# lelecaruso/NavierStokes_Project_NM4PDE

Hardware: AMD Instinct MI355X
Metric: time-steps/sec (assemble_time_step + solve_time_step), 3D flow past a cylinder, P2/P1, Yosida, per-rank ILU(0) (higher is better)
Workload: dtype f64

## Files before the change

### include/nsx.h

```cpp
#ifndef NSX_H
#define NSX_H

#include <stdint.h>

#ifdef __cplusplus
extern "C" {
#endif

typedef struct nsx_handle nsx_handle;

typedef enum {
  NSX_OK = 0,
  NSX_ERR_ARG = -1,
  NSX_ERR_HIP = -2,
  NSX_ERR_UNSUPPORTED = -3,
  NSX_ERR_NOCONV = -4,
  NSX_ERR_NUMERIC = -5,
  NSX_ERR_COMM = -6
} nsx_status;

typedef enum { NSX_PREC_YOSIDA = 0, NSX_PREC_SIMPLE = 1, NSX_PREC_AYOSIDA = 2, NSX_PREC_ASIMPLE = 3 } nsx_prec;

enum {
  NSX_TEMAM = 1,
// ... 32 lines not shown
                 int n_u, int n_p);

int nsx_set_ranks(nsx_handle *h, int n_ranks, const int32_t *u_ptr, const int32_t *p_ptr);
int nsx_set_schur_blocks(nsx_handle *h, int n_blocks, const int32_t *p_ptr);

enum { NSX_ORDER_FIRST_TOUCH = 0, NSX_ORDER_COLOUR = 1, NSX_ORDER_COLOUR_ALL = 2 };
int nsx_set_internal_layout(nsx_handle *h, int n_virtual_ranks, int order, int schur_max_rows);
int nsx_layout_info(nsx_handle *h, int info[5]);
int nsx_layout_get(nsx_handle *h, int32_t *node_perm, int32_t *pnode_perm, int32_t *u_ptr, int32_t *p_ptr, int32_t *schur_ptr);

int nsx_set_solution(nsx_handle *h, const double *solution_owned);
int nsx_get_solution(nsx_handle *h, double *solution_owned);
int nsx_get_solution_ghosted(nsx_handle *h, double *solution);
int nsx_get_rhs(nsx_handle *h, double *system_rhs);
int nsx_set_rhs(nsx_handle *h, const double *system_rhs);


int nsx_assemble(nsx_handle *h, int flags);
int nsx_assemble_time_step(nsx_handle *h, int flags);
int nsx_add_rhs(nsx_handle *h, int n, const int32_t *dofs, const double *values);
int nsx_apply_boundary_values(nsx_handle *h, int n, const int32_t *dofs, const double *values);
int nsx_solve_time_step(nsx_handle *h, int prec_type, double tol_abs, double inner_rtol, int maxiter,
                        int inner_maxiter, nsx_solve_stats *stats);

int nsx_prec_initialize(nsx_handle *h, int prec_type);
int nsx_prec_vmult(nsx_handle *h, int prec_type, double inner_rtol, int inner_maxiter, double *dst, const double *src,
                   nsx_solve_stats *stats);
int nsx_system_vmult(nsx_handle *h, double *dst, const double *src);
int nsx_ilu_apply(nsx_handle *h, int which, double *dst, const double *src);

enum { NSX_INNER_FP64 = 0, NSX_INNER_FP32 = 1 };
int nsx_set_inner_precision(nsx_handle *h, int precision);
int nsx_inner_F_vmult(nsx_handle *h, double *dst, const double *src);

int nsx_export_block(nsx_handle *h, int which, int block, int n_rows, const int32_t *rowptr, const int32_t *colind,
                     double *values);
int nsx_schur_nnz(nsx_handle *h, int64_t *nnz);
int nsx_schur_get(nsx_handle *h, int32_t *rowptr, int32_t *colind, double *values);
int nsx_scalar_graph_nnz(nsx_handle *h, int which, int64_t *nnz);
int nsx_scalar_graph(nsx_handle *h, int which, int32_t *rowptr, int32_t *colind);
int nsx_ilu_get(nsx_handle *h, int which, double *values);

int nsx_set_force_faces(nsx_handle *h, int n_faces, const int32_t *cells, const int32_t *local_faces, int n_qf, const double *N2f,
                        const double *dN2f, const double *N1f, const double *wf);
int nsx_compute_forces(nsx_handle *h, double *drag, double *lift);

int nsx_profile_enable(nsx_handle *h, int on);
int nsx_profile_reset(nsx_handle *h);
int nsx_profile_count(nsx_handle *h);
int nsx_profile_get(nsx_handle *h, int i, const char **name, int64_t *launches, double *total_ms, double *bytes_per_launch);

int nsx_persistent_state(nsx_handle *h, int state[4]);

int nsx_path_info(nsx_handle *h, int info[32]);

int nsx_gram_schmidt_cycle(nsx_handle *h, int n, int m, double *vectors, double norm_guard, double *coeffs, double *norms2);

int nsx_comm_unique_id(uint8_t id[128]);
int nsx_comm_init(nsx_handle *h, int rank, int world, const uint8_t id[128]);
typedef int (*nsx_allreduce_fn)(void *ctx, double *buf, int count);
typedef int (*nsx_exchange_fn)(void *ctx, int n, const int *ranks, const double *const *send, const int *send_count,
                               double *const *recv, const int *recv_count);
int nsx_comm_init_callbacks(nsx_handle *h, int rank, int world, nsx_allreduce_fn allreduce, nsx_exchange_fn exchange, void *ctx);
int nsx_comm_counters(const nsx_handle *h, long long counts[2]);
int nsx_comm_self_halo_test(nsx_handle *h, int n_own, int n_ghost, int ncomp, double *max_err);
int nsx_set_mesh_distributed(nsx_handle *h, int n_cells, int n_cells_layer1, int dofs_per_cell, const int32_t *cell_dofs,
// ... 10 lines not shown
```

### include/nsx_host.h

```cpp
#ifndef NSX_HOST_H
#define NSX_HOST_H

#include <stdint.h>

#ifdef __cplusplus
extern "C" {
#endif

typedef struct nsxh_mesh nsxh_mesh;
typedef struct nsxh_dofs nsxh_dofs;
typedef struct nsxh_tables nsxh_tables;


nsxh_mesh *nsxh_mesh_cylinder(int dim, int m, int nr, int nxu, int nxd, int nyb, int nyt, int nz,
                              double grade_x, double grade_r);
nsxh_mesh *nsxh_mesh_cylinder_level(int dim, int level);
nsxh_mesh *nsxh_mesh_cube(int n);
nsxh_mesh *nsxh_mesh_box(int dim, int nx, int ny, int nz, const double *lo, const double *hi);
nsxh_mesh *nsxh_mesh_read_msh(const char *path);
void nsxh_mesh_free(nsxh_mesh *);

int nsxh_mesh_dim(const nsxh_mesh *);
int nsxh_mesh_n_vertices(const nsxh_mesh *);
int nsxh_mesh_n_cells(const nsxh_mesh *);
// ... 52 lines not shown
const int32_t *nsxh_rank_view_send_u_ptr(const nsxh_rank_view *);
const int32_t *nsxh_rank_view_send_u_nodes(const nsxh_rank_view *);
const int32_t *nsxh_rank_view_send_p_ptr(const nsxh_rank_view *);
const int32_t *nsxh_rank_view_send_p_nodes(const nsxh_rank_view *);


nsxh_tables *nsxh_tables_create(int dim, int rule, int order);
void nsxh_tables_free(nsxh_tables *);
int nsxh_tables_n_q(const nsxh_tables *);
int nsxh_tables_n_p2(const nsxh_tables *);
int nsxh_tables_n_p1(const nsxh_tables *);
const double *nsxh_tables_points(const nsxh_tables *);
const double *nsxh_tables_weights(const nsxh_tables *);
const double *nsxh_tables_N2(const nsxh_tables *);
const double *nsxh_tables_dN2(const nsxh_tables *);
const double *nsxh_tables_N1(const nsxh_tables *);
const double *nsxh_tables_dN1(const nsxh_tables *);
int nsxh_tables_n_qf(const nsxh_tables *);


int nsxh_write_vtu(const nsxh_dofs *, const double *solution, const char *directory, const char *basename, unsigned counter);

int nsxh_pressure_difference(const nsxh_dofs *, const double *solution, const double *point_a, const double *point_b, double *diff);


int nsxh_ilu_stream_stats(int n_rows, const int32_t *rowptr, const int32_t *colind, int n_blocks, const int32_t *block_ptr,
                          int blocks_per_wave, int ncomp, int gap, int entries_per_tick, int64_t out[6]);
int nsxh_ilu_stream_apply(int n_rows, const int32_t *rowptr, const int32_t *colind, int n_blocks, const int32_t *block_ptr,
                          int blocks_per_wave, int ncomp, int gap, int entries_per_tick, const double *lu, const double *b, double *x);

int nsxh_ilu_stream_apply_f32(int n_rows, const int32_t *rowptr, const int32_t *colind, int n_blocks, const int32_t *block_ptr,
                              int blocks_per_wave, int ncomp, int gap, int entries_per_tick, const double *lu, const double *b, double *x);

int nsxh_internal_layout(int dim, int n_cells, int dofs_per_cell, const int32_t *cell_dofs, const double *cell_coords, int n_u, int n_p,
                         int n_in_ranks, const int32_t *in_u_ptr, const int32_t *in_p_ptr, int n_virtual, int order, int schur_max_rows,
                         int32_t *node_perm, int32_t *pnode_perm, int32_t *n_ranks, int32_t *u_ptr, int32_t *p_ptr, int32_t *n_schur,
                         int32_t *schur_ptr, int32_t *colours);

#ifdef __cplusplus
}
#endif
#endif
```

### navierstokes_project_nm4pde_amd/csrc/nsx_blas.hip

```cpp
#include "nsx_grid.hpp"
#include "nsx_ilu_lanes.hpp"

namespace nsx {

constexpr int RED_BLOCKS = 512;
constexpr int RED_STRIDE = 1024;

struct SRef {
  double c;
  int num, den;
  int num_nb, den_nb;
};

__device__ __forceinline__ double wave_sum_all(double v) {
#pragma unroll
  for (int o = 32; o > 0; o >>= 1) v += __shfl_xor(v, o, 64);
  return v;
}

__device__ __forceinline__ double slot_value(const double *__restrict__ scal, const double *__restrict__ partial, int slot, int nb,
                                             double *sh) {
  if (nb == 0) return scal[slot];
  if (threadIdx.x < 64) {
    const double *p = partial + (size_t)slot * RED_STRIDE;
// ... 1780 lines not shown
    double nrm2 = read_scalar(h, S_LS_NORM);
    if (nrm2 != nrm2) {
      v_dot(h, sp, w, w, S_LS_NORM);
      nrm2 = read_scalar(h, S_LS_NORM);
    }
    out[dim] = nrm2;
    if (ran_ahead) h->mgs_redo_ahead = true;
    return false;
  }
  if (!normalize) return false;
  return !consider || std::sqrt(out[dim]) > 10. * std::sqrt(out[dim + 1]) * 1.4901161193847656e-08;
}

__global__ __launch_bounds__(256) void k_axpby(int n, int split, int gap, double *__restrict__ d, SRef s, SRef a, const double *__restrict__ v,
                                               const double *__restrict__ scal, const double *__restrict__ partial, int mode) {
  __shared__ double sh;
  const double sv = mode == 1 ? 0.0 : sval(scal, partial, s, &sh), av = mode == 2 ? 0.0 : sval(scal, partial, a, &sh);
#pragma unroll 4
  for (int i0 = blockIdx.x * 256 + threadIdx.x; i0 < n; i0 += gridDim.x * 256) {
    const int i = i0 + (i0 >= split ? gap : 0);
    if (mode == 0) d[i] = sv * d[i] + av * v[i];
    else if (mode == 1) d[i] = av * v[i];
    else d[i] = sv * d[i];
  }
}
__global__ void k_scale_vec(int n, double *__restrict__ d, const double *__restrict__ f) {
  for (int i = blockIdx.x * 256 + threadIdx.x; i < n; i += gridDim.x * 256) d[i] *= f[i];
}
struct MultiArgs {
  const double *v[32];
  double c[32];
  int k;
};
__global__ void k_axpy_multi(int n, int split, int gap, double *__restrict__ x, MultiArgs m) {
  for (int i0 = blockIdx.x * 256 + threadIdx.x; i0 < n; i0 += gridDim.x * 256) {
    const int i = i0 + (i0 >= split ? gap : 0);
    double s = x[i];
    for (int j = 0; j < m.k; ++j) s += m.c[j] * m.v[j][i];
    x[i] = s;
  }
}
__global__ __launch_bounds__(256) void k_cg_update(int n, double *__restrict__ x, const double *__restrict__ dvec, double *__restrict__ g,
                                                   const double *__restrict__ hvec, SRef a, const double *__restrict__ scal,
                                                   const double *__restrict__ partial_in, double *__restrict__ partial) {
  __shared__ double sh[5];
  const double alpha = sval(scal, partial_in, a, sh + 4);
  double acc = 0.0;
#pragma unroll 2
  for (int i = blockIdx.x * 256 + threadIdx.x; i < n; i += gridDim.x * 256) {
    x[i] += alpha * dvec[i];
    const double gi = g[i] + alpha * hvec[i];
    g[i] = gi;
    acc += gi * gi;
  }
  const double t = block_sum_256(acc, sh);
  if (threadIdx.x == 0) partial[blockIdx.x] = t;
}

static int ew_blocks(int n) { return std::max(1, std::min(2048, cdiv(n, 512))); }

static void axpby(nsx_handle *h, Span sp, double *d, SRef s, SRef a, const double *v, int mode, double bytes_per) {
  const int n = sp.n;
  LaunchScope ls(h, "axpby", bytes_per * n);
  hipLaunchKernelGGL(k_axpby, dim3(ew_blocks(n)), dim3(256), 0, h->stream, n, sp.split, sp.gap, d, s, a, v, h->scal.p, h->red_partial.p, mode);
}

void v_copy(nsx_handle *h, int n, double *d, const double *s) {
  if (d != s && n) HIP_CHECK(hipMemcpyAsync(d, s, (size_t)n * sizeof(double), hipMemcpyDeviceToDevice, h->stream));
}
void v_zero(nsx_handle *h, int n, double *d) {
  if (n) HIP_CHECK(hipMemsetAsync(d, 0, (size_t)n * sizeof(double), h->stream));
}
void v_add(nsx_handle *h, Span n, double *d, double a, const double *v) { axpby(h, n, d, SRef{1, -1, -1, 0, 0}, SRef{a, -1, -1, 0, 0}, v, 0, 24); }
void v_add_dev(nsx_handle *h, Span n, double *d, double a, int slot, const double *v) {
  axpby(h, n, d, SRef{1, -1, -1, 0, 0}, sref(h, a, slot, -1), v, 0, 24);
}
void v_sadd(nsx_handle *h, Span n, double *d, double s, double a, const double *v) {
  axpby(h, n, d, SRef{s, -1, -1, 0, 0}, SRef{a, -1, -1, 0, 0}, v, 0, 24);
}
void v_scale(nsx_handle *h, Span n, double *d, double a) { axpby(h, n, d, SRef{a, -1, -1, 0, 0}, SRef{0, -1, -1, 0, 0}, nullptr, 2, 16); }
void v_scale_dev_inv(nsx_handle *h, Span n, double *d, int slot) { axpby(h, n, d, sref(h, 1, -1, slot), SRef{0, -1, -1, 0, 0}, nullptr, 2, 16); }
void v_scale_vec(nsx_handle *h, int n, double *d, const double *f) {
  LaunchScope ls(h, "scale_vec", 24.0 * n);
  hipLaunchKernelGGL(k_scale_vec, dim3(ew_blocks(n)), dim3(256), 0, h->stream, n, d, f);
}
void v_axpy_multi(nsx_handle *h, Span sp, double *x, int k, double *const *vs, const double *coef) {
  const int n = sp.n;
  for (int j0 = 0; j0 < k; j0 += 32) {
    MultiArgs m;
    m.k = std::min(32, k - j0);
    for (int j = 0; j < m.k; ++j) {
      m.v[j] = vs[j0 + j];
      m.c[j] = coef[j0 + j];
    }
    LaunchScope ls(h, "axpy_multi", 8.0 * n * (2 + m.k));
    hipLaunchKernelGGL(k_axpy_multi, dim3(ew_blocks(n)), dim3(256), 0, h->stream, n, sp.split, sp.gap, x, m);
  }
}

void cg_update(nsx_handle *h, int n, double *x, const double *d, double *g, const double *hv, int gh_slot, int dh_slot, int res_slot) {
  LaunchScope ls(h, "cg_update", 48.0 * n);
  const int nb = red_blocks(h, n);
  hipLaunchKernelGGL(k_cg_update, dim3(nb), dim3(256), 0, h->stream, n, x, d, g, hv, sref(h, 1, gh_slot, dh_slot), h->scal.p,
                     h->red_partial.p, red_out(h, res_slot, nb));
  after_reduction(h, res_slot, nb);
}
void cg_direction(nsx_handle *h, int n, double *d, const double *hv, int num_slot, int den_slot) {
  axpby(h, n, d, sref(h, 1, num_slot, den_slot), SRef{-1, -1, -1, 0, 0}, hv, 0, 24);
}

double read_scalar(nsx_handle *h, int slot) {
  double v;
  read_scalars(h, slot, 1, &v);
  return v;
}
unsigned long long publish_scalars(nsx_handle *h, int slot0, int count) {
  if (count > 64) NSX_THROW(NSX_ERR_ARG, "internal: read_scalars range too long");
  NbArgs args;
  for (int i = 0; i < count; ++i) {
    args.nb[i] = h->slot_nb[slot0 + i];
    h->slot_nb[slot0 + i] = 0;
  }
  const unsigned long long seq = ++h->pub_seq;
  unsigned long long *flag_dev = (unsigned long long *)(h->pub_dev + N_SLOTS);
  hipLaunchKernelGGL(k_publish, dim3(count), dim3(256), 0, h->stream, slot0, count, args, h->red_partial.p, h->scal.p, h->pub_dev, flag_dev, seq,
                     h->pub_counter.p);
  return seq;
}
void collect_published(nsx_handle *h, unsigned long long seq, int slot0, int count, double *out) {
// ... 93 lines not shown
    info[7] = h->cu_reserved;
    info[8] = h->cg_last_path;
    info[9] = h->schedS.n_blocks;
    info[10] = (int)h->haloU.nbr.size();
    info[11] = h->haloU.nbr.empty() ? 0 : h->haloU.send_ptr[h->haloU.nbr.size()];
    info[12] = h->N2_loc - h->N2;
    info[13] = h->schedS.dense ? 1 : 0;
    info[14] = h->mgs_disabled ? 1 : 0;
    info[15] = h->n_persistent_fallbacks;
    if (!h->mgs_disabled) {
      nsx::mgs_setup(h);
      auto fit = [&](int n, const int *caps, int n_inst) {
        for (int k = 0; k < n_inst; ++k) {
          const int es[3] = {8, 10, 12};
          if (caps[k] <= 0) continue;
          const int nwg = std::max(1, std::min(caps[k], nsx::cdiv(n, 256 * 4)));
          if (nsx::cdiv(n, (int64_t)nwg * 256) <= es[k]) return es[k];
        }
        return 0;
      };
      info[16] = fit(h->n_u, h->mgs_max_wg_dist, 1);
      info[17] = fit(h->n_u, h->mgs_dist_cap_reserved, 3);
      info[18] = fit(h->n_u + h->n_p, h->mgs_max_wg_dist, 1);
      info[19] = fit(h->n_u + h->n_p, h->mgs_dist_cap_reserved, 3);
      info[21] = fit(h->n_u, h->mgs_max_wg_e, 3);
    }
    info[20] = nsx::cdiv(std::max(1, h->schedS.n_blocks), 1024);
    info[22] = h->N2;
    info[23] = h->NP;
    info[24] = h->mgs_last_fused;
    info[25] = h->mgs_fused_launches;
    info[26] = h->inner_F_fp32_used;
    info[27] = h->ilu_F_fp32_used;
  } catch (const nsx::Error &e) {
    h->err = e.msg;
    return e.code;
  }
  return NSX_OK;
}
```

### navierstokes_project_nm4pde_amd/csrc/nsx_cg.hip

```cpp
#include "nsx_grid.hpp"

namespace nsx {

constexpr int CG_THREADS = 256;
constexpr int CG_NW = CG_THREADS / 64, CG_NG = CG_THREADS / 16;
constexpr int CG_MAXB = 256;
constexpr int CG_MAX_WG = 1024;
constexpr int CG_NV = 3;
constexpr int CG_RING = 4;
constexpr size_t CG_REGION = (size_t)CG_RING * CG_NV * CG_MAX_WG + (size_t)CG_RING * CG_NV;
enum { S_CGP = 100 };

__device__ __forceinline__ double ld_agent(const double *p) { return __hip_atomic_load(p, __ATOMIC_RELAXED, __HIP_MEMORY_SCOPE_AGENT); }
__device__ __forceinline__ void st_agent(double *p, double v) { __hip_atomic_store(p, v, __ATOMIC_RELAXED, __HIP_MEMORY_SCOPE_AGENT); }

template <int W>
__device__ __forceinline__ double cg_group_sum(double v) {
  v += dpp_f64<0xB1>(v);
  v += dpp_f64<0x4E>(v);
  if (W >= 8) v += dpp_f64<0x141>(v);
  if (W >= 16) v += dpp_f64<0x140>(v);
  return v;
}

// ... 100 lines not shown
                                              double (&va)[CG_PF], int (&la)[CG_PF]) {
  const int grp = tid >> 4, lane = tid & 15;
  double vb[CG_PF];
  int lb[CG_PF];
  double acc = 0.0;
#define NSX_CG_USE(V, L, S0)                                    \
  _Pragma("unroll") for (int k = 0; k < CG_PF; ++k) {           \
    const int s_ = (S0) + k;                                    \
    if (s_ < s1) {                                              \
      acc += V[k] * xst[L[k]];                                  \
      const int inf = sinfo[s_];                                \
      if (inf & 0x8000) {                                       \
        const double r_ = cg_group_sum<16>(acc);                \
        if (lane == 0) hvs[(inf & 0x7fff) * 16 + grp] = r_;     \
        acc = 0.0;                                              \
      }                                                         \
    }                                                           \
  }
  for (int sb = s0; sb < s1; sb += 2 * CG_PF) {
    NSX_CG_LOAD(vb, lb, sb + CG_PF)
    NSX_CG_USE(va, la, sb)
    NSX_CG_LOAD(va, la, sb + 2 * CG_PF)
    NSX_CG_USE(vb, lb, sb + CG_PF)
  }
#undef NSX_CG_USE
}
#undef NSX_CG_LOAD

template <int RPG, bool LRES>
__global__ __launch_bounds__(CG_THREADS) void k_cg_schur(const int32_t *__restrict__ bptr, const int32_t *__restrict__ u_ptr,
                                                  const int32_t *__restrict__ u_cols, const int32_t *__restrict__ s_ptr,
                                                  const double *__restrict__ sval, const uint16_t *__restrict__ slidx,
                                                  const int32_t *__restrict__ sinfo, const int64_t *__restrict__ dn_off,
                                                  const double *__restrict__ P, const double *__restrict__ b, double *x, double *D0, double *D1,
                                                  double *H, double rtol, int maxiter, unsigned long long *box, unsigned long long *box_other,
                                                  double *pub_vals, unsigned long long *pub_flag, unsigned long long seq, int *err_dev, int drop_wg,
                                                  const int32_t *__restrict__ a_rowptr, const double *__restrict__ a_val,
                                                  const uint16_t *__restrict__ a_lidx) {
  static_assert(!LRES || RPG > 0, "the LDS-resident operator needs the register-resident block inverses");
  constexpr int MAXB = RPG > 0 ? 16 * RPG : CG_MAXB;
  __shared__ double gs[MAXB], hs[MAXB], ds[MAXB], hvs[MAXB], xs[MAXB], xst[CG_MAX_UCOLS];
  __shared__ double sh[4][CG_NV * 8], bc[CG_NV];
  __shared__ int s_err;
  __shared__ double lval[LRES ? CG_LPOOL : 1];
  __shared__ uint16_t lidx[LRES ? CG_LPOOL : 2];
  __shared__ int lrow[LRES ? MAXB + 1 : 1];
  const int wg = blockIdx.x, tid = threadIdx.x, nwg = gridDim.x;
  if (tid == 0) s_err = 0;
  for (size_t q = (size_t)wg * CG_THREADS + tid; q < CG_REGION; q += (size_t)nwg * CG_THREADS) box_other[q] = GX_EMPTY;
  const int r0 = bptr[wg], nb = bptr[wg + 1] - r0;
  const int u0 = u_ptr[wg], nu = u_ptr[wg + 1] - u0;
  const int half = tid >> 8, ht = tid & 255;
  const int s0 = s_ptr[3 * wg + half], s1 = s_ptr[3 * wg + (CG_THREADS == 512 ? half + 1 : 2)];
  const double *Pb = P + dn_off[wg];
  const int grp = tid >> 4, lane = tid & 15;
  const bool own = tid < nb;
  int e = 0;
  constexpr int NU = CG_MAX_UCOLS / CG_THREADS;
  int ucol[NU];
#pragma unroll
  for (int k = 0; k < NU; ++k) ucol[k] = tid + CG_THREADS * k < nu ? u_cols[u0 + tid + CG_THREADS * k] : -1;
  if (tid < MAXB) gs[tid] = 0.0;

  double pa[8], pb[8];
  auto fetch = [&](int q, double(&pv)[8]) {
    const bool live = q < nb;
    const double *prow = Pb + (size_t)(live ? q : 0) * nb;
// ... 76 lines not shown
  double va[LRES ? 1 : CG_PF];
  int la[LRES ? 1 : CG_PF];
  if constexpr (LRES) {
    const int p0 = a_rowptr[r0], nz = a_rowptr[r0 + nb] - p0;
    for (int q = tid; q < nz; q += CG_THREADS) {
      lval[q] = a_val[p0 + q];
      lidx[q] = a_lidx[p0 + q];
    }
    if (tid <= nb) lrow[tid] = a_rowptr[r0 + tid] - p0;
  }
  auto prefetch_A = [&]() {
    if constexpr (!LRES) cg_spmv_prefetch(s0, s1, sval, slidx, ht, va, la);
  };
  auto block_spmv = [&]() {
    if constexpr (LRES) {
#pragma unroll
      for (int r = 0; r < RPG; ++r) {
        const int q = grp + CG_NG * r;
        if (q < nb) {
          const int e1 = lrow[q + 1];
          double acc = 0.0;
          for (int e = lrow[q] + lane; e < e1; e += 16) acc += lval[e] * xst[lidx[e]];
          acc = cg_group_sum<16>(acc);
          if (lane == 0) hvs[q] = acc;
        }
      }
    } else {
      cg_block_spmv(s0, s1, sval, slidx, sinfo, xst, hvs, ht, va, la);
    }
  };

  double bi = 0.0;
  if (own) {
    xs[tid] = x[r0 + tid];
    bi = b[r0 + tid];
  }
#pragma unroll
  for (int k = 0; k < NU; ++k)
    if (ucol[k] >= 0) xst[tid + CG_THREADS * k] = x[ucol[k]];
  prefetch_A();
  __syncthreads();
  block_spmv();
  __syncthreads();
  prefetch_P();
  if (own) gs[tid] = hvs[tid] - bi;
  __syncthreads();
  apply_P();
  double tot3[3];
  {
    const double part[3] = {own ? gs[tid] * gs[tid] : 0.0, own ? bi * bi : 0.0, own ? gs[tid] * hs[tid] : 0.0};
    cg_post<3>(part, box, e, nwg, sh, &s_err, wg == drop_wg);
    prefetch_A();
    if (!cg_collect<3>(tot3, box, e++, bc, &s_err)) {
      if (tid == 0) __hip_atomic_store(err_dev, 1, __ATOMIC_RELAXED, __HIP_MEMORY_SCOPE_AGENT);
      if (wg == 0 && tid == 0) {
        __hip_atomic_store(pub_vals + 2, 3.0, __ATOMIC_RELAXED, __HIP_MEMORY_SCOPE_SYSTEM);
        asm volatile("s_waitcnt vmcnt(0)" ::: "memory");
        __hip_atomic_store(pub_flag, seq, __ATOMIC_RELAXED, __HIP_MEMORY_SCOPE_SYSTEM);
      }
      return;
    }
  }
  const double tol = rtol * sqrt(tot3[1]);
  double res = sqrt(tot3[0]), gh = tot3[2], beta = 0.0;
  int it = 0;
  int conv = res <= tol ? 1 : ((it >= maxiter || res != res) ? 2 : 0);
  bool dead = false;
  while (conv == 0) {
    ++it;
    const double *Dp = (it & 1) ? D0 : D1;
    double *Dc = (it & 1) ? D1 : D0;
#pragma unroll
// ... 122 lines not shown
  hipLaunchKernelGGL(k_cg_pack, dim3(cdiv(pl.n_slots, 256)), dim3(256), 0, h->stream, pl.n_slots, pl.s_src.p, h->vSchur.p, pl.s_val.p);
  pl.values_current = true;
}

static void cg_setup(nsx_handle *h) {
  if (h->cg_box.p || h->cg_disabled) return;
  h->cg_max_wg = 0;
  if (getenv("NSX_CG_PERSISTENT") && atoi(getenv("NSX_CG_PERSISTENT")) == 0) {
    h->cg_disabled = true;
    return;
  }
  int cus = 0, per_cu = 0;
  HIP_CHECK(hipDeviceGetAttribute(&cus, hipDeviceAttributeMultiprocessorCount, h->prm.device));
  int per_cu_res[2] = {0, 0};
  HIP_CHECK(hipOccupancyMaxActiveBlocksPerMultiprocessor(&per_cu, k_cg_schur<0, false>, CG_THREADS, 0));
  HIP_CHECK(hipOccupancyMaxActiveBlocksPerMultiprocessor(&per_cu_res[0], k_cg_schur<6, false>, CG_THREADS, 0));
  HIP_CHECK(hipOccupancyMaxActiveBlocksPerMultiprocessor(&per_cu_res[1], k_cg_schur<8, false>, CG_THREADS, 0));
  h->cg_max_wg_res[0] = std::min(CG_MAX_WG, per_cu_res[0] * cus);
  h->cg_max_wg_res[1] = std::min(CG_MAX_WG, per_cu_res[1] * cus);
  int per_cu_lres[2] = {0, 0};
  HIP_CHECK(hipOccupancyMaxActiveBlocksPerMultiprocessor(&per_cu_lres[0], k_cg_schur<6, true>, CG_THREADS, 0));
  HIP_CHECK(hipOccupancyMaxActiveBlocksPerMultiprocessor(&per_cu_lres[1], k_cg_schur<8, true>, CG_THREADS, 0));
  h->cg_max_wg_lres[0] = std::min(CG_MAX_WG, per_cu_lres[0] * cus);
  h->cg_max_wg_lres[1] = std::min(CG_MAX_WG, per_cu_lres[1] * cus);
  h->cg_box.alloc(2 * CG_REGION + 2);
  HIP_CHECK(hipMemsetAsync(h->cg_box.p, 0xff, 2 * CG_REGION * sizeof(unsigned long long), h->stream));
  HIP_CHECK(hipMemsetAsync(h->cg_box.p + 2 * CG_REGION, 0, 2 * sizeof(unsigned long long), h->stream));
  h->cg_max_wg = std::min(CG_MAX_WG, per_cu * cus);
  if (getenv("NSX_DEBUG"))
    fprintf(stderr, "[nsx] persistent Schur CG: %d CUs x %d resident workgroups, grid <= %d (block inverses in registers: <= 96 rows x %d, <= 128 rows x %d; operator in LDS as well: x %d, x %d)\n", cus, per_cu,
            h->cg_max_wg, per_cu_res[0], per_cu_res[1], per_cu_lres[0], per_cu_lres[1]);
}

bool cg_schur_persistent(nsx_handle *h, double *x, const double *b, double rtol, int maxiter, int *steps, double *last, int *status) {
  const IluSchedule &s = h->schedS;
  const CgPlan &pl = h->cgplan;
  if (h->comm || !s.dense || s.max_rows > CG_MAXB || !pl.ok || !pl.values_current) return false;
  cg_setup(h);
  if (h->cg_max_wg == 0 || s.n_blocks > h->cg_max_wg) return false;
  const bool pres_ok = !(getenv("NSX_CG_PRES") && atoi(getenv("NSX_CG_PRES")) == 0);
  const int rpg = !pres_ok ? 0 : (s.max_rows <= 96 && s.n_blocks <= h->cg_max_wg_res[0]) ? 6 : (s.max_rows <= 128 && s.n_blocks <= h->cg_max_wg_res[1]) ? 8 : 0;
  const bool pres = rpg > 0;
  const bool lres_ok = !(getenv("NSX_CG_LRES") && atoi(getenv("NSX_CG_LRES")) == 0);
  const bool lres = lres_ok && pres && pl.max_block_nnz <= CG_LPOOL && s.n_blocks <= h->cg_max_wg_lres[rpg == 6 ? 0 : 1];
  const int n = h->n_p;
  if ((int)h->cg_vec.n < 3 * n) h->cg_vec.alloc((size_t)3 * n);
  double *D0 = h->cg_vec.p, *D1 = D0 + n, *H = D1 + n;
  const unsigned long long seq = ++h->pub_seq;
  unsigned long long *box = h->cg_box.p + (size_t)h->cg_parity * CG_REGION, *box_other = h->cg_box.p + (size_t)(1 - h->cg_parity) * CG_REGION;
  int *err_dev = (int *)(h->cg_box.p + 2 * CG_REGION);
  double *pub_vals = h->pub_dev + S_CGP;
  unsigned long long *pub_flag = (unsigned long long *)(h->pub_dev + N_SLOTS);
  ProfEntry *pe = nullptr;
  {
    LaunchScope ls(h, "cg_S", 0.0);
    pe = ls.e;
#define NSX_CG_GO(PRES_, LRES_)                                                                                                                       \
  hipLaunchKernelGGL((k_cg_schur<PRES_, LRES_>), dim3(s.n_blocks), dim3(CG_THREADS), 0, h->stream, s.block_ptr.p, pl.u_ptr.p, pl.u_cols.p, pl.s_ptr.p,  \
                     pl.s_val.p, pl.s_lidx.p, pl.s_info.p, s.dn_off.p, s.dn_P.p, b, x, D0, D1, H, rtol, maxiter, box, box_other, pub_vals, pub_flag, seq, \
                     err_dev, h->gx_drop_wg, h->gS.rowptr.p, h->vSchur.p, pl.a_lidx.p)
    if (rpg == 6 && lres) NSX_CG_GO(6, true); else if (rpg == 8 && lres) NSX_CG_GO(8, true);
    else if (rpg == 6) NSX_CG_GO(6, false); else if (rpg == 8) NSX_CG_GO(8, false); else NSX_CG_GO(0, false);
#undef NSX_CG_GO
    if (getenv("NSX_DEBUG") && (h->cg_resident != pres || h->cg_lds_resident != lres || !h->cg_variant_said)) {
      fprintf(stderr, "[nsx] Schur CG variant: block inverses in registers %d (rows per lane group %d), operator in LDS %d (largest block: %d entries)\n", (int)pres, rpg,
              (int)lres, (int)pl.max_block_nnz);
      h->cg_variant_said = true;
    }
    h->cg_resident = pres;
    h->cg_lds_resident = lres;
  }
  h->cg_parity ^= 1;
  h->cg_last_path = 2;
  wait_published(h, seq);
  const int st = (int)h->pub_host[S_CGP + 2];
  if (st == 3) {
    HIP_CHECK(hipStreamSynchronize(h->stream));
    HIP_CHECK(hipMemsetAsync(h->cg_box.p, 0xff, 2 * CG_REGION * sizeof(unsigned long long), h->stream));
    HIP_CHECK(hipMemsetAsync(h->cg_box.p + 2 * CG_REGION, 0, 2 * sizeof(unsigned long long), h->stream));
    h->cg_max_wg = 0;
    h->cg_disabled = true;
    h->n_persistent_fallbacks++;
    fprintf(stderr, "[nsx] warning: the persistent Schur CG timed out (grid not co-resident): this handle uses one launch per operation from now on\n");
    return false;
  }
  *steps = (int)h->pub_host[S_CGP];
  *last = h->pub_host[S_CGP + 1];
  *status = st;
  if (pe) pe->bytes += (lres ? 1.0 : (double)(*steps + 1)) * 10.0 * h->gS.nnz() + (double)(*steps + 1) * 48.0 * n + (pres ? 1.0 : (double)(*steps + 1)) * 8.0 * (double)s.dn_entries;
  return true;
}

// ... 264 lines not shown
```

### navierstokes_project_nm4pde_amd/csrc/nsx_internal.hpp

```cpp
#pragma once
#include <hip/hip_runtime.h>

#include <cstdint>
#include <cstdio>
#include <cstring>
#include <map>
#include <string>
#include <functional>
#include <vector>

#include "../../include/nsx.h"
#include "../host/graph.hpp"

#ifndef NSX_NT
#define NSX_NT 1
#endif
template <int BIT, class T>
__device__ __forceinline__ T ld_stream(const T *p) {
  if constexpr ((NSX_NT & BIT) != 0) return __builtin_nontemporal_load(p);
  else return *p;
}

namespace nsx {

// ... 165 lines not shown
  int N2_loc = 0, NP_loc = 0;
  int n_cells1 = 0;
  int g_u = 0, g_p = 0, off_p = 0, len_blk = 0, len_u = 0, len_p = 0;
  bool dist = false;
  int rank = 0, world = 1, goff_u = 0, goff_p = 0, n_u_glob = 0, n_p_glob = 0;
  std::vector<int32_t> ghost_u, ghost_p;
  nsx::HaloPlan haloU, haloP;
  nsx::RowSplit splitA, splitVel, splitB, splitG, splitS;
  hipStream_t comm_stream = nullptr;
  hipEvent_t ev_ready = nullptr;
  bool have_tables = false, have_mesh = false, assembled = false, prec_ready = false;
  std::vector<double> N2_h, dN2_h, N1_h, w_h;
  nsx::DevBuf<double> tab_N2, tab_dN2, tab_N1, tab_w, tab_N2T, tab_dN2T;
  nsx::DevBuf<int32_t> cell_n2, cell_n1;
  nsx::DevBuf<double> geo;
  std::vector<int32_t> cell_n2_h, cell_n1_h;
  std::vector<int32_t> cell_n2_in, cell_n1_in;
  std::vector<double> cell_coords_in;
  std::vector<int32_t> in_rank_u_h, in_rank_p_h, in_sblk_h;
  int layout_req_ranks = 0, layout_req_order = 0, layout_req_schur = 0;
  bool layout_on = false;
  int layout_colours = 0, layout_colours_p = 0;
  std::vector<int32_t> perm2_h, perm1_h, iperm2_h, iperm1_h;
  nsx::DevBuf<int32_t> perm2_d, perm1_d;
  nsx::DevBuf<double> io_stage;
  nsx::Csr caller_graph[2];
  std::vector<int32_t> caller_pos[2];
  nsx::DevCsr gA, gG, gB, gS, gPM;
  nsx::SpmvBlocked blkA;
  nsx::DevBuf<double> vS0, vMass, vStiff, vConv, vF, vG, vB, vPM, vSchur, luF, luS;
  int inner_precision = NSX_INNER_FP64;
  nsx::DevBuf<float> vF32;
  int inner_F_fp32_used = 0, ilu_F_fp32_used = 0;
  nsx::DevBuf<int32_t> bt_of_g;
  nsx::GatherMap gmA, gmG, gmB, gmPM;
  nsx::DevBuf<double> cellbuf;
  nsx::DevBuf<double> sol, sol_owned, prev_sol, rhs;
  std::vector<int32_t> rank_u_h, rank_p_h, sblk_h;
  nsx::DevBuf<int32_t> rank_u;
  nsx::IluSchedule schedF, schedS;
  nsx::DevBuf<double> dbar;
  nsx::DevBuf<int32_t> bc_dofs;
  nsx::DevBuf<double> bc_vals;
  nsx::DevBuf<double> dirmask;
  std::vector<int32_t> bc_cache;
  nsx::DevBuf<double> diag_D, diag_D_inv, neg_diag_D_inv, lump_M, schur_w;
  nsx::DevBuf<double> schur_w_prev;
  bool schur_valid = false, schur_pending = false;
  int schur_type = -1;
  std::vector<nsx::DevBuf<double> *> pool;
  nsx::DevBuf<double> red_partial;
  nsx::DevBuf<double> scal;
  int slot_nb[nsx::N_SLOTS] = {0};
  double *scal_host = nullptr;
  double *pub_host = nullptr, *pub_dev = nullptr;
  unsigned long long pub_seq = 0;
  nsx::DevBuf<unsigned int> pub_counter;
  nsx::DevBuf<unsigned long long> mgs_box;
  bool sched_dirty = true;
  int mgs_used_wg[2] = {0, 0}, mgs_used_steps[2] = {0, 0};
  int mgs_parity = 0, mgs_max_wg = 0;
  int mgs_max_wg_e[3] = {0, 0, 0};
  int mgs_links = 2;
  bool mgs_disabled = false;
  double mgs_guard_override = -1.0;
  int gx_drop_wg = -1;
// ... 56 lines not shown
  LaunchScope(nsx_handle *h_, const char *name, double bytes) : h(h_) {
    if (!h->prof_on) return;
    e = &h->prof[name];
    e->bytes += bytes;
    (void)hipEventCreate(&a);
    (void)hipEventCreate(&b);
    (void)hipEventRecord(a, h->stream);
  }
  ~LaunchScope() {
    if (!e) return;
    (void)hipEventRecord(b, h->stream);
    e->launches++;
    e->pending.emplace_back(a, b);
  }
};

inline int cdiv(int64_t a, int64_t b) { return (int)((a + b - 1) / b); }

void setup_ilu_schedule(nsx_handle *h, const Csr &g, const std::vector<int32_t> &block_ptr, IluSchedule &s, int blocks_per_wave, bool allow_dense = false,
                        int ncomp = 1);
void build_schur_graph(nsx_handle *h);
void vec_from_caller(nsx_handle *h, double *dev, const double *host, bool with_ghosts);
void vec_to_caller(nsx_handle *h, const double *dev, double *host);
void part_from_caller(nsx_handle *h, int which, double *dev, const double *host);
void part_to_caller(nsx_handle *h, int which, const double *dev, double *host);
inline int32_t node_to_internal(const nsx_handle *h, int32_t local_node) { return h->layout_on ? h->perm2_h[local_node] : local_node; }
inline int32_t pnode_to_internal(const nsx_handle *h, int32_t local_node) { return h->layout_on ? h->perm1_h[local_node] : local_node; }
void ensure_schedules(nsx_handle *h);

void run_assemble(nsx_handle *h, bool first, int flags);
void run_dirichlet(nsx_handle *h, int n, const int32_t *dofs, const double *vals);

bool blocked_usable(const nsx_handle *h);
void spmv_F(nsx_handle *h, const double *vals, const double *x, double *y, const float *vals32 = nullptr);
void spmv_F_inner(nsx_handle *h, const double *x, double *y);
void convert_F_f32(nsx_handle *h);
void spmv_saddle(nsx_handle *h, const double *x, double *y);
void spmv_G(nsx_handle *h, const double *xp, double *yu, bool accumulate);
void spmv_B(nsx_handle *h, const double *xu, double *yp);
void spmv_S(nsx_handle *h, const double *x, double *y);
void schur_numeric(nsx_handle *h, const double *w);
void ilu_factor(nsx_handle *h, const DevCsr &g, IluSchedule &s, const double *vals, double *lu, const char *name, bool f32 = false);
void ilu_check(nsx_handle *h);
bool ilu_solve(nsx_handle *h, const DevCsr &g, const IluSchedule &s, const double *lu, const double *b, double *x, int ncomp,
               const char *name, int dot_slot = -1, bool f32 = false, int *used_f32 = nullptr);
void extract_diag(nsx_handle *h, const DevCsr &g, const double *vals, double *d);
void abs_rowsum(nsx_handle *h, const DevCsr &g, const double *vals, double *d);

struct Span {
  int n, split, gap;
  Span(int n_) : n(n_), split(n_), gap(0) {}
  Span(int n_, int split_, int gap_) : n(n_), split(split_), gap(gap_) {}
};
inline Span blk_span(const nsx_handle *h) { return Span(h->n_u + h->n_p, h->n_u, h->g_u); }

template <int CTRL>
__device__ __forceinline__ double dpp_f64(double v) {
  int lo = __double2loint(v), hi = __double2hiint(v);
  lo = __builtin_amdgcn_update_dpp(0, lo, CTRL, 0xf, 0xf, true);
  hi = __builtin_amdgcn_update_dpp(0, hi, CTRL, 0xf, 0xf, true);
  return __hiloint2double(hi, lo);
}
template <int CTRL, int ROW_MASK>
__device__ __forceinline__ double dpp_f64_rows(double v) {
  int lo = __double2loint(v), hi = __double2hiint(v);
  lo = __builtin_amdgcn_update_dpp(0, lo, CTRL, ROW_MASK, 0xf, false);
  hi = __builtin_amdgcn_update_dpp(0, hi, CTRL, ROW_MASK, 0xf, false);
  return __hiloint2double(hi, lo);
}

void v_copy(nsx_handle *h, int n, double *d, const double *s);
void v_zero(nsx_handle *h, int n, double *d);
void v_add(nsx_handle *h, Span n, double *d, double a, const double *v);
void v_add_dev(nsx_handle *h, Span n, double *d, double a, int slot, const double *v);
void v_sadd(nsx_handle *h, Span n, double *d, double s, double a, const double *v);
void v_scale(nsx_handle *h, Span n, double *d, double a);
void v_scale_dev_inv(nsx_handle *h, Span n, double *d, int slot);
void v_scale_vec(nsx_handle *h, int n, double *d, const double *f);
void v_dot(nsx_handle *h, Span n, const double *a, const double *b, int slot);
void v_add_and_dot(nsx_handle *h, Span n, double *d, double a, int aslot, const double *v, const double *w, int slot);
bool v_mgs(nsx_handle *h, Span n, double *w, int dim, double *const *vs, int slot0, bool normalize, double *out,
           const std::function<void()> *after_launch = nullptr, bool consider = false, double *gram = nullptr, const double *ilu_rhs = nullptr);
void v_axpy_multi(nsx_handle *h, Span n, double *x, int k, double *const *vs, const double *coef_host);
void finalize_slots(nsx_handle *h, int slot0, int count);
double *red_out(nsx_handle *h, int slot, int nb);
void after_reduction(nsx_handle *h, int slot, int nb);
void defer_reductions(nsx_handle *h, bool on);
double read_scalar(nsx_handle *h, int slot);
void read_scalars(nsx_handle *h, int slot0, int count, double *out);
unsigned long long publish_scalars(nsx_handle *h, int slot0, int count);
void collect_published(nsx_handle *h, unsigned long long seq, int slot0, int count, double *out);
void wait_published(nsx_handle *h, unsigned long long seq);
void build_cg_plan(nsx_handle *h);
void cg_pack_values(nsx_handle *h);
bool cg_schur_persistent(nsx_handle *h, double *x, const double *b, double rtol, int maxiter, int *steps, double *last, int *status);
bool cg_schur_fused(nsx_handle *h, double *x, const double *b, double rtol, int maxiter, int *steps, double *last, int *status);
void write_scalar(nsx_handle *h, int slot, double v);

void prec_initialize(nsx_handle *h, int type);
void prec_confirm(nsx_handle *h);
void prec_vmult(nsx_handle *h, int type, double inner_rtol, int inner_maxiter, double *dst, const double *src,
                nsx_solve_stats *st);
void solve_time_step(nsx_handle *h, int type, double tol, double inner_rtol, int maxiter, int inner_maxiter,
                     nsx_solve_stats *st);

void comm_allreduce_scalars(nsx_handle *h, int slot0, int count);
void comm_allreduce_partials(nsx_handle *h, double *partials, int count);
bool comm_agree_all(nsx_handle *h, bool mine);
void comm_release_cus(nsx_handle *h);
bool comm_reserve_cus(nsx_handle *h);
bool comm_streams_concurrent(nsx_handle *h);
bool comm_on_stream(const nsx_handle *h);
void comm_ext_allreduce(nsx_handle *h, double *vals, int count, int fail_word, unsigned int *arrive, unsigned int expected, unsigned long long *flag,
                        unsigned long long seq);
void comm_halo(nsx_handle *h, HaloPlan &plan, double *x, int ncomp);
void comm_halo_begin(nsx_handle *h, HaloPlan &plan, double *x, int ncomp,
                     const std::function<void(hipStream_t, double *sendbuf, const int32_t *send_idx, int n_send)> *packer = nullptr);
void comm_halo_finish(nsx_handle *h, HaloPlan &plan, double *x, int ncomp);
void build_row_splits(nsx_handle *h);
inline void comm_halo_u(nsx_handle *h, const double *x) { if (h->dist) comm_halo(h, h->haloU, const_cast<double *>(x), h->dim); }
inline void comm_halo_p(nsx_handle *h, const double *x) { if (h->dist) comm_halo(h, h->haloP, const_cast<double *>(x), 1); }
void comm_destroy(nsx_handle *h);

}
```

### navierstokes_project_nm4pde_amd/csrc/nsx_setup.hip

```cpp
#include <algorithm>
#include <cmath>
#include <numeric>

#include "nsx_internal.hpp"
#include "../host/ilu_stream.hpp"
#include "../host/layout.hpp"

using namespace nsx;

static thread_local std::string g_create_error;

namespace nsx {

static void upload_csr(nsx_handle *h, DevCsr &d, bool square) {
  d.rowptr.upload(d.host.rowptr, h->stream);
  d.colind.upload(d.host.colind, h->stream);
  if (square) {
    std::vector<int32_t> diag(d.host.n_rows);
    for (int32_t i = 0; i < d.host.n_rows; ++i) {
      diag[i] = find_in_row(d.host, i, i);
      if (diag[i] < 0) NSX_THROW(NSX_ERR_ARG, "square graph has no diagonal entry in row %d", i);
    }
    d.diag.upload(diag, h->stream);
  }
// ... 168 lines not shown
    }
    const int64_t limit = getenv("NSX_DENSE_MAX") ? atoll(getenv("NSX_DENSE_MAX")) : ((int64_t)32 << 20);
    if (off[nb] > 0 && (off[nb] <= limit || (s.max_rows <= 256 && !getenv("NSX_DENSE_MAX"))) && s.max_rows <= 4096) {
      s.dense = true;
      s.dn_entries = off[nb];
      s.dn_off.upload(off, h->stream);
      s.dn_P.alloc((size_t)off[nb]);
      if (getenv("NSX_DEBUG")) fprintf(stderr, "[nsx] ilu schedule: explicit block inverses, %lld entries (%.1f MB)\n", (long long)off[nb], 8e-6 * off[nb]);
    }
  }
  const bool stream_fits = ((size_t)s.max_rows + 64) * sizeof(double) * ncomp <= 65536;
  s.n_waves = 0;
  s.n_slabs = 0;
  s.stream_ncomp = 0;
  if (!s.dense && stream_fits) {
    IluStream st;
    const int ept = getenv("NSX_ILU_EPT") ? std::max(1, std::min(4, atoi(getenv("NSX_ILU_EPT")))) : 2;
    build_ilu_stream(g, bptr, std::max(1, blocks_per_wave), ncomp, 2, st, ept);
    s.stream_ncomp = ncomp;
    s.stream_epl = st.epl;
    s.blocks_per_wave = blocks_per_wave;
    s.n_waves = st.n_waves;
    s.max_wave_rows = st.max_wave_rows;
    s.n_slabs = st.n_slabs;
    s.packed_ok = st.ok;
    if (getenv("NSX_DEBUG"))
      fprintf(stderr, "[nsx] ilu schedule: rows %d blocks %d max_rows %d levels(max) %d lane-owner stream: %d waves (%d blocks each), %d entries per tick, slabs %lld (max/wave %lld) fill %.2f, "
                      "%.1f MB, in-block entries %lld, LDS rows/wave <= %d%s\n",
              g.n_rows, nb, s.max_rows, s.max_levels, st.n_waves, blocks_per_wave, st.epl, (long long)st.n_slabs, (long long)st.max_wave_slabs,
              (double)st.used_slots / (double)std::max<int64_t>(1, st.n_slabs * 64 * st.epl), 1e-6 * (double)st.n_slabs * 64 * (8 * st.epl + 4 * ilu_meta_words(st.epl)),
              (long long)st.in_block_nnz, st.max_wave_rows, st.ok ? "" : " (too many: not used)");
    s.pk_row_ptr.upload(st.row_ptr, h->stream);
    s.pk_rows.upload(st.rows, h->stream);
    {
      std::vector<int32_t> slot(g.n_rows);
      for (size_t k = 0; k < st.rows.size(); ++k) slot[st.rows[k]] = (int32_t)k;
      s.pk_dinv_slot.upload(slot, h->stream);
    }
    s.pk_slab_ptr.upload(st.slab_ptr, h->stream);
    s.pk_meta.upload(reinterpret_cast<const int32_t *>(st.meta.data()), st.meta.size(), h->stream);
    s.pk_slot_of.upload(st.slot_of, h->stream);
    s.pk_val.alloc((size_t)(st.n_slabs + ILU_STREAM_PAD) * 64 * st.epl);
    s.pk_val.zero(h->stream);
    s.pk_val32.release();
    s.stream_f32 = false;
    s.pk_dinv.alloc(g.n_rows);
  }

}

void build_blocked(nsx_handle *h, const Csr &g, const std::vector<int32_t> &bounds, SpmvBlocked &b, int n_own) {
  b.n_chunks = (int)bounds.size() - 1;
  std::vector<int32_t> cptr((size_t)b.n_chunks + 1, 0), ucols, tmp;
  std::vector<uint16_t> lidx(g.nnz());
  b.max_ucols = b.max_rows = 0;
  for (int c = 0; c < b.n_chunks; ++c) {
    const int r0 = bounds[c], r1 = bounds[c + 1];
    b.max_rows = std::max(b.max_rows, r1 - r0);
    tmp.assign(g.colind.begin() + g.rowptr[r0], g.colind.begin() + g.rowptr[r1]);
    std::sort(tmp.begin(), tmp.end());
    tmp.erase(std::unique(tmp.begin(), tmp.end()), tmp.end());
    if (tmp.size() > 65535) NSX_THROW(NSX_ERR_UNSUPPORTED, "blocked SpMV: chunk touches more than 65535 columns");
    for (int p = g.rowptr[r0]; p < g.rowptr[r1]; ++p)
      lidx[p] = (uint16_t)(std::lower_bound(tmp.begin(), tmp.end(), g.colind[p]) - tmp.begin());
    ucols.insert(ucols.end(), tmp.begin(), tmp.end());
    cptr[c + 1] = (int32_t)ucols.size();
    b.max_ucols = std::max<int>(b.max_ucols, (int)tmp.size());
  }
  b.ucols_total = (double)ucols.size();
  auto make_desc = [&](const std::vector<int32_t> &chunks, DevBuf<int32_t> &out, int &grid, std::vector<int32_t> *order) {
    const int nc = (int)chunks.size();
// ... 994 lines not shown
```

### navierstokes_project_nm4pde_amd/csrc/nsx_solve.hip

```cpp
#include <chrono>
#include <cmath>
#include <functional>
#include <memory>

#include "nsx_internal.hpp"

namespace nsx {

void cg_update(nsx_handle *h, int n, double *x, const double *d, double *g, const double *hv, int gh_slot, int dh_slot, int res_slot);
void cg_direction(nsx_handle *h, int n, double *d, const double *hv, int num_slot, int den_slot);
void v_reciprocal(nsx_handle *h, int n, double *d, const double *s, double num);

struct Tmp {
  nsx_handle *h;
  DevBuf<double> *b;
  Tmp(nsx_handle *h_, size_t n) : h(h_), b(nullptr) {
    for (size_t i = 0; i < h->pool.size(); ++i)
      if (h->pool[i]->n >= n) {
        b = h->pool[i];
        h->pool.erase(h->pool.begin() + i);
        break;
      }
    if (!b) {
      b = new DevBuf<double>();
      b->alloc(n);
      b->zero(h->stream);
    }
  }
  ~Tmp() { h->pool.push_back(b); }
  Tmp(const Tmp &) = delete;
  double *p() const { return b->p; }
};

using Op = std::function<void(double *dst, const double *src)>;

struct SolveResult {
  int status;
  int steps;
  double last;
};

struct DeferScope {
  nsx_handle *h;
  bool active;
  DeferScope(nsx_handle *h_, bool on) : h(h_), active(on) {
    if (active) defer_reductions(h, true);
  }
  void release() {
    if (!active) return;
    active = false;
    defer_reductions(h, false);
  }
  ~DeferScope() {
    if (!active) return;
    h->defer_red = false;
    h->pending_red.clear();
  }
};

static int sc_check(int step, double value, double tol, int maxsteps) {
  if (value <= tol) return 1;
  if (step >= maxsteps || std::isnan(value)) return 2;
  return 0;
}

static double now_s() { return std::chrono::duration<double>(std::chrono::steady_clock::now().time_since_epoch()).count(); }

constexpr int N_TMP = 30;
enum { S_H = 8 , S_NRM = 40, S_H2 = 41 , S_DH = 2, S_GH = 3, S_RES = 4, S_GH2 = 5 , S_T = 6 };

static SolveResult gmres(nsx_handle *h, const Op &A, double *x, const double *b, const Op &P, Span n, int len, double tol, int maxiter,
                         bool zero_new = false, bool x_is_zero = false, bool plain_P = false, bool P_is_ilu_F = false) {
  SolveResult res{1, 0, 0.0};
  std::vector<std::unique_ptr<Tmp>> tmp(N_TMP);
  auto vec = [&](int i) -> double * {
    if (!tmp[i]) {
      tmp[i] = std::make_unique<Tmp>(h, len);
      if (zero_new) v_zero(h, len, tmp[i]->p());
    }
    return tmp[i]->p();
  };
  struct Depth {
    nsx_handle *h;
    int d;
    explicit Depth(nsx_handle *h_) : h(h_), d(h_->gmres_depth++) {}
    ~Depth() { h->gmres_depth--; }
  } depth(h);
  double *gram = nullptr;
  if (depth.d < 4) {
    if (!h->ls_gram.p) {
      h->ls_gram.alloc(4 * 1024);
      h->ls_gram.zero(h->stream);
    }
    gram = h->ls_gram.p + (size_t)depth.d * 1024;
  }
  const bool ilu_conv = P_is_ilu_F && h->inner_precision == NSX_INNER_FP64  && !h->comm && h->schedF.packed_ok && !h->schedF.levelled && h->schedF.stream_ncomp == h->dim &&
                        (getenv("NSX_ILU_MGS") && atoi(getenv("NSX_ILU_MGS")) == 1);
  double H[N_TMP][N_TMP - 1];
  double gamma[N_TMP], ci[N_TMP - 1], si[N_TMP - 1], hh[N_TMP + 2], h2[N_TMP + 2];
  int accumulated = 0, state = 0, dim = 0;
  bool re_orth = false;
  double *v = vec(0), *p = vec(N_TMP - 1);
  int ahead = 0;
  do {
    ahead = 0;
    if (x_is_zero) {
      P(v, b);
      x_is_zero = false;
    } else {
      A(p, x);
      v_sadd(h, n, p, -1., 1., b);
      P(v, p);
    }
    v_dot(h, n, v, v, S_NRM);
    double rho = std::sqrt(read_scalar(h, S_NRM));
    res.last = rho;
    state = sc_check(accumulated, rho, tol, maxiter);
    if (state != 0) break;
    gamma[0] = rho;
    v_scale(h, n, v, 1. / rho);
    dim = 0;
    double rho_before = 0.0;
    for (int inner = 0; inner < N_TMP - 2 && state == 0; ++inner) {
      ++accumulated;
      static const bool trace = getenv("NSX_TRACE") != nullptr;
      if (trace && h->gmres_depth == 1) fprintf(stderr, "[nsx trace] rank %d: outer iteration %d, residual %.3e\n", h->rank, accumulated, rho);
      double *vv = vec(inner + 1);
      auto apply_AP = [&](double *dst, const double *src) {
        A(p, src);
        P(dst, p);
      };
      const bool fuse = ilu_conv && !re_orth;
      if (ilu_conv) {
        if (ahead == 0) A(vv, vec(inner));
        if (!fuse) {
          v_copy(h, n.n, p, vv);
          P(vv, p);
        }
      } else if (ahead == 0) apply_AP(vv, vec(inner));
      else if (ahead == 1) P(vv, p);
      ahead = 0;
      dim = inner + 1;
      const bool consider = !re_orth && (inner % 5 == 4);
      double *basis[N_TMP];
      for (int i = 0; i < dim; ++i) basis[i] = vec(i);
      static const double ahead_margin = getenv("NSX_AHEAD_MARGIN") ? atof(getenv("NSX_AHEAD_MARGIN")) : 2.0;
      const bool likely_last = rho_before > 0.0 && rho * std::min(1.0, rho / rho_before) <= ahead_margin * tol;
      const std::function<void()> next_A = [&]() {
        if (inner + 1 < N_TMP - 2 && !likely_last) {
          static const int ahead_mode = getenv("NSX_AHEAD_MODE") ? atoi(getenv("NSX_AHEAD_MODE")) : 2;
          if (ilu_conv) {
            A(vec(inner + 2), vv);
            ahead = 1;
          } else if (plain_P && ahead_mode == 2) {
            apply_AP(vec(inner + 2), vv);
            ahead = 2;
          } else {
            A(p, vv);
            ahead = 1;
          }
        }
// ... 10 lines not shown
      }
      if (re_orth) {
        normalized = v_mgs(h, n, vv, dim, basis, S_H2, true, h2, nullptr, false, gram);
        for (int i = 0; i < dim; ++i) hh[i] += h2[i];
        s = std::sqrt(h2[dim]);
      }
      hh[inner + 1] = s;
      if (s != 0 && !normalized) v_scale(h, n, vv, 1. / s);
      for (int i = 0; i < inner; ++i) {
        const double sn = si[i], cs = ci[i], dummy = hh[i];
        hh[i] = cs * dummy + sn * hh[i + 1];
        hh[i + 1] = -sn * dummy + cs * hh[i + 1];
      }
      const double r = 1. / std::sqrt(hh[inner] * hh[inner] + hh[inner + 1] * hh[inner + 1]);
      si[inner] = hh[inner + 1] * r;
      ci[inner] = hh[inner] * r;
      hh[inner] = ci[inner] * hh[inner] + si[inner] * hh[inner + 1];
      gamma[inner + 1] = -si[inner] * gamma[inner];
      gamma[inner] *= ci[inner];
      for (int i = 0; i < dim; ++i) H[i][inner] = hh[i];
      rho_before = rho;
      rho = std::fabs(gamma[dim]);
      res.last = rho;
      state = sc_check(accumulated, rho, tol, maxiter);
    }
    double y[N_TMP];
    for (int i = dim - 1; i >= 0; --i) {
      double s = gamma[i];
      for (int j = i + 1; j < dim; ++j) s -= H[i][j] * y[j];
      y[i] = s / H[i][i];
    }
    double *vs[N_TMP];
    for (int i = 0; i < dim; ++i) vs[i] = vec(i);
    v_axpy_multi(h, n, x, dim, vs, y);
  } while (state == 0);
  res.status = state == 1 ? 0 : 1;
  res.steps = accumulated;
  return res;
}

using OpDot = std::function<bool(double *dst, const double *src, int slot)>;
static SolveResult cg(nsx_handle *h, const Op &A, double *x, const double *b, const Op &P, Span n, int len, double tol, int maxiter,
                      const OpDot *Pdot = nullptr) {
  auto apply_P_dot = [&](double *dst, const double *src, int slot) {
    if (Pdot && (*Pdot)(dst, src, slot)) return;
    if (!Pdot) P(dst, src);
    v_dot(h, n, src, dst, slot);
  };
  SolveResult res{1, 0, 0.0};
  Tmp g(h, len), d(h, len), hv(h, len);
  int it = 0;
  A(g.p(), x);
  v_add(h, n, g.p(), -1., b);
  v_dot(h, n, g.p(), g.p(), S_RES);
  double r = std::sqrt(read_scalar(h, S_RES));
  res.last = r;
  int conv = sc_check(0, r, tol, maxiter);
  if (conv == 0) {
    int gh = S_GH, gh_new = S_GH2;
    apply_P_dot(hv.p(), g.p(), gh);
    v_copy(h, n.n, d.p(), hv.p());
    v_scale(h, n, d.p(), -1.);
    while (conv == 0) {
      it++;
      A(hv.p(), d.p());
      v_dot(h, n, d.p(), hv.p(), S_DH);
      const bool batch = h->comm != nullptr;
      DeferScope defer(h, batch);
// ... 101 lines not shown
  }
  if (h->schur_pending) {
    h->schur_pending = false;
    h->schur_valid = true;
  }
}

static void count(nsx_solve_stats *st, bool F, const SolveResult &r) {
  if (!st) return;
  if (F) {
    st->inner_F_iterations += r.steps;
    st->n_F_solves++;
  } else {
    st->inner_S_iterations += r.steps;
    st->n_S_solves++;
  }
  if (r.status) st->status = 2;
}

void prec_vmult(nsx_handle *h, int type, double tol, int maxit, double *dst, const double *src, nsx_solve_stats *st) {
  if (!h->prec_ready) NSX_THROW(NSX_ERR_ARG, "preconditioner not initialised");
  const int n_u = h->n_u, n_p = h->n_p, dim = h->dim, len_u = h->len_u, len_p = h->len_p;
  const double *src_u = src, *src_p = src + h->off_p;
  double *dst_u = dst, *dst_p = dst + h->off_p;
  Op Fm = [h](double *d, const double *s) { spmv_F_inner(h, s, d); };
  const bool f32 = h->inner_precision == NSX_INNER_FP32;
  Op Sm = [h](double *d, const double *s) { spmv_S(h, s, d); };
  Op PF = [h, dim, f32](double *d, const double *s) {
    int used = 0;
    ilu_solve(h, h->gA, h->schedF, h->luF.p, s, d, dim, "ilu_solve_F", -1, f32, &used);
    if (used) h->ilu_F_fp32_used = 1;
  };
  Op PS = [h](double *d, const double *s) { ilu_solve(h, h->gS, h->schedS, h->luS.p, s, d, 1, "ilu_solve_S"); };
  OpDot PSdot = [h](double *d, const double *s, int slot) { return ilu_solve(h, h->gS, h->schedS, h->luS.p, s, d, 1, "ilu_solve_S", slot); };
  auto cg_S = [&](double *x, const double *b) {
    int steps = 0, status = 0;
    double last = 0.0;
    if (cg_schur_persistent(h, x, b, tol, maxit, &steps, &last, &status)) return SolveResult{status, steps, last};
    if (cg_schur_fused(h, x, b, tol, maxit, &steps, &last, &status)) return SolveResult{status, steps, last};
    h->cg_last_path = 1;
    return cg(h, Sm, x, b, PS, n_p, len_p, tol * norm2(h, n_p, b), maxit, &PSdot);
  };

  if (type == NSX_PREC_YOSIDA) {
    Tmp yu(h, len_u), yp(h, len_p), tmp(h, len_p), tmp2(h, len_u), res(h, len_u);
    v_copy(h, n_u, yu.p(), src_u);
    v_copy(h, n_p, yp.p(), src_p);
    count(st, true, gmres(h, Fm, yu.p(), src_u, PF, n_u, len_u, tol * norm2(h, n_u, src_u), maxit, false, false, true, true));
    spmv_B(h, yu.p(), tmp.p());
    v_add(h, n_p, tmp.p(), -1.0, src_p);
    count(st, false, cg_S(yp.p(), tmp.p()));
    v_copy(h, n_p, dst_p, yp.p());
    spmv_G(h, dst_p, tmp2.p(), false);
    v_zero(h, n_u, res.p());
    v_copy(h, n_u, dst_u, yu.p());
    count(st, true, gmres(h, Fm, res.p(), tmp2.p(), PF, n_u, len_u, tol * norm2(h, n_u, tmp2.p()), maxit, false, true, true, true));
    v_sadd(h, n_u, dst_u, -1., 1., res.p());
  } else if (type == NSX_PREC_SIMPLE) {
    Tmp sol1_u(h, len_u), sol1_p(h, len_p), temp_1(h, len_p), tmp(h, len_u);
    v_copy(h, n_u, sol1_u.p(), src_u);
    v_copy(h, n_p, sol1_p.p(), src_p);
    count(st, true, gmres(h, Fm, sol1_u.p(), src_u, PF, n_u, len_u, tol * norm2(h, n_u, src_u), maxit, false, false, true, true));
    spmv_B(h, sol1_u.p(), temp_1.p());
    v_add(h, n_p, temp_1.p(), -1.0, src_p);
    count(st, false, cg_S(sol1_p.p(), temp_1.p()));
    v_copy(h, n_p, dst_p, sol1_p.p());
    v_scale(h, n_p, dst_p, 1. / 0.5);
    v_copy(h, n_u, dst_u, sol1_u.p());
    spmv_G(h, dst_p, tmp.p(), false);
    v_scale_vec(h, n_u, tmp.p(), h->diag_D_inv.p);
    v_add(h, n_u, dst_u, -1.0, tmp.p());
  } else if (type == NSX_PREC_ASIMPLE) {
    Tmp tmp_u(h, len_u), tmp_p(h, len_p);
    count(st, true, gmres(h, Fm, dst_u, src_u, PF, n_u, len_u, tol * norm2(h, n_u, src_u), maxit, false, false, true, true));
    spmv_B(h, dst_u, dst_p);
    v_sadd(h, n_p, dst_p, -1.0, 1.0, src_p);
    v_copy(h, n_p, tmp_p.p(), dst_p);
    count(st, false, gmres(h, Sm, dst_p, tmp_p.p(), PS, n_p, len_p, tol * norm2(h, n_p, tmp_p.p()), maxit));
    v_scale_vec(h, n_u, dst_u, h->diag_D.p);
    v_scale(h, n_p, dst_p, 1. / 1.0);
    spmv_G(h, dst_p, tmp_u.p(), false);
    v_add(h, n_u, dst_u, -1.0, tmp_u.p());
    v_scale_vec(h, n_u, dst_u, h->diag_D_inv.p);
  } else if (type == NSX_PREC_AYOSIDA) {
    Tmp tmp(h, len_u), tmp2(h, len_p), yu(h, len_u), yp(h, len_p), t(h, len_u);
    v_copy(h, n_p, yp.p(), src_p);
    v_copy(h, n_u, tmp.p(), src_u);
    v_scale_vec(h, n_u, tmp.p(), h->diag_D_inv.p);
    v_copy(h, n_u, yu.p(), tmp.p());
    spmv_B(h, tmp.p(), tmp2.p());
    v_sadd(h, n_p, yp.p(), -1.0, 1.0, tmp2.p());
    count(st, false, cg_S(dst_p, yp.p()));
    v_copy(h, n_p, yp.p(), dst_p);
    spmv_F_inner(h, yu.p(), t.p());
    v_copy(h, n_u, yu.p(), t.p());
    spmv_G(h, yp.p(), tmp.p(), false);
    v_sadd(h, n_u, yu.p(), -1.0, 1.0, tmp.p());
    v_scale_vec(h, n_u, yu.p(), h->diag_D_inv.p);
    v_copy(h, n_u, dst_u, yu.p());
  } else {
    NSX_THROW(NSX_ERR_ARG, "Invalid preconditioner type");
  }
}

void solve_time_step(nsx_handle *h, int type, double tol, double inner_rtol, int maxiter, int inner_maxiter, nsx_solve_stats *st) {
  HIP_CHECK(hipSetDevice(h->prm.device));
  const Span n = blk_span(h);
  nsx_solve_stats local;
  if (!st) st = &local;
  memset(st, 0, sizeof(*st));
  h->inner_F_fp32_used = h->ilu_F_fp32_used = 0;
  v_copy(h, h->len_blk, h->prev_sol.p, h->sol.p);
  HIP_CHECK(hipStreamSynchronize(h->stream));
  double t0 = now_s();
  h->defer_red = false;
  h->pending_red.clear();
  static const bool trace = getenv("NSX_TRACE") != nullptr;
  if (trace) fprintf(stderr, "[nsx trace] rank %d: solve_time_step: preconditioner set-up\n", h->rank);
  prec_initialize(h, type);
  HIP_CHECK(hipStreamSynchronize(h->stream));
  prec_confirm(h);
  if (trace) fprintf(stderr, "[nsx trace] rank %d: solve_time_step: outer solve\n", h->rank);
  st->t_prec = now_s() - t0;
  t0 = now_s();
  Op A = [h](double *d, const double *s) { spmv_saddle(h, s, d); };
  Op P = [h, type, inner_rtol, inner_maxiter, st](double *d, const double *s) { prec_vmult(h, type, inner_rtol, inner_maxiter, d, s, st); };
  SolveResult r = gmres(h, A, h->sol_owned.p, h->rhs.p, P, n, h->len_blk, tol, maxiter, true);
  v_copy(h, h->len_blk, h->sol.p, h->sol_owned.p);
  comm_halo_u(h, h->sol.p);
  comm_halo_p(h, h->sol.p + h->off_p);
  HIP_CHECK(hipStreamSynchronize(h->stream));
  ilu_check(h);
  st->t_solve = now_s() - t0;
  st->outer_iterations = r.steps;
  st->final_residual = r.last;
  st->persistent_fallbacks = h->n_persistent_fallbacks;
  if (r.status && st->status == 0) st->status = 1;
}

__global__ void k_reciprocal(int n, double *__restrict__ d, const double *__restrict__ s, double num) {
  const int i = blockIdx.x * blockDim.x + threadIdx.x;
  if (i < n) d[i] = num / s[i];
}
void v_reciprocal(nsx_handle *h, int n, double *d, const double *s, double num) {
// ... 19 lines not shown

int nsx_solve_time_step(nsx_handle *h, int prec_type, double tol_abs, double inner_rtol, int maxiter, int inner_maxiter,
                        nsx_solve_stats *stats) {
  NSX_API_BODY(h, {
    if (!h->assembled) NSX_THROW(NSX_ERR_ARG, "assemble before solving");
    nsx::solve_time_step(h, prec_type, tol_abs, inner_rtol, maxiter, inner_maxiter, stats);
    if (stats && stats->status) {
      h->err = stats->status == 1 ? "outer GMRES did not converge (SolverControl::NoConvergence)" : "an inner solve did not converge";
      return NSX_ERR_NOCONV;
    }
  })
}

int nsx_prec_initialize(nsx_handle *h, int prec_type) {
  NSX_API_BODY(h, {
    nsx::prec_initialize(h, prec_type);
    HIP_CHECK(hipStreamSynchronize(h->stream));
    nsx::prec_confirm(h);
  })
}

int nsx_prec_vmult(nsx_handle *h, int prec_type, double inner_rtol, int inner_maxiter, double *dst, const double *src, nsx_solve_stats *stats) {
  NSX_API_BODY(h, {
    if (!dst || !src) NSX_THROW(NSX_ERR_ARG, "null vector");
    if (h->dist) NSX_THROW(NSX_ERR_UNSUPPORTED, "nsx_prec_vmult with host vectors works on a single-process handle only");
    HIP_CHECK(hipSetDevice(h->prm.device));
    const int n = h->n_u + h->n_p;
    nsx::Tmp d(h, n), s(h, n);
    nsx::vec_from_caller(h, s.p(), src, false);
    nsx::vec_from_caller(h, d.p(), dst, false);
    if (stats) memset(stats, 0, sizeof(*stats));
    h->defer_red = false;
    h->pending_red.clear();
    h->inner_F_fp32_used = h->ilu_F_fp32_used = 0;
    nsx::prec_vmult(h, prec_type, inner_rtol, inner_maxiter, d.p(), s.p(), stats);
    if (stats) stats->persistent_fallbacks = h->n_persistent_fallbacks;
    nsx::vec_to_caller(h, d.p(), dst);
    nsx::ilu_check(h);
  })
}

int nsx_system_vmult(nsx_handle *h, double *dst, const double *src) {
  NSX_API_BODY(h, {
    if (!dst || !src || !h->assembled) NSX_THROW(NSX_ERR_ARG, "null vector / nothing assembled");
    HIP_CHECK(hipSetDevice(h->prm.device));
    nsx::Tmp d(h, h->len_blk), s(h, h->len_blk);
    nsx::vec_from_caller(h, s.p(), src, false);
    nsx::spmv_saddle(h, s.p(), d.p());
    nsx::vec_to_caller(h, d.p(), dst);
  })
}

int nsx_ilu_apply(nsx_handle *h, int which, double *dst, const double *src) {
  NSX_API_BODY(h, {
    if (!dst || !src || which < 0 || which > 1) NSX_THROW(NSX_ERR_ARG, "bad arguments");
    if (!h->prec_ready) NSX_THROW(NSX_ERR_ARG, "no factors: call nsx_prec_initialize first");
    if (h->dist) NSX_THROW(NSX_ERR_UNSUPPORTED, "nsx_ilu_apply with host vectors works on a single-process handle only");
    HIP_CHECK(hipSetDevice(h->prm.device));
    const int n = which == 0 ? h->n_u : h->n_p;
    nsx::Tmp d(h, n), s(h, n);
    nsx::part_from_caller(h, which, s.p(), src);
    if (which == 0) nsx::ilu_solve(h, h->gA, h->schedF, h->luF.p, s.p(), d.p(), h->dim, "ilu_solve_F", -1, h->inner_precision == NSX_INNER_FP32, &h->ilu_F_fp32_used);
    else nsx::ilu_solve(h, h->gS, h->schedS, h->luS.p, s.p(), d.p(), 1, "ilu_solve_S");
    nsx::part_to_caller(h, which, d.p(), dst);
    nsx::ilu_check(h);
  })
}

int nsx_set_inner_precision(nsx_handle *h, int precision) {
  NSX_API_BODY(h, {
    if (precision != NSX_INNER_FP64 && precision != NSX_INNER_FP32) NSX_THROW(NSX_ERR_ARG, "unknown inner precision %d (NSX_INNER_FP64 = 0, NSX_INNER_FP32 = 1)", precision);
    h->inner_precision = precision;
    h->prec_ready = false;
  })
}

int nsx_inner_F_vmult(nsx_handle *h, double *dst, const double *src) {
  NSX_API_BODY(h, {
    if (!dst || !src || !h->assembled) NSX_THROW(NSX_ERR_ARG, "null vector / nothing assembled");
    if (!h->prec_ready) NSX_THROW(NSX_ERR_ARG, "call nsx_prec_initialize first (it brings F's copy in the inner precision up to date)");
    if (h->dist) NSX_THROW(NSX_ERR_UNSUPPORTED, "nsx_inner_F_vmult with host vectors works on a single-process handle only");
    HIP_CHECK(hipSetDevice(h->prm.device));
    nsx::Tmp d(h, h->n_u), s(h, h->n_u);
    nsx::part_from_caller(h, 0, s.p(), src);
    h->inner_F_fp32_used = 0;
    nsx::spmv_F_inner(h, s.p(), d.p());
    nsx::part_to_caller(h, 0, d.p(), dst);
  })
}

}
```

### navierstokes_project_nm4pde_amd/csrc/nsx_sparse.hip

```cpp
#include <atomic>

#include "nsx_internal.hpp"
#include "nsx_ilu_lanes.hpp"

namespace nsx {

template <int LW>
__device__ __forceinline__ double lane_group_sum(double v) {
  if (LW >= 2) v += dpp_f64<0xB1>(v);
  if (LW >= 4) v += dpp_f64<0x4E>(v);
  if (LW >= 8) v += dpp_f64<0x141>(v);
  if (LW >= 16) v += dpp_f64<0x140>(v);
  if (LW >= 32) v += __shfl_xor(v, 16, 64);
  if (LW >= 64) v += __shfl_xor(v, 32, 64);
  return v;
}

template <int W>
__device__ __forceinline__ double group_sum(double v) {
  return lane_group_sum<W>(v);
}

template <int DIM, int W, bool WITH_G>
__global__ __launch_bounds__(256) void k_spmv_vel(int n_rows, const int32_t *__restrict__ rp, const int32_t *__restrict__ ci,
// ... 78 lines not shown

template <int W>
__global__ __launch_bounds__(256) void k_spmv_csr(int n_rows, const int32_t *__restrict__ rp, const int32_t *__restrict__ ci,
                                                  const double *__restrict__ v, const double *__restrict__ x,
                                                  double *__restrict__ y, const int32_t *__restrict__ rows) {
  const int slot = (blockIdx.x * 256 + threadIdx.x) / W, lane = threadIdx.x % W;
  if (slot >= n_rows) return;
  const int row = rows ? rows[slot] : slot;
  double acc = 0.0;
  const int e = rp[row + 1];
  for (int p = rp[row] + lane; p < e; p += W) acc += v[p] * x[ci[p]];
  acc = group_sum<W>(acc);
  if (lane == 0) y[row] = acc;
}

#ifdef NSX_SPMV_TRACE
__device__ unsigned long long *g_spmv_trace = nullptr;
__device__ int g_spmv_dbg = 0;
#define SPMV_DBG (g_spmv_trace ? g_spmv_dbg : 0)
#define SPMV_STAMP(k)                                                                              \
  do {                                                                                             \
    if (g_spmv_trace && threadIdx.x == 0) g_spmv_trace[(size_t)blockIdx.x * 4 + (k)] = wall_clock64(); \
  } while (0)
#else
#define SPMV_DBG 0
#define SPMV_STAMP(k) \
  do {                \
  } while (0)
#endif

template <int DIM, int W, class VT>
__device__ __forceinline__ void spmv_blocked_rows(int n_rows, const int32_t *__restrict__ desc, const int32_t *__restrict__ rp,
                                                  const uint16_t *__restrict__ lidx, const VT *__restrict__ av, const int32_t *__restrict__ ucols,
                                                  const double *__restrict__ x, double *__restrict__ y) {
  extern __shared__ double xs[];
  __shared__ int rps[449];
  const int4 d = reinterpret_cast<const int4 *>(desc)[blockIdx.x];
  const int c0 = d.x, nu = d.y, r0 = d.z, r1 = d.w;
  if (r1 <= r0) return;
  SPMV_STAMP(0);
  [[maybe_unused]] const int dbg = SPMV_DBG;
  for (int t = threadIdx.x; t <= r1 - r0; t += 256) rps[t] = rp[r0 + t];
  for (int t = threadIdx.x; t < nu && dbg != 4; t += 256) {
    const int u = dbg == 2 ? (c0 + t) % n_rows : ucols[c0 + t];
    const double *xj = x + (size_t)u * DIM;
#pragma unroll
    for (int c = 0; c < DIM; ++c) xs[t * DIM + c] = dbg == 1 ? (double)u : xj[c];
  }
  __syncthreads();
  SPMV_STAMP(1);
  static_assert(W == 8 || W == 16 || W == 32, "lanes per row");
  constexpr int G = 256 / W, U = 64 / W;
  const int grp = threadIdx.x / W, lane = threadIdx.x % W;
  double a[U], na[U];
  int l[U], nl[U];
  int row = r0 + grp;
  auto fetch = [&](int rw, double (&va)[U], int (&vl)[U]) {
    const bool live = rw < r1;
    const int p0 = live ? rps[rw - r0] + lane : 0, e = live ? rps[rw - r0 + 1] : 0;
#pragma unroll
    for (int k = 0; k < U; ++k) {
      const int q = p0 + k * W;
      const bool ok = q < e;
      va[k] = ok ? (double)ld_stream<2>(av + q) : 0.0;
      vl[k] = ok ? (int)ld_stream<2>(lidx + q) : 0;
    }
  };
  auto consume = [&](int rw, const double (&va)[U], const int (&vl)[U]) {
    if (rw >= r1) return;
    double acc[DIM];
#pragma unroll
    for (int c = 0; c < DIM; ++c) acc[c] = 0.0;
#pragma unroll
    for (int k = 0; k < U; ++k) {
      const double *xj = xs + vl[k] * DIM;
#pragma unroll
      for (int c = 0; c < DIM; ++c) acc[c] += va[k] * xj[c];
    }
    const int e = rps[rw - r0 + 1];
    for (int p = rps[rw - r0] + lane + U * W; p < e; p += W) {
      const double av_ = (double)av[p];
      const double *xj = xs + (int)lidx[p] * DIM;
#pragma unroll
      for (int c = 0; c < DIM; ++c) acc[c] += av_ * xj[c];
    }
#pragma unroll
    for (int c = 0; c < DIM; ++c) acc[c] = group_sum<W>(acc[c]);
    if (lane == 0) {
#pragma unroll
      for (int c = 0; c < DIM; ++c) y[(size_t)rw * DIM + c] = acc[c];
    }
  };
  if (SPMV_DBG == 3) row = r1;
  fetch(row, a, l);
  fetch(row + G, na, nl);
  for (; row < r1; row += 2 * G) {
    consume(row, a, l);
    fetch(row + 2 * G, a, l);
    consume(row + G, na, nl);
    fetch(row + 3 * G, na, nl);
  }
#ifdef NSX_SPMV_TRACE
  __syncthreads();
  SPMV_STAMP(2);
  if (g_spmv_trace && threadIdx.x == 0) {
    unsigned xcc, id;
    asm volatile("s_getreg_b32 %0, hwreg(HW_REG_XCC_ID)" : "=s"(xcc));
    asm volatile("s_getreg_b32 %0, hwreg(HW_REG_HW_ID)" : "=s"(id));
    g_spmv_trace[(size_t)blockIdx.x * 4 + 3] = ((unsigned long long)xcc << 32) | id;
  }
#endif
}

template <int DIM, int W>
__global__ __launch_bounds__(256) void k_spmv_blocked(int n_rows, const int32_t *__restrict__ desc, const int32_t *__restrict__ rp, const uint16_t *__restrict__ lidx,
                                                      const double *__restrict__ av, const int32_t *__restrict__ ucols, const double *__restrict__ x,
                                                      double *__restrict__ y) {
  spmv_blocked_rows<DIM, W, double>(n_rows, desc, rp, lidx, av, ucols, x, y);
}
#ifndef NSX_SPMV_F32_W
#define NSX_SPMV_F32_W 16
#endif
template <int DIM, int W>
__global__ __launch_bounds__(256) void k_spmv_blocked_f32(int n_rows, const int32_t *__restrict__ desc, const int32_t *__restrict__ rp, const uint16_t *__restrict__ lidx,
                                                          const float *__restrict__ av, const int32_t *__restrict__ ucols, const double *__restrict__ x,
                                                          double *__restrict__ y) {
  spmv_blocked_rows<DIM, W, float>(n_rows, desc, rp, lidx, av, ucols, x, y);
}

__global__ __launch_bounds__(256) void k_to_f32(int64_t n, const double *__restrict__ v, float *__restrict__ out, int *__restrict__ err) {
  const int64_t i = (int64_t)blockIdx.x * 256 + threadIdx.x;
  if (i >= n) return;
  const double d = v[i];
  const float f = (float)d;
  out[i] = f;
  if (!(fabsf(f) <= 3.402823466e+38f)) __hip_atomic_store(err, 4, __ATOMIC_RELAXED, __HIP_MEMORY_SCOPE_SYSTEM);
}

static double bytes_vel(nsx_handle *h, bool with_g, bool f32 = false) {
  double b = (f32 ? 8.0 : 12.0) * h->gA.nnz() + (double)h->N2 * (4 + 8.0 * h->dim * 2);
  if (with_g) b += (4.0 + 8.0 * h->dim) * h->gG.nnz() + 4.0 * h->N2 + 8.0 * h->NP;
  return b;
}

static void launch_vel(nsx_handle *h, bool with_g, const double *vals, const double *x, const double *xp, double *y, const int32_t *rows, int n) {
  if (n <= 0) return;
  static const int Wsel = getenv("NSX_SPMV_W") ? atoi(getenv("NSX_SPMV_W")) : 16;
#define NSX_SPMV(D, W_, G_)                                                                                                            \
  hipLaunchKernelGGL((k_spmv_vel<D, W_, G_>), dim3((cdiv((int64_t)n * W_, 256) + 7) & ~7), dim3(256), 0, h->stream, n, h->gA.rowptr.p, \
                     h->gA.colind.p, vals, x, h->gG.rowptr.p, h->gG.colind.p, h->vG.p, xp, y, rows)
  if (with_g) {
    if (h->dim == 2) NSX_SPMV(2, 16, true); else NSX_SPMV(3, 16, true);
  } else if (h->dim == 2) {
    if (Wsel == 8) NSX_SPMV(2, 8, false); else if (Wsel == 32) NSX_SPMV(2, 32, false); else NSX_SPMV(2, 16, false);
  } else {
    if (Wsel == 8) NSX_SPMV(3, 8, false); else if (Wsel == 32) NSX_SPMV(3, 32, false); else NSX_SPMV(3, 16, false);
  }
#undef NSX_SPMV
}
static void launch_B(nsx_handle *h, const double *xu, double *yp, const int32_t *rows, int n) {
  if (n <= 0) return;
  if (h->dim == 2)
    hipLaunchKernelGGL((k_spmv_B<2, 32>), dim3(cdiv((int64_t)n * 32, 256)), dim3(256), 0, h->stream, n, h->gB.rowptr.p, h->gB.colind.p, h->vB.p, xu, yp, rows);
  else
    hipLaunchKernelGGL((k_spmv_B<3, 64>), dim3(cdiv((int64_t)n * 64, 256)), dim3(256), 0, h->stream, n, h->gB.rowptr.p, h->gB.colind.p, h->vB.p, xu, yp, rows);
}
static void launch_G(nsx_handle *h, const double *xp, double *yu, bool accumulate, const int32_t *rows, int n) {
  if (n <= 0) return;
  const int W = 8, grid = cdiv((int64_t)n * W, 256);
  if (h->dim == 2)
    hipLaunchKernelGGL((k_spmv_G<2, W>), dim3(grid), dim3(256), 0, h->stream, n, h->gG.rowptr.p, h->gG.colind.p, h->vG.p, xp, yu, (int)accumulate, rows);
  else
    hipLaunchKernelGGL((k_spmv_G<3, W>), dim3(grid), dim3(256), 0, h->stream, n, h->gG.rowptr.p, h->gG.colind.p, h->vG.p, xp, yu, (int)accumulate, rows);
}
static void launch_S(nsx_handle *h, const double *x, double *y, const int32_t *rows, int n) {
  if (n <= 0) return;
  const int W = 32;
  hipLaunchKernelGGL((k_spmv_csr<W>), dim3(cdiv((int64_t)n * W, 256)), dim3(256), 0, h->stream, n, h->gS.rowptr.p, h->gS.colind.p, h->vSchur.p, x, y, rows);
}

bool blocked_usable(const nsx_handle *h) {
  static const bool blocked = !(getenv("NSX_SPMV_BLOCKED") && atoi(getenv("NSX_SPMV_BLOCKED")) == 0);
  const SpmvBlocked &b = h->blkA;
  return blocked && b.n_chunks > 0 && b.max_rows <= 448 && (size_t)b.max_ucols * h->dim * sizeof(double) <= 64 * 1024;
}
static bool launch_blocked(nsx_handle *h, const double *vals, const double *x, double *y, int part = 0, const float *vals32 = nullptr) {
  const SpmvBlocked &b = h->blkA;
  if (!blocked_usable(h)) return false;
  const size_t shm = (size_t)b.max_ucols * h->dim * sizeof(double);
  const int grid = part ? b.grid_if : b.grid;
  const int32_t *desc = part ? b.desc_if.p : b.desc.p;
  if (grid == 0) return true;
#define NSX_BLK(D) \
  hipLaunchKernelGGL((k_spmv_blocked<D, 16>), dim3(grid), dim3(256), shm, h->stream, h->N2, desc, h->gA.rowptr.p, b.lidx.p, vals, b.ucols.p, x, y)
  if (vals32) {
    if (h->dim == 2)
      hipLaunchKernelGGL((k_spmv_blocked_f32<2, NSX_SPMV_F32_W>), dim3(grid), dim3(256), shm, h->stream, h->N2, desc, h->gA.rowptr.p, b.lidx.p, vals32, b.ucols.p, x, y);
    else
      hipLaunchKernelGGL((k_spmv_blocked_f32<3, NSX_SPMV_F32_W>), dim3(grid), dim3(256), shm, h->stream, h->N2, desc, h->gA.rowptr.p, b.lidx.p, vals32, b.ucols.p, x, y);
    return true;
  }
#ifdef NSX_SPMV_TRACE
  static int n_call = 0;
  const bool traced = getenv("NSX_SPMV_TRACE_OUT") && ++n_call == (getenv("NSX_SPMV_TRACE_CALL") ? atoi(getenv("NSX_SPMV_TRACE_CALL")) : 5000);
  for (int mode = 0; traced && part == 0 && mode <= 4; ++mode) {
    unsigned long long *tr = nullptr;
    (void)hipStreamSynchronize(h->stream);
    (void)hipMalloc(&tr, (size_t)grid * 4 * sizeof(unsigned long long));
    (void)hipMemset(tr, 0, (size_t)grid * 4 * sizeof(unsigned long long));
    (void)hipMemcpyToSymbol(HIP_SYMBOL(g_spmv_trace), &tr, sizeof(tr));
    (void)hipMemcpyToSymbol(HIP_SYMBOL(g_spmv_dbg), &mode, sizeof(mode));
    if (h->dim == 2) NSX_BLK(2); else NSX_BLK(3);
    (void)hipStreamSynchronize(h->stream);
    std::vector<unsigned long long> host((size_t)grid * 4);
    (void)hipMemcpy(host.data(), tr, host.size() * sizeof(unsigned long long), hipMemcpyDeviceToHost);
    unsigned long long *none = nullptr;
    (void)hipMemcpyToSymbol(HIP_SYMBOL(g_spmv_trace), &none, sizeof(none));
    (void)hipFree(tr);
    const std::string path = std::string(getenv("NSX_SPMV_TRACE_OUT")) + "_mode" + std::to_string(mode) + ".txt";
    if (FILE *f = fopen(path.c_str(), "w")) {
      fprintf(f, "# block chunk rows ucols t_start t_staged t_end xcc hw_id   (wall_clock64 ticks of 10 ns)\n");
      std::vector<int32_t> ds((size_t)grid * 4);
      (void)hipMemcpy(ds.data(), b.desc.p, ds.size() * 4, hipMemcpyDeviceToHost);
      for (int blk = 0; blk < grid; ++blk) {
        if (b.order[blk] < 0) continue;
        fprintf(f, "%d %d %d %d %llu %llu %llu %llu %llu\n", blk, b.order[blk], ds[4 * (size_t)blk + 3] - ds[4 * (size_t)blk + 2], ds[4 * (size_t)blk + 1],
                host[4 * (size_t)blk], host[4 * (size_t)blk + 1], host[4 * (size_t)blk + 2], host[4 * (size_t)blk + 3] >> 32, host[4 * (size_t)blk + 3] & 0xffffffffull);
      }
      fclose(f);
    }
  }
#endif
  if (h->dim == 2) NSX_BLK(2); else NSX_BLK(3);
#undef NSX_BLK
  return true;
}

static double bytes_halo(const HaloPlan &p, int ncomp) {
  const int nn = (int)p.nbr.size();
  return nn ? 16.0 * (p.send_ptr[nn] + p.recv_ptr[nn]) * ncomp : 0.0;
}

void spmv_F(nsx_handle *h, const double *vals, const double *x, double *y, const float *vals32) {
  if (vals32 && !blocked_usable(h)) vals32 = nullptr;
  const bool f32 = vals32 != nullptr;
  if (f32) h->inner_F_fp32_used = 1;
  if (h->dist) {
    double *xx = const_cast<double *>(x);
    const bool blk = blocked_usable(h);
    const double frac_if = blk ? h->blkA.frac_if : (double)h->splitA.n_interface / std::max(1, h->N2);
    comm_halo_begin(h, h->haloU, xx, h->dim);
    {
      LaunchScope ls(h, "spmv_F", bytes_vel(h, false, f32) * (1.0 - frac_if));
      if (blk) launch_blocked(h, vals, x, y, 0, vals32);
      else launch_vel(h, false, vals, x, nullptr, y, h->splitA.interior.p, h->splitA.n_interior);
    }
    {
      LaunchScope ls(h, "halo_u_wait", bytes_halo(h->haloU, h->dim));
      comm_halo_finish(h, h->haloU, xx, h->dim);
    }
    {
      LaunchScope ls(h, "spmv_F_if", bytes_vel(h, false, f32) * frac_if);
      if (blk) launch_blocked(h, vals, x, y, 1, vals32);
      else launch_vel(h, false, vals, x, nullptr, y, h->splitA.interface.p, h->splitA.n_interface);
    }
    return;
  }
  LaunchScope ls(h, "spmv_F", bytes_vel(h, false, f32));
  if (!launch_blocked(h, vals, x, y, 0, vals32)) launch_vel(h, false, vals, x, nullptr, y, nullptr, h->N2);
}

void spmv_F_inner(nsx_handle *h, const double *x, double *y) {
  spmv_F(h, h->vF.p, x, y, h->inner_precision == NSX_INNER_FP32 ? h->vF32.p : nullptr);
}

static double bytes_B(nsx_handle *h) { return (4.0 + 8.0 * h->dim) * h->gB.nnz() + 12.0 * h->NP + 8.0 * h->dim * h->N2; }
void spmv_B(nsx_handle *h, const double *xu, double *yp) {
  LaunchScope ls(h, "spmv_B", bytes_B(h));
  if (h->dist) {
    double *xx = const_cast<double *>(xu);
    comm_halo_begin(h, h->haloU, xx, h->dim);
    launch_B(h, xu, yp, h->splitB.interior.p, h->splitB.n_interior);
    comm_halo_finish(h, h->haloU, xx, h->dim);
    launch_B(h, xu, yp, h->splitB.interface.p, h->splitB.n_interface);
    return;
  }
  launch_B(h, xu, yp, nullptr, h->NP);
}

void spmv_G(nsx_handle *h, const double *xp, double *yu, bool accumulate) {
  LaunchScope ls(h, "spmv_G", (4.0 + 8.0 * h->dim) * h->gG.nnz() + (double)h->N2 * (4 + 8.0 * h->dim) + 8.0 * h->NP);
  if (h->dist) {
    double *xx = const_cast<double *>(xp);
    comm_halo_begin(h, h->haloP, xx, 1);
    launch_G(h, xp, yu, accumulate, h->splitG.interior.p, h->splitG.n_interior);
    comm_halo_finish(h, h->haloP, xx, 1);
    launch_G(h, xp, yu, accumulate, h->splitG.interface.p, h->splitG.n_interface);
    return;
  }
  launch_G(h, xp, yu, accumulate, nullptr, h->N2);
}

void spmv_saddle(nsx_handle *h, const double *x, double *y) {
  double *xx = const_cast<double *>(x);
  if (h->dist) {
    comm_halo_begin(h, h->haloU, xx, h->dim);
// ... 729 lines not shown
    for (int r = grp; r < cnt; r += ngrp) {
      const int i = rowsB[l0 + r];
      double acc[NCOMP];
#pragma unroll
      for (int c = 0; c < NCOMP; ++c) acc[c] = 0.0;
      const int e = rp[i + 1];
      for (int p = diag[i] + 1 + lane; p < e; p += LW) {
        const int j = ci[p];
        if (j < r1) {
          const double u = lu[p];
#pragma unroll
          for (int c = 0; c < NCOMP; ++c) acc[c] += u * xs[(j - r0) * NCOMP + c];
        }
      }
#pragma unroll
      for (int c = 0; c < NCOMP; ++c) acc[c] = group_sum<LW>(acc[c]);
      if (lane == 0) {
#pragma unroll
        for (int c = 0; c < NCOMP; ++c) xs[(i - r0) * NCOMP + c] -= acc[c];
      }
    }
    __syncthreads();
  }
  if (USE_LDS)
    for (int t = threadIdx.x; t < nloc * NCOMP; t += 256) x[(size_t)r0 * NCOMP + t] = xs[t];
}

constexpr int LANES_K = 12;

template <int NCOMP, int E, int PF, class VT>
__device__ __forceinline__ void ilu_solve_lanes_wave(const int32_t *__restrict__ row_ptr, const int32_t *__restrict__ rows,
                                                     const int32_t *__restrict__ slab_ptr, const uint32_t *__restrict__ meta,
                                                     const VT *__restrict__ val, const double *__restrict__ dinv, const double *b, double *x,
                                                     double *__restrict__ dot_partial, int *err_host, int force_guard) {
  extern __shared__ double xs[];
  if ((uint32_t)(uintptr_t)(lds_f64 *)xs != 0u || force_guard) {
    if (threadIdx.x == 0) __hip_atomic_store(err_host, 3, __ATOMIC_RELAXED, __HIP_MEMORY_SCOPE_SYSTEM);
    return;
  }
  const int w = blockIdx.x;
  const unsigned lane = threadIdx.x;
  const int s0 = slab_ptr[2 * w], s1 = slab_ptr[2 * w + 1], s2 = slab_ptr[2 * w + 2];
  const int rb = row_ptr[w], nr = row_ptr[w + 1] - rb;
  constexpr int K = LANES_K;
  LaneSlot<E, VT> A[PF];
  lane_load<E, PF, VT>(A, s0, meta, val, lane);
  int idx0[K];
  double d0[K];
#pragma unroll
  for (int k = 0; k < K; ++k) {
    const int t = 64 * k + (int)lane;
    idx0[k] = t < nr ? rows[rb + t] : -1;
    d0[k] = t < nr ? dinv[rb + t] : 0.0;
  }
  {
    double v[K][NCOMP];
#pragma unroll
    for (int k = 0; k < K; ++k)
#pragma unroll
      for (int c = 0; c < NCOMP; ++c) v[k][c] = idx0[k] >= 0 ? b[(size_t)idx0[k] * NCOMP + c] : 0.0;
#pragma unroll
    for (int k = 0; k < K; ++k)
      if (idx0[k] >= 0) {
#pragma unroll
        for (int c = 0; c < NCOMP; ++c) xs[(64 * k + (int)lane) * NCOMP + c] = v[k][c];
      }
  }
  for (int base = 64 * K; base < nr; base += 64 * K) {
    int idx[K];
    double v[K][NCOMP];
#pragma unroll
    for (int k = 0; k < K; ++k) {
      const int t = base + 64 * k + (int)lane;
      idx[k] = t < nr ? rows[rb + t] : -1;
    }
#pragma unroll
    for (int k = 0; k < K; ++k)
#pragma unroll
      for (int c = 0; c < NCOMP; ++c) v[k][c] = idx[k] >= 0 ? b[(size_t)idx[k] * NCOMP + c] : 0.0;
#pragma unroll
    for (int k = 0; k < K; ++k)
      if (idx[k] >= 0) {
#pragma unroll
        for (int c = 0; c < NCOMP; ++c) xs[(base + 64 * k + (int)lane) * NCOMP + c] = v[k][c];
      }
  }
#pragma unroll
  for (int c = 0; c < NCOMP; ++c) xs[(nr + lane) * NCOMP + c] = 0.0;
  const uint32_t scratch = (uint32_t)(nr + lane) * (8u * NCOMP);
  __builtin_amdgcn_wave_barrier();
  lane_sweep<NCOMP, E, PF, VT>(A, s0, s1, meta, val, lane, scratch);
  lane_load<E, PF, VT>(A, s1, meta, val, lane);
#pragma unroll
  for (int k = 0; k < K; ++k) {
    const int t = 64 * k + (int)lane;
    if (t < nr) {
#pragma unroll
      for (int c = 0; c < NCOMP; ++c) xs[t * NCOMP + c] *= d0[k];
    }
  }
  for (int base = 64 * K; base < nr; base += 64 * K) {
    double d[K];
#pragma unroll
    for (int k = 0; k < K; ++k) {
      const int t = base + 64 * k + (int)lane;
      d[k] = t < nr ? dinv[rb + t] : 0.0;
    }
#pragma unroll
    for (int k = 0; k < K; ++k) {
      const int t = base + 64 * k + (int)lane;
      if (t < nr) {
#pragma unroll
        for (int c = 0; c < NCOMP; ++c) xs[t * NCOMP + c] *= d[k];
      }
    }
  }
  __builtin_amdgcn_wave_barrier();
  lane_sweep<NCOMP, E, PF, VT>(A, s1, s2, meta, val, lane, scratch);
  double dot = 0.0;
  for (int base = 0; base < nr; base += 64 * K) {
    int idx[K];
    double bv[K][NCOMP];
#pragma unroll
    for (int k = 0; k < K; ++k) {
      const int t = base + 64 * k + (int)lane;
      idx[k] = base == 0 ? idx0[k] : (t < nr ? rows[rb + t] : -1);
    }
    if (dot_partial) {
#pragma unroll
      for (int k = 0; k < K; ++k)
#pragma unroll
        for (int c = 0; c < NCOMP; ++c) bv[k][c] = idx[k] >= 0 ? b[(size_t)idx[k] * NCOMP + c] : 0.0;
    }
#pragma unroll
    for (int k = 0; k < K; ++k)
      if (idx[k] >= 0) {
#pragma unroll
        for (int c = 0; c < NCOMP; ++c) {
          const double xv = xs[(base + 64 * k + (int)lane) * NCOMP + c];
          if (dot_partial) dot += bv[k][c] * xv;
          x[(size_t)idx[k] * NCOMP + c] = xv;
        }
      }
  }
  if (dot_partial) {
    dot = lane_group_sum<64>(dot);
    if (lane == 0) dot_partial[w] = dot;
  }
}

template <int NCOMP, int E, int PF>
__global__ __launch_bounds__(64) void k_ilu_solve_lanes(const int32_t *__restrict__ row_ptr, const int32_t *__restrict__ rows,
                                                        const int32_t *__restrict__ slab_ptr, const uint32_t *__restrict__ meta,
                                                        const double *__restrict__ val, const double *__restrict__ dinv, const double *b, double *x,
                                                        double *__restrict__ dot_partial, int *err_host, int force_guard) {
  ilu_solve_lanes_wave<NCOMP, E, PF, double>(row_ptr, rows, slab_ptr, meta, val, dinv, b, x, dot_partial, err_host, force_guard);
}
template <int NCOMP, int E, int PF>
__global__ __launch_bounds__(64) void k_ilu_solve_lanes_f32(const int32_t *__restrict__ row_ptr, const int32_t *__restrict__ rows,
                                                            const int32_t *__restrict__ slab_ptr, const uint32_t *__restrict__ meta,
                                                            const float *__restrict__ val, const double *__restrict__ dinv, const double *b, double *x,
                                                            double *__restrict__ dot_partial, int *err_host, int force_guard) {
  ilu_solve_lanes_wave<NCOMP, E, PF, float>(row_ptr, rows, slab_ptr, meta, val, dinv, b, x, dot_partial, err_host, force_guard);
}

template <int NCOMP>
static void launch_lanes(nsx_handle *h, const IluSchedule &s, const double *b, double *x, double *dot_partial, bool f32) {
  const size_t shm = (size_t)(s.max_wave_rows + 64) * NCOMP * sizeof(double);
  static const int pf = getenv("NSX_PF") ? atoi(getenv("NSX_PF")) : 8;
  int *err = (int *)(h->pub_dev + N_SLOTS + 3);
  const int force_guard = getenv("NSX_ILU_LDS_GUARD_TEST") ? atoi(getenv("NSX_ILU_LDS_GUARD_TEST")) : 0;
#define NSX_GO(E_, PF_)                                                                                                                        \
  hipLaunchKernelGGL((k_ilu_solve_lanes<NCOMP, E_, PF_>), dim3(s.n_waves), dim3(64), shm, h->stream, s.pk_row_ptr.p, s.pk_rows.p, s.pk_slab_ptr.p, \
                     reinterpret_cast<const uint32_t *>(s.pk_meta.p), s.pk_val.p, s.pk_dinv.p, b, x, dot_partial, err, force_guard)
#define NSX_GO32(E_, PF_)                                                                                                                          \
  hipLaunchKernelGGL((k_ilu_solve_lanes_f32<NCOMP, E_, PF_>), dim3(s.n_waves), dim3(64), shm, h->stream, s.pk_row_ptr.p, s.pk_rows.p, s.pk_slab_ptr.p, \
                     reinterpret_cast<const uint32_t *>(s.pk_meta.p), s.pk_val32.p, s.pk_dinv.p, b, x, dot_partial, err, force_guard)
#define NSX_GO_E(E_)                                            \
  if (f32) {                                                    \
    if (pf == 4) NSX_GO32(E_, 4); else NSX_GO32(E_, 8);         \
  } else if (pf == 4) NSX_GO(E_, 4); else NSX_GO(E_, 8)
  switch (s.stream_epl) {
    case 1: NSX_GO_E(1); break;
    case 2: NSX_GO_E(2); break;
    case 3: NSX_GO_E(3); break;
    case 4: NSX_GO_E(4); break;
    default: NSX_THROW(NSX_ERR_ARG, "internal: %d entries per tick", s.stream_epl);
  }
#undef NSX_GO_E
#undef NSX_GO32
#undef NSX_GO
}

template <int NCOMP>
static void launch_ilu_solve(nsx_handle *h, const DevCsr &g, const IluSchedule &s, const double *lu, const double *b, double *x) {
  const size_t shm = (size_t)s.max_rows * NCOMP * sizeof(double);
  constexpr int LW = 8;
#define NSX_ILU_ARGS s.block_ptr.p, s.blk_lvl_off.p, s.fwd_lvl_ptr.p, s.fwd_rows.p, s.blk_lvl_off_b.p, s.bwd_lvl_ptr.p, s.bwd_rows.p, \
                     g.rowptr.p, g.colind.p, g.diag.p, lu, b, x
  if (shm <= 64 * 1024)
    hipLaunchKernelGGL((k_ilu_solve<NCOMP, LW, true>), dim3(s.n_blocks), dim3(256), shm, h->stream, NSX_ILU_ARGS);
  else
    hipLaunchKernelGGL((k_ilu_solve<NCOMP, LW, false>), dim3(s.n_blocks), dim3(256), 0, h->stream, NSX_ILU_ARGS);
#undef NSX_ILU_ARGS
}

bool ilu_solve(nsx_handle *h, const DevCsr &g, const IluSchedule &s, const double *lu, const double *b, double *x, int ncomp,
               const char *name, int dot_slot, bool f32, int *used_f32) {
  if (used_f32) *used_f32 = 0;
  if (s.levelled) {
    LaunchScope ls(h, name, 12.0 * (double)s.in_block_nnz + (double)g.n_rows() * (4 + 16.0 * ncomp));
    if (ncomp == 1) ilu_solve_levelled<1>(h, g, s, lu, b, x);
    else if (ncomp == 2) ilu_solve_levelled<2>(h, g, s, lu, b, x);
    else ilu_solve_levelled<3>(h, g, s, lu, b, x);
    return false;
  }
  const bool packed = ilu_lanes_stream(s, ncomp);
  if (s.dense && ncomp == 1 && (size_t)s.max_rows * sizeof(double) <= 48 * 1024) {
    LaunchScope ls(h, name, 8.0 * (double)s.dn_entries + 16.0 * g.n_rows());
    const bool with_dot = dot_slot >= 0 && !h->comm && s.n_blocks >= 2 && s.n_blocks <= 512;
    hipLaunchKernelGGL(k_ilu_apply_dense, dim3(s.n_blocks), dim3(DENSE_THREADS), (size_t)s.max_rows * sizeof(double), h->stream, s.block_ptr.p, s.dn_off.p,
                       s.dn_P.p, b, x, with_dot ? red_out(h, dot_slot, s.n_blocks) : nullptr);
    if (with_dot) after_reduction(h, dot_slot, s.n_blocks);
    return with_dot;
  }
  const bool lanes32 = packed && f32 && s.stream_f32;
  if (packed && s.stream_f32 && !lanes32) NSX_THROW(NSX_ERR_ARG, "internal: the double solve stream is stale (the last factorisation wrote the float stream)");
  LaunchScope ls(h, name, 12.0 * (double)s.in_block_nnz - (lanes32 ? 4.0 * (double)(s.in_block_nnz - g.n_rows()) : 0.0) + (double)g.n_rows() * (4 + 16.0 * ncomp));
  if (packed) {
    if (used_f32) *used_f32 = lanes32 ? 1 : 0;
    const bool with_dot = dot_slot >= 0 && !h->comm && s.n_waves >= 2 && s.n_waves <= 512;
    double *dp = with_dot ? red_out(h, dot_slot, s.n_waves) : nullptr;
    if (ncomp == 1) launch_lanes<1>(h, s, b, x, dp, lanes32);
    else if (ncomp == 2) launch_lanes<2>(h, s, b, x, dp, lanes32);
    else launch_lanes<3>(h, s, b, x, dp, lanes32);
    if (with_dot) after_reduction(h, dot_slot, s.n_waves);
    return with_dot;
  }
  if (ncomp == 1) launch_ilu_solve<1>(h, g, s, lu, b, x);
  else if (ncomp == 2) launch_ilu_solve<2>(h, g, s, lu, b, x);
  else launch_ilu_solve<3>(h, g, s, lu, b, x);
  return false;
}

}
```

### navierstokes_project_nm4pde_amd/frontend.py

```python
import ctypes as C

import numpy as np

from ._lib import HOST_SO, load

_i32p = C.POINTER(C.c_int32)
_f64p = C.POINTER(C.c_double)


def _lib():
    lib = load(HOST_SO)
    if getattr(lib, "_nsxh_ready", False):
        return lib
    vp = C.c_void_p
    sig = {
        "nsxh_mesh_cylinder": (vp, [C.c_int] * 8 + [C.c_double] * 2),
        "nsxh_mesh_cylinder_level": (vp, [C.c_int, C.c_int]),
        "nsxh_mesh_cube": (vp, [C.c_int]),
        "nsxh_mesh_box": (vp, [C.c_int] * 4 + [_f64p, _f64p]),
        "nsxh_mesh_read_msh": (vp, [C.c_char_p]),
        "nsxh_mesh_free": (None, [vp]),
        "nsxh_mesh_dim": (C.c_int, [vp]),
        "nsxh_mesh_n_vertices": (C.c_int, [vp]),
        "nsxh_mesh_n_cells": (C.c_int, [vp]),
# ... 13 lines not shown
        "nsxh_write_vtu": (C.c_int, [vp, C.POINTER(C.c_double), C.c_char_p, C.c_char_p, C.c_uint]),
        "nsxh_pressure_difference": (C.c_int, [vp, C.POINTER(C.c_double), C.POINTER(C.c_double), C.POINTER(C.c_double), C.POINTER(C.c_double)]),
        "nsxh_dofs_free": (None, [vp]),
        "nsxh_dofs_per_cell": (C.c_int, [vp]),
        "nsxh_n_nodes_p2": (C.c_int, [vp]),
        "nsxh_n_nodes_p1": (C.c_int, [vp]),
        "nsxh_n_u": (C.c_int, [vp]),
        "nsxh_n_p": (C.c_int, [vp]),
        "nsxh_cell_dofs": (_i32p, [vp]),
        "nsxh_cell_coords": (_f64p, [vp]),
        "nsxh_support_points": (_f64p, [vp]),
        "nsxh_node_owner": (_i32p, [vp]),
        "nsxh_pnode_owner": (_i32p, [vp]),
        "nsxh_owned_u_ptr": (_i32p, [vp]),
        "nsxh_owned_p_ptr": (_i32p, [vp]),
        "nsxh_n_subdomains": (C.c_int, [vp]),
        "nsxh_boundary_dofs": (C.c_int, [vp, C.c_int, C.POINTER(_i32p)]),
        "nsxh_reference_sparsity": (C.c_int, [vp, C.c_int, C.POINTER(_i32p), C.POINTER(_i32p)]),
        "nsxh_tables_create": (vp, [C.c_int, C.c_int, C.c_int]),
        "nsxh_tables_free": (None, [vp]),
        "nsxh_tables_n_q": (C.c_int, [vp]),
        "nsxh_tables_n_qf": (C.c_int, [vp]),
        "nsxh_tables_n_p2": (C.c_int, [vp]),
        "nsxh_tables_n_p1": (C.c_int, [vp]),
        "nsxh_tables_points": (_f64p, [vp]),
        "nsxh_tables_weights": (_f64p, [vp]),
        "nsxh_tables_N2": (_f64p, [vp]),
        "nsxh_tables_dN2": (_f64p, [vp]),
        "nsxh_tables_N1": (_f64p, [vp]),
        "nsxh_tables_dN1": (_f64p, [vp]),
        "nsxh_ilu_stream_stats": (C.c_int, [C.c_int, _i32p, _i32p, C.c_int, _i32p, C.c_int, C.c_int, C.c_int, C.c_int, C.POINTER(C.c_int64)]),
        "nsxh_ilu_stream_apply": (C.c_int, [C.c_int, _i32p, _i32p, C.c_int, _i32p, C.c_int, C.c_int, C.c_int, C.c_int, _f64p, _f64p, _f64p]),
        "nsxh_ilu_stream_apply_f32": (C.c_int, [C.c_int, _i32p, _i32p, C.c_int, _i32p, C.c_int, C.c_int, C.c_int, C.c_int, _f64p, _f64p, _f64p]),
        "nsxh_internal_layout": (C.c_int, [C.c_int, C.c_int, C.c_int, _i32p, _f64p, C.c_int, C.c_int, C.c_int, _i32p, _i32p, C.c_int, C.c_int, C.c_int,
                                           _i32p, _i32p, _i32p, _i32p, _i32p, _i32p, _i32p, _i32p]),
    }
    for name, (res, args) in sig.items():
        fn = getattr(lib, name)
        fn.restype = res
        fn.argtypes = args
    lib._nsxh_ready = True
    return lib


def _arr(ptr, shape, dtype, copy=True):
    n = int(np.prod(shape))
    if n == 0:
        return np.zeros(shape, dtype=dtype)
    nbytes = n * np.dtype(dtype).itemsize
    buf = (C.c_char * nbytes).from_address(C.cast(ptr, C.c_void_p).value)
    a = np.frombuffer(buf, dtype=dtype, count=n).reshape(shape)
    return a.copy() if copy else a


class Mesh:

    def __init__(self, handle):
        if not handle:
            raise ValueError("mesh construction failed (bad parameters or unreadable file)")
        self._h = handle
        self._lib = _lib()
        self.refresh()

    def refresh(self):
        L, h = self._lib, self._h
        self.dim = L.nsxh_mesh_dim(h)
# ... 163 lines not shown
        self.dN2 = _arr(L.nsxh_tables_dN2(h), (nq, n2, dim), np.float64)
        self.N1 = _arr(L.nsxh_tables_N1(h), (nq, n1), np.float64)
        self.dN1 = _arr(L.nsxh_tables_dN1(h), (nq, n1, dim), np.float64)
        L.nsxh_tables_free(h)


def ilu_stream_stats(rowptr, colind, block_ptr, blocks_per_wave=8, ncomp=3, gap=2, entries_per_tick=1):
    rp, ci, bp = (np.ascontiguousarray(a, dtype=np.int32) for a in (rowptr, colind, block_ptr))
    out = (C.c_int64 * 6)()
    rc = _lib().nsxh_ilu_stream_stats(len(rp) - 1, rp.ctypes.data_as(_i32p), ci.ctypes.data_as(_i32p), len(bp) - 1, bp.ctypes.data_as(_i32p),
                                      int(blocks_per_wave), int(ncomp), int(gap), int(entries_per_tick), out)
    if rc:
        raise ValueError("nsxh_ilu_stream_stats failed (%d)" % rc)
    keys = ("slabs", "max_wave_slabs", "in_block_nnz", "max_wave_rows", "waves", "used_slots")
    d = dict(zip(keys, (int(v) for v in out)))
    d["fill"] = d["used_slots"] / max(1, 64 * d["slabs"] * int(entries_per_tick))
    d["stream_bytes"] = d["slabs"] * 64 * (8 * int(entries_per_tick) + 4 * ((int(entries_per_tick) + 2) // 2))
    return d


def ilu_stream_apply(rowptr, colind, block_ptr, lu, b, ncomp=1, blocks_per_wave=8, gap=2, entries_per_tick=1, f32=False):
    rp, ci, bp = (np.ascontiguousarray(a, dtype=np.int32) for a in (rowptr, colind, block_ptr))
    lu, b = np.ascontiguousarray(lu, dtype=np.float64), np.ascontiguousarray(b, dtype=np.float64)
    x = np.empty_like(b)
    fn = _lib().nsxh_ilu_stream_apply_f32 if f32 else _lib().nsxh_ilu_stream_apply
    rc = fn(len(rp) - 1, rp.ctypes.data_as(_i32p), ci.ctypes.data_as(_i32p), len(bp) - 1, bp.ctypes.data_as(_i32p),
            int(blocks_per_wave), int(ncomp), int(gap), int(entries_per_tick), lu.ctypes.data_as(_f64p), b.ctypes.data_as(_f64p),
            x.ctypes.data_as(_f64p))
    if rc:
        raise ValueError("nsxh_ilu_stream_apply%s failed (%d)" % ("_f32" if f32 else "", rc))
    return x


def merge_ranks(ptr, max_rows):
    ptr = np.asarray(ptr)
    out = [int(ptr[0])]
    for k in range(1, len(ptr)):
        if ptr[k] - out[-1] > max_rows and ptr[k - 1] > out[-1]:
            out.append(int(ptr[k - 1]))
    if out[-1] != ptr[-1]:
        out.append(int(ptr[-1]))
    return np.array(out, dtype=np.int32)


def internal_layout(dofs, n_virtual, order="colour", schur_max_rows=0):
    L = _lib()
    cd = np.ascontiguousarray(dofs.cell_dofs, dtype=np.int32)
    cc = np.ascontiguousarray(dofs.cell_coords, dtype=np.float64)
    iu, ip = (np.ascontiguousarray(a, dtype=np.int32) for a in (dofs.owned_u_ptr, dofs.owned_p_ptr))
    cap = int(n_virtual) + len(iu) + 1
    perm2, perm1 = np.empty(dofs.n_nodes_p2, np.int32), np.empty(dofs.n_nodes_p1, np.int32)
    u_ptr, p_ptr, s_ptr = (np.empty(cap, np.int32) for _ in range(3))
    nr, ns, col = C.c_int32(), C.c_int32(), (C.c_int32 * 2)()
    rc = L.nsxh_internal_layout(dofs.dim, dofs.n_cells, dofs.dofs_per_cell, cd.ctypes.data_as(_i32p), cc.ctypes.data_as(_f64p), dofs.n_u, dofs.n_p,
                                len(iu) - 1, iu.ctypes.data_as(_i32p), ip.ctypes.data_as(_i32p), int(n_virtual), DoFs.ORDERINGS[order], int(schur_max_rows),
                                perm2.ctypes.data_as(_i32p), perm1.ctypes.data_as(_i32p), C.byref(nr), u_ptr.ctypes.data_as(_i32p),
                                p_ptr.ctypes.data_as(_i32p), C.byref(ns), s_ptr.ctypes.data_as(_i32p), col)
    if rc:
        raise ValueError("nsxh_internal_layout failed (%d)" % rc)
    return {"node_perm": perm2, "pnode_perm": perm1, "u_ptr": u_ptr[:nr.value + 1].copy(), "p_ptr": p_ptr[:nr.value + 1].copy(),
            "schur_ptr": s_ptr[:ns.value + 1].copy(), "colours": (int(col[0]), int(col[1]))}


class PermutedDoFs:

    def __init__(self, dofs, node_perm, pnode_perm, u_ptr, p_ptr):
# ... 44 lines not shown
```

### navierstokes_project_nm4pde_amd/host/frontend.cpp

```cpp
#include "../../include/nsx_host.h"

#include <algorithm>
#include <array>
#include <cmath>
#include <cstdio>
#include <cstring>
#include <fstream>
#include <iomanip>
#include <map>
#include <numeric>
#include <sstream>
#include <string>
#include <unordered_map>
#include <vector>

#include <sys/stat.h>

#include "graph.hpp"
#include "ilu_stream.hpp"
#include "layout.hpp"

namespace {

const int TRI_LINES[3][2] = {{0, 1}, {1, 2}, {2, 0}};
// ... 1274 lines not shown
  if (!rowptr || !colind || !block_ptr || !lu || !b || !x || ncomp < 1 || gap < 1 || entries_per_tick < 1 || entries_per_tick > 4) return -1;
  try {
    const nsx::Csr g = csr_of(n_rows, rowptr, colind);
    const std::vector<int32_t> bptr(block_ptr, block_ptr + n_blocks + 1);
    nsx::IluStream s;
    nsx::build_ilu_stream(g, bptr, blocks_per_wave, ncomp, gap, s, entries_per_tick);
    if (!s.ok) return -3;
    nsx::replay_ilu_stream(g, bptr, s, lu, b, x);
    return 0;
  } catch (const std::exception &) {
    return -1;
  }
}

extern "C" int nsxh_ilu_stream_apply_f32(int n_rows, const int32_t *rowptr, const int32_t *colind, int n_blocks, const int32_t *block_ptr,
                                         int blocks_per_wave, int ncomp, int gap, int entries_per_tick, const double *lu, const double *b, double *x) {
  if (!rowptr || !colind || !block_ptr || !lu || !b || !x || ncomp < 1 || gap < 1 || entries_per_tick < 1 || entries_per_tick > 4) return -1;
  try {
    const nsx::Csr g = csr_of(n_rows, rowptr, colind);
    const std::vector<int32_t> bptr(block_ptr, block_ptr + n_blocks + 1);
    nsx::IluStream s;
    nsx::build_ilu_stream(g, bptr, blocks_per_wave, ncomp, gap, s, entries_per_tick);
    if (!s.ok) return -3;
    std::vector<double> lu32(lu, lu + g.nnz());
    for (int64_t q = 0; q < g.nnz(); ++q)
      if (s.slot_of[q] >= 0) lu32[q] = (double)(float)lu[q];
    nsx::replay_ilu_stream(g, bptr, s, lu32.data(), b, x);
    return 0;
  } catch (const std::exception &) {
    return -1;
  }
}

extern "C" int nsxh_internal_layout(int dim, int n_cells, int dofs_per_cell, const int32_t *cell_dofs, const double *cell_coords, int n_u, int n_p,
                                    int n_in_ranks, const int32_t *in_u_ptr, const int32_t *in_p_ptr, int n_virtual, int order, int schur_max_rows,
                                    int32_t *node_perm, int32_t *pnode_perm, int32_t *n_ranks, int32_t *u_ptr, int32_t *p_ptr, int32_t *n_schur,
                                    int32_t *schur_ptr, int32_t *colours) {
  if ((dim != 2 && dim != 3) || n_cells < 1 || !cell_dofs || !cell_coords || n_in_ranks < 1 || !in_u_ptr || !in_p_ptr || n_virtual < 1 || n_u % dim) return -1;
  const int nv = dim + 1, nl = dim == 2 ? 3 : 6, np2 = nv + nl;
  if (dofs_per_cell != nv * (dim + 1) + nl * dim) return -1;
  std::vector<int32_t> c2((size_t)n_cells * np2), c1((size_t)n_cells * nv);
  std::vector<double> cen((size_t)n_cells * dim, 0.0);
  for (int c = 0; c < n_cells; ++c) {
    const int32_t *cd = cell_dofs + (size_t)c * dofs_per_cell;
    for (int a = 0; a < np2; ++a) c2[(size_t)c * np2 + a] = cd[a < nv ? (dim + 1) * a : nv * (dim + 1) + dim * (a - nv)] / dim;
    for (int v = 0; v < nv; ++v) c1[(size_t)c * nv + v] = cd[(dim + 1) * v + dim] - n_u;
    for (int k = 0; k < nv; ++k)
      for (int d = 0; d < dim; ++d) cen[(size_t)c * dim + d] += cell_coords[((size_t)c * nv + k) * dim + d] / nv;
  }
  nsx::LayoutIn in;
  in.dim = dim;
  in.n_cells = n_cells;
  in.np2 = np2;
  in.np1 = nv;
  in.c2 = c2.data();
  in.c1 = c1.data();
  in.cen = cen.data();
  in.N2 = in.N2_all = n_u / dim;
  in.NP = n_p;
  in.in_u_ptr.assign(in_u_ptr, in_u_ptr + n_in_ranks + 1);
  in.in_p_ptr.assign(in_p_ptr, in_p_ptr + n_in_ranks + 1);
  nsx::LayoutOut out;
  nsx::build_layout(in, n_virtual, order, schur_max_rows, out);
  std::copy(out.perm2.begin(), out.perm2.end(), node_perm);
  std::copy(out.perm1.begin(), out.perm1.end(), pnode_perm);
  *n_ranks = (int32_t)out.u_ptr.size() - 1;
// ... 12 lines not shown
```

### navierstokes_project_nm4pde_amd/host/ilu_stream.hpp

```cpp
#pragma once
#include <algorithm>
#include <cstdint>
#include <queue>
#include <stdexcept>
#include <vector>

#include "graph.hpp"

namespace nsx {

struct IluStream {
  int n_waves = 0, ncomp = 1, gap = 2, epl = 1;
  int max_wave_rows = 0;
  int64_t n_slabs = 0, max_wave_slabs = 0;
  int64_t in_block_nnz = 0;
  int64_t used_slots = 0;
  std::vector<int32_t> wave_ptr;
  std::vector<int32_t> wave_blk;
  std::vector<int32_t> slab_ptr;
  std::vector<uint32_t> meta;
  std::vector<int32_t> slot_of;
  std::vector<int32_t> xoff;
  std::vector<int32_t> row_ptr;
  std::vector<int32_t> rows;
  bool ok = false;
};

constexpr int ilu_meta_words(int epl) { return (epl + 2) / 2; }
constexpr int ILU_STREAM_PAD = 32;
#ifndef NSX_ILU_STREAM_ALIGN
#define NSX_ILU_STREAM_ALIGN 4
#endif
constexpr int ILU_STREAM_ALIGN = NSX_ILU_STREAM_ALIGN;

inline void build_ilu_stream(const Csr &g, const std::vector<int32_t> &bptr, int blocks_per_wave, int ncomp, int gap, IluStream &s,
                             int entries_per_tick = 1) {
  const int E = std::max(1, std::min(4, entries_per_tick)), MW = ilu_meta_words(E);
  s.epl = E;
  const int nb = (int)bptr.size() - 1, BPW = std::max(1, blocks_per_wave);
  const int nw = std::max(1, (nb + BPW - 1) / BPW);
  gap = std::max(1, gap);
  s.n_waves = nw;
  s.ncomp = ncomp;
  s.gap = gap;
  s.slab_ptr.assign(2 * (size_t)nw + 1, 0);
  s.meta.clear();
  s.slot_of.assign((size_t)g.nnz(), -1);
  s.xoff.assign(g.n_rows, 0);
  s.max_wave_rows = 0;
  s.in_block_nnz = s.used_slots = 0;
  std::vector<int32_t> blk_of(g.n_rows, 0);
  std::vector<int64_t> blk_work(nb, 0);
  for (int b = 0; b < nb; ++b)
    for (int i = bptr[b]; i < bptr[b + 1]; ++i) {
      blk_of[i] = b;
      for (int q = g.rowptr[i]; q < g.rowptr[i + 1]; ++q) blk_work[b] += g.colind[q] >= bptr[b] && g.colind[q] < bptr[b + 1];
    }
// ... 146 lines not shown
          for (int e = 0; e < n_here; ++e) {
            const int q = order[order_ptr[L.row] + L.k + e];
            put_half(base + l, e, (uint32_t)s.xoff[g.colind[q]] * row_bytes);
            s.slot_of[q] = (int32_t)((base + l) * E + e);
            s.used_slots++;
          }
          L.k += n_here;
          const uint32_t last = L.k == len[L.row] ? 2u : 0u;
          s.meta[(base + l) * MW] |= first | last;
          put_half(base + l, E, (uint32_t)s.xoff[L.row] * row_bytes);
          if (last) {
            ++done;
            L.row = -1;
          }
        }
        avail.erase(avail.begin(), avail.begin() + next_avail);
        if (!any && planned.empty()) throw std::runtime_error("ILU stream: dependency cycle (graph not structurally symmetric inside a block?)");
        for (int j : started) {
          const int b = blk_of[j];
          for (int q = g.rowptr[j]; q < g.rowptr[j + 1]; ++q) {
            const int i = g.colind[q];
            if (!(fwd ? (i > j && i < bptr[b + 1]) : (i < j && i >= bptr[b]))) continue;
            if (len[i] == 0) continue;
            if (--pend[i] == 0) plan(i, tick + 1);
          }
        }
        ++tick;
      }
      for (; tick % ILU_STREAM_ALIGN != 0; ++tick) idle_slab();
      s.slab_ptr[2 * (size_t)w + 1 + dir] = (int32_t)(s.meta.size() / ((size_t)64 * MW));
    }
    s.max_wave_slabs = std::max<int64_t>(s.max_wave_slabs, s.slab_ptr[2 * (size_t)w + 2] - s.slab_ptr[2 * (size_t)w]);
  }
  s.n_slabs = (int64_t)(s.meta.size() / ((size_t)64 * MW));
  s.meta.resize(s.meta.size() + (size_t)ILU_STREAM_PAD * 64 * MW, 0u);
}

inline void replay_ilu_stream(const Csr &g, const std::vector<int32_t> &bptr, const IluStream &s, const double *lu, const double *b, double *x) {
  const int nc = s.ncomp, E = s.epl, MW = ilu_meta_words(E);
  std::vector<double> val((size_t)(s.n_slabs + ILU_STREAM_PAD) * 64 * E, 0.0);
  for (int64_t q = 0; q < g.nnz(); ++q)
    if (s.slot_of[q] >= 0) val[s.slot_of[q]] = -lu[q];
  std::vector<int32_t> diag(g.n_rows, -1);
  for (int i = 0; i < g.n_rows; ++i) diag[i] = find_in_row(g, i, i);
  auto half = [&](size_t slot, int k) { return (s.meta[slot * MW + k / 2] >> (16 * (k & 1))) & 0xffffu; };
  std::vector<double> xs, acc(64 * (size_t)nc), gx(64 * (size_t)nc * E), fx(64 * (size_t)nc), pend_w(64 * (size_t)nc);
  std::vector<int64_t> pend_a(64);
  for (int w = 0; w < s.n_waves; ++w) {
    xs.assign((size_t)(s.max_wave_rows + 64) * nc, 0.0);
    for (int t = s.row_ptr[w]; t < s.row_ptr[w + 1]; ++t)
      for (int c = 0; c < nc; ++c) xs[(size_t)(t - s.row_ptr[w]) * nc + c] = b[(size_t)s.rows[t] * nc + c];
    for (int dir = 0; dir < 2; ++dir) {
      std::fill(acc.begin(), acc.end(), 0.0);
      std::fill(pend_a.begin(), pend_a.end(), -1);
      const int sa = s.slab_ptr[2 * (size_t)w + dir], sb = s.slab_ptr[2 * (size_t)w + dir + 1];
      auto land = [&]() {
        for (int l = 0; l < 64; ++l)
          if (pend_a[l] >= 0) {
            for (int c = 0; c < nc; ++c) xs[(size_t)pend_a[l] + c] = pend_w[(size_t)l * nc + c];
            pend_a[l] = -1;
          }
      };
      for (int sl = sa; sl < sb; ++sl) {
        for (int l = 0; l < 64; ++l) {
          const size_t slot = (size_t)sl * 64 + l;
          for (int e = 0; e < E; ++e) {
            const size_t ca = (half(slot, e) & 0xfff8u) / 8;
            for (int c = 0; c < nc; ++c) gx[((size_t)l * E + e) * nc + c] = xs[ca + c];
          }
          const size_t da = half(slot, E) / 8;
          for (int c = 0; c < nc; ++c) fx[(size_t)l * nc + c] = xs[da + c];
        }
        land();
        for (int l = 0; l < 64; ++l) {
          const size_t slot = (size_t)sl * 64 + l;
          const uint32_t fl = half(slot, 0) & 3u;
          for (int c = 0; c < nc; ++c) {
            double a = (fl & 1u) ? fx[(size_t)l * nc + c] : acc[(size_t)l * nc + c];
            for (int e = 0; e < E; ++e) a += val[slot * E + e] * gx[((size_t)l * E + e) * nc + c];
            acc[(size_t)l * nc + c] = a;
            if (fl & 2u) pend_w[(size_t)l * nc + c] = a;
          }
          if (fl & 2u) pend_a[l] = (int64_t)(half(slot, E) / 8);
        }
// ... 13 lines not shown
```

### navierstokes_project_nm4pde_amd/nsx.py

```python
import ctypes as C

import numpy as np

from ._lib import DEV_SO, load

_i32p = C.POINTER(C.c_int32)
_f64p = C.POINTER(C.c_double)

TEMAM, DOUBLE_CONVECTION = 1, 2
YOSIDA, SIMPLE, AYOSIDA, ASIMPLE = 0, 1, 2, 3

API = [
    "nsx_create", "nsx_destroy", "nsx_last_error", "nsx_version", "nsx_set_tables", "nsx_set_mesh", "nsx_set_ranks",
    "nsx_set_schur_blocks", "nsx_set_solution", "nsx_get_solution", "nsx_get_solution_ghosted", "nsx_get_rhs",
    "nsx_set_rhs", "nsx_assemble", "nsx_assemble_time_step", "nsx_add_rhs", "nsx_apply_boundary_values",
    "nsx_solve_time_step", "nsx_prec_initialize", "nsx_prec_vmult", "nsx_system_vmult", "nsx_ilu_apply",
    "nsx_export_block", "nsx_schur_nnz", "nsx_schur_get", "nsx_scalar_graph_nnz", "nsx_scalar_graph", "nsx_ilu_get",
    "nsx_profile_enable", "nsx_profile_reset", "nsx_profile_count", "nsx_profile_get", "nsx_persistent_state", "nsx_path_info", "nsx_comm_self_halo_test", "nsx_comm_unique_id",
    "nsx_comm_init", "nsx_comm_init_callbacks", "nsx_comm_counters", "nsx_set_mesh_distributed", "nsx_set_force_faces", "nsx_compute_forces",
    "nsx_set_internal_layout", "nsx_layout_info", "nsx_layout_get", "nsx_gram_schmidt_cycle", "nsx_set_inner_precision",
]
API_EXTRA = ["nsx_inner_F_vmult"]
FIRST_TOUCH, COLOUR, COLOUR_ALL = 0, 1, 2
INNER_FP64, INNER_FP32 = 0, 1

ALLREDUCE_FN = C.CFUNCTYPE(C.c_int, C.c_void_p, _f64p, C.c_int)
EXCHANGE_FN = C.CFUNCTYPE(C.c_int, C.c_void_p, C.c_int, C.POINTER(C.c_int), C.POINTER(_f64p), C.POINTER(C.c_int),
                          C.POINTER(_f64p), C.POINTER(C.c_int))


class Params(C.Structure):
    _fields_ = [("dim", C.c_int), ("device", C.c_int), ("nu", C.c_double), ("deltat", C.c_double)]


class Stats(C.Structure):
    _fields_ = [("outer_iterations", C.c_int), ("inner_F_iterations", C.c_int), ("inner_S_iterations", C.c_int),
                ("n_F_solves", C.c_int), ("n_S_solves", C.c_int), ("final_residual", C.c_double),
                ("t_prec", C.c_double), ("t_solve", C.c_double), ("status", C.c_int), ("persistent_fallbacks", C.c_int)]

    def as_dict(self):
        return {k: getattr(self, k) for k, _ in self._fields_}


class NsxError(RuntimeError):
    def __init__(self, code, msg):
        super().__init__("nsx error %d: %s" % (code, msg))
        self.code = code


def lib():
    L = load(DEV_SO)
    if getattr(L, "_nsx_ready", False):
        return L
    vp = C.c_void_p
    L.nsx_create.argtypes = [C.POINTER(Params), C.POINTER(vp)]
# ... 11 lines not shown
    L.nsx_gram_schmidt_cycle.argtypes = [vp, C.c_int, C.c_int, _f64p, C.c_double, _f64p, _f64p]
    for f in ("nsx_set_solution", "nsx_get_solution", "nsx_get_solution_ghosted", "nsx_get_rhs", "nsx_set_rhs"):
        getattr(L, f).argtypes = [vp, _f64p]
    L.nsx_assemble.argtypes = [vp, C.c_int]
    L.nsx_assemble_time_step.argtypes = [vp, C.c_int]
    L.nsx_add_rhs.argtypes = [vp, C.c_int, _i32p, _f64p]
    L.nsx_apply_boundary_values.argtypes = [vp, C.c_int, _i32p, _f64p]
    L.nsx_solve_time_step.argtypes = [vp, C.c_int, C.c_double, C.c_double, C.c_int, C.c_int, C.POINTER(Stats)]
    L.nsx_prec_initialize.argtypes = [vp, C.c_int]
    L.nsx_prec_vmult.argtypes = [vp, C.c_int, C.c_double, C.c_int, _f64p, _f64p, C.POINTER(Stats)]
    L.nsx_system_vmult.argtypes = [vp, _f64p, _f64p]
    L.nsx_ilu_apply.argtypes = [vp, C.c_int, _f64p, _f64p]
    L.nsx_export_block.argtypes = [vp, C.c_int, C.c_int, C.c_int, _i32p, _i32p, _f64p]
    L.nsx_schur_nnz.argtypes = [vp, C.POINTER(C.c_int64)]
    L.nsx_schur_get.argtypes = [vp, _i32p, _i32p, _f64p]
    L.nsx_scalar_graph_nnz.argtypes = [vp, C.c_int, C.POINTER(C.c_int64)]
    L.nsx_scalar_graph.argtypes = [vp, C.c_int, _i32p, _i32p]
    L.nsx_ilu_get.argtypes = [vp, C.c_int, _f64p]
    L.nsx_profile_enable.argtypes = [vp, C.c_int]
    L.nsx_profile_reset.argtypes = [vp]
    L.nsx_profile_count.argtypes = [vp]
    L.nsx_profile_get.argtypes = [vp, C.c_int, C.POINTER(C.c_char_p), C.POINTER(C.c_int64), _f64p, _f64p]
    L.nsx_persistent_state.argtypes = [vp, C.POINTER(C.c_int)]
    L.nsx_comm_unique_id.argtypes = [C.POINTER(C.c_uint8)]
    L.nsx_comm_init.argtypes = [vp, C.c_int, C.c_int, C.POINTER(C.c_uint8)]
    L.nsx_comm_init_callbacks.argtypes = [vp, C.c_int, C.c_int, ALLREDUCE_FN, EXCHANGE_FN, C.c_void_p]
    L.nsx_comm_counters.argtypes = [vp, C.POINTER(C.c_longlong)]
    L.nsx_set_mesh_distributed.argtypes = [vp, C.c_int, C.c_int, C.c_int, _i32p, _f64p, C.c_int, C.c_int, C.c_int, C.c_int,
                                           _i32p, _i32p, C.c_int, _i32p, _i32p, _i32p, _i32p, _i32p]
    L.nsx_set_force_faces.argtypes = [vp, C.c_int, _i32p, _i32p, C.c_int, _f64p, _f64p, _f64p, _f64p]
    L.nsx_compute_forces.argtypes = [vp, _f64p, _f64p]
    L.nsx_set_inner_precision.argtypes = [vp, C.c_int]
    L.nsx_inner_F_vmult.argtypes = [vp, _f64p, _f64p]
    L._nsx_ready = True
    return L


def _i(a):
    return a.ctypes.data_as(_i32p)


def _d(a):
    return a.ctypes.data_as(_f64p)


def _ci(a):
    return np.ascontiguousarray(a, dtype=np.int32)


def _cd(a):
    return np.ascontiguousarray(a, dtype=np.float64)


def gloo_callbacks():
    import torch
    import torch.distributed as dist

    def allreduce(ctx, buf, count):
        t = torch.from_numpy(np.ctypeslib.as_array(buf, shape=(count,)))
        dist.all_reduce(t)
        return 0

    def exchange(ctx, n, ranks, send, scount, recv, rcount):
        reqs, keep = [], []
        for k in range(n):
            if rcount[k]:
# ... 39 lines not shown
            return
        v = dofs.rank_view(rank, world)
        self.view = v
        cd, cc = _ci(v["cell_dofs"]), _cd(v["cell_coords"])
        arrs = [_ci(v[k]) for k in ("gpu_u_ptr", "gpu_p_ptr", "neighbors", "send_u_ptr", "send_u_nodes", "send_p_ptr", "send_p_nodes")]
        self._ck(L.nsx_set_mesh_distributed(self._h, v["n_cells"], v["n_cells_layer1"], dofs.dofs_per_cell, _i(cd), _d(cc),
                                            dofs.n_u, dofs.n_p, world, rank, _i(arrs[0]), _i(arrs[1]), len(arrs[2]), _i(arrs[2]),
                                            _i(arrs[3]), _i(arrs[4]), _i(arrs[5]), _i(arrs[6])))
        if len(v["rank_u_ptr"]) > 2:
            self.set_ranks(v["rank_u_ptr"], v["rank_p_ptr"])
        if comm == "callbacks":
            self._cb = gloo_callbacks()
            self._ck(L.nsx_comm_init_callbacks(self._h, rank, world, self._cb[0], self._cb[1], None))
        else:
            import torch.distributed as dist
            ident = (C.c_uint8 * 128)()
            if rank == 0:
                self._ck(L.nsx_comm_unique_id(ident))
            box = [bytes(ident)]
            dist.broadcast_object_list(box, src=0)
            ident = (C.c_uint8 * 128).from_buffer_copy(box[0])
            self._ck(L.nsx_comm_init(self._h, rank, world, ident))

    def persistent_state(self):
        st = (C.c_int * 4)()
        self._ck(self.L.nsx_persistent_state(self._h, st))
        return {"sweep_persistent": bool(st[0]), "cg_persistent": bool(st[1]), "fallbacks": int(st[2]), "dirty_mailbox_words": int(st[3])}

    PATH_KEYS = ("spmv_lds_staged", "spmv_chunks", "spmv_chunks_behind_halo", "sweep_entries_per_thread", "sweep_grid", "sweep_collective_inside",
                 "sweep_entries_per_thread_max", "cus_reserved", "schur_cg_path", "schur_blocks", "neighbours", "nodes_sent_per_exchange", "ghost_nodes",
                 "schur_dense_inverses", "sweep_off", "fallbacks", "rccl_sweep_velocity_plain", "rccl_sweep_velocity_masked", "rccl_sweep_block_plain",
                 "rccl_sweep_block_masked", "schur_blocks_per_partial", "sweep_velocity_one_gpu", "owned_p2_nodes", "owned_p1_nodes", "sweep_with_ilu_inside", "fused_launches",
                 "inner_F_fp32", "ilu_F_fp32")

    def path_info(self):
        v = (C.c_int * 32)()
        self._ck(self.L.nsx_path_info(self._h, v))
        return {k: int(v[i]) for i, k in enumerate(self.PATH_KEYS)}

    def comm_counters(self):
        c = (C.c_longlong * 2)()
        self._ck(self.L.nsx_comm_counters(self._h, c))
        return int(c[0]), int(c[1])

    def comm_self_halo_test(self, n_own, n_ghost, ncomp):
        e = C.c_double(0.0)
        self._ck(self.L.nsx_comm_self_halo_test(self._h, int(n_own), int(n_ghost), int(ncomp), C.byref(e)))
        return float(e.value)

    def comm_init_single(self):
        ident = (C.c_uint8 * 128)()
        self._ck(self.L.nsx_comm_unique_id(ident))
        self._ck(self.L.nsx_comm_init(self._h, 0, 1, ident))

    def gather_solution(self):
        x = np.zeros(self.n)
        self._ck(self.L.nsx_get_solution(self._h, _d(x)))
        if self.world > 1:
            import torch
            import torch.distributed as dist
            t = torch.from_numpy(x)
            if dist.get_backend() == "nccl":
                t = t.cuda()
            dist.all_reduce(t)
            x = t.cpu().numpy()
        return x

    def _ck(self, rc):
        if rc:
            raise NsxError(rc, (self.L.nsx_last_error(self._h) or b"").decode())

# ... 80 lines not shown
        dofs, vals = _ci(dofs), _cd(vals)
        self._ck(self.L.nsx_apply_boundary_values(self._h, len(dofs), _i(dofs), _d(vals)))

    def solve_time_step(self, prec=YOSIDA, tol_abs=1e-4, inner_rtol=1e-2, maxiter=100000, inner_maxiter=100000,
                        check=True):
        st = Stats()
        rc = self.L.nsx_solve_time_step(self._h, prec, tol_abs, inner_rtol, maxiter, inner_maxiter, C.byref(st))
        if rc and (check or rc != -4):
            self._ck(rc)
        return st.as_dict()

    def prec_initialize(self, prec):
        self._ck(self.L.nsx_prec_initialize(self._h, prec))

    def prec_vmult(self, prec, src, inner_rtol=1e-2, inner_maxiter=100000, dst0=None):
        src = _cd(src)
        dst = np.zeros_like(src) if dst0 is None else _cd(dst0).copy()
        st = Stats()
        self._ck(self.L.nsx_prec_vmult(self._h, prec, inner_rtol, inner_maxiter, _d(dst), _d(src), C.byref(st)))
        return dst, st.as_dict()

    def system_vmult(self, src):
        src = _cd(src)
        dst = np.zeros_like(src)
        self._ck(self.L.nsx_system_vmult(self._h, _d(dst), _d(src)))
        return dst

    def inner_F_vmult(self, src):
        src = _cd(src)
        dst = np.empty_like(src)
        self._ck(self.L.nsx_inner_F_vmult(self._h, _d(dst), _d(src)))
        return dst

    def ilu_apply(self, which, src):
        src = _cd(src)
        dst = np.empty_like(src)
        self._ck(self.L.nsx_ilu_apply(self._h, which, _d(dst), _d(src)))
        return dst

    def gram_schmidt_cycle(self, vectors, norm_guard=-1.0):
        v = np.ascontiguousarray(vectors, dtype=np.float64).copy()
        m, n = v.shape
        coeffs, norms2 = np.zeros((m, m)), np.zeros(m)
        self._ck(self.L.nsx_gram_schmidt_cycle(self._h, n, m, _d(v), float(norm_guard), _d(coeffs), _d(norms2)))
        return v, coeffs, norms2

    def set_force_faces(self, cells, lfaces, ftab):
        cells, lfaces = np.asarray(cells), np.asarray(lfaces)
        if self.world > 1:
            n_sub = self.dofs.n_subdomains // self.world
            mine = (self.dofs.mesh.subdomain[cells] // n_sub) == self.rank
            pos = {int(c): i for i, c in enumerate(self.view["cell_ids"])}
            cells = np.array([pos[int(c)] for c in cells[mine]], dtype=np.int32)
            lfaces = lfaces[mine]
        cells, lfaces = _ci(cells), _ci(lfaces)
        N2, dN2, N1, w = _cd(ftab.N2), _cd(ftab.dN2), _cd(ftab.N1), _cd(ftab.weights[:ftab.n_qf])
        self._ck(self.L.nsx_set_force_faces(self._h, len(cells), _i(cells), _i(lfaces), ftab.n_qf, _d(N2), _d(dN2), _d(N1), _d(w)))

    def compute_forces(self):
        d, l = C.c_double(), C.c_double()
        self._ck(self.L.nsx_compute_forces(self._h, C.byref(d), C.byref(l)))
        return d.value, l.value

    def export_block(self, which, block, graph=None):
        rowptr, colind = graph if graph is not None else self.dofs.reference_sparsity(3 if which == 4 else block)
        rowptr, colind = _ci(rowptr), _ci(colind)
# ... 39 lines not shown
```

Baseline: 14.09.

## Hand F SpMV output to ILU in packed order and drop Yosida copies

Adds a fused path in which the F matrix-vector product writes its result directly in the ILU stream's packed row order, so the ILU solve reads it without a gather. GMRES now accepts a separate initial guess and a final destination with subtraction, which removes several vector copies and zeroing passes in the Yosida preconditioner (the lean mode is on by default). The CG Schur solve likewise reads its initial guess from a separate buffer. These changes target memory traffic and launch count per preconditioner application, at the cost of more complex buffer aliasing logic in GMRES.

```diff
diff --git a/include/nsx.h b/include/nsx.h
--- a/include/nsx.h
+++ b/include/nsx.h
@@ -88,6 +88,7 @@
 enum { NSX_INNER_FP64 = 0, NSX_INNER_FP32 = 1 };
 int nsx_set_inner_precision(nsx_handle *h, int precision);
 int nsx_inner_F_vmult(nsx_handle *h, double *dst, const double *src);
+int nsx_inner_F_ilu_apply(nsx_handle *h, double *dst, const double *src, int packed);
 
 int nsx_export_block(nsx_handle *h, int which, int block, int n_rows, const int32_t *rowptr, const int32_t *colind,
                      double *values);
diff --git a/include/nsx_host.h b/include/nsx_host.h
--- a/include/nsx_host.h
+++ b/include/nsx_host.h
@@ -108,6 +108,12 @@
 int nsxh_ilu_stream_apply_f32(int n_rows, const int32_t *rowptr, const int32_t *colind, int n_blocks, const int32_t *block_ptr,
                               int blocks_per_wave, int ncomp, int gap, int entries_per_tick, const double *lu, const double *b, double *x);
 
+int nsxh_ilu_stream_tables(int n_rows, const int32_t *rowptr, const int32_t *colind, int n_blocks, const int32_t *block_ptr,
+                           int blocks_per_wave, int ncomp, int gap, int entries_per_tick, int32_t *rows, int32_t *pos_of_row,
+                           int32_t *n_waves, int32_t *row_ptr);
+int nsxh_ilu_stream_apply_packed(int n_rows, const int32_t *rowptr, const int32_t *colind, int n_blocks, const int32_t *block_ptr,
+                                 int blocks_per_wave, int ncomp, int gap, int entries_per_tick, const double *lu, const double *b_packed, double *x);
+
 int nsxh_internal_layout(int dim, int n_cells, int dofs_per_cell, const int32_t *cell_dofs, const double *cell_coords, int n_u, int n_p,
                          int n_in_ranks, const int32_t *in_u_ptr, const int32_t *in_p_ptr, int n_virtual, int order, int schur_max_rows,
                          int32_t *node_perm, int32_t *pnode_perm, int32_t *n_ranks, int32_t *u_ptr, int32_t *p_ptr, int32_t *n_schur,
diff --git a/navierstokes_project_nm4pde_amd/csrc/nsx_blas.hip b/navierstokes_project_nm4pde_amd/csrc/nsx_blas.hip
--- a/navierstokes_project_nm4pde_amd/csrc/nsx_blas.hip
+++ b/navierstokes_project_nm4pde_amd/csrc/nsx_blas.hip
@@ -1836,12 +1836,12 @@
   double c[32];
   int k;
 };
-__global__ void k_axpy_multi(int n, int split, int gap, double *__restrict__ x, MultiArgs m) {
+__global__ void k_axpy_multi(int n, int split, int gap, const double *x_in, double *x_out, const double *sub, MultiArgs m) {
   for (int i0 = blockIdx.x * 256 + threadIdx.x; i0 < n; i0 += gridDim.x * 256) {
     const int i = i0 + (i0 >= split ? gap : 0);
-    double s = x[i];
+    double s = x_in ? x_in[i] : 0.0;
     for (int j = 0; j < m.k; ++j) s += m.c[j] * m.v[j][i];
-    x[i] = s;
+    x_out[i] = sub ? s - sub[i] : s;
   }
 }
 __global__ __launch_bounds__(256) void k_cg_update(int n, double *__restrict__ x, const double *__restrict__ dvec, double *__restrict__ g,
@@ -1888,17 +1888,19 @@
   LaunchScope ls(h, "scale_vec", 24.0 * n);
   hipLaunchKernelGGL(k_scale_vec, dim3(ew_blocks(n)), dim3(256), 0, h->stream, n, d, f);
 }
-void v_axpy_multi(nsx_handle *h, Span sp, double *x, int k, double *const *vs, const double *coef) {
+void v_axpy_multi(nsx_handle *h, Span sp, double *x, int k, double *const *vs, const double *coef) { v_axpy_multi(h, sp, x, x, k, vs, coef, nullptr); }
+void v_axpy_multi(nsx_handle *h, Span sp, const double *x_in, double *x_out, int k, double *const *vs, const double *coef, const double *sub) {
   const int n = sp.n;
-  for (int j0 = 0; j0 < k; j0 += 32) {
+  for (int j0 = 0; j0 < std::max(k, 1); j0 += 32) {
     MultiArgs m;
     m.k = std::min(32, k - j0);
     for (int j = 0; j < m.k; ++j) {
       m.v[j] = vs[j0 + j];
       m.c[j] = coef[j0 + j];
     }
-    LaunchScope ls(h, "axpy_multi", 8.0 * n * (2 + m.k));
-    hipLaunchKernelGGL(k_axpy_multi, dim3(ew_blocks(n)), dim3(256), 0, h->stream, n, sp.split, sp.gap, x, m);
+    const bool last = j0 + 32 >= k;
+    LaunchScope ls(h, "axpy_multi", 8.0 * n * ((x_in ? 2 : 1) + (sub && last ? 1 : 0) + m.k));
+    hipLaunchKernelGGL(k_axpy_multi, dim3(ew_blocks(n)), dim3(256), 0, h->stream, n, sp.split, sp.gap, j0 == 0 ? x_in : x_out, x_out, last ? sub : nullptr, m);
   }
 }
 
@@ -2058,6 +2060,7 @@
     info[25] = h->mgs_fused_launches;
     info[26] = h->inner_F_fp32_used;
     info[27] = h->ilu_F_fp32_used;
+    info[28] = h->handover_used;
   } catch (const nsx::Error &e) {
     h->err = e.msg;
     return e.code;
diff --git a/navierstokes_project_nm4pde_amd/csrc/nsx_cg.hip b/navierstokes_project_nm4pde_amd/csrc/nsx_cg.hip
--- a/navierstokes_project_nm4pde_amd/csrc/nsx_cg.hip
+++ b/navierstokes_project_nm4pde_amd/csrc/nsx_cg.hip
@@ -156,7 +156,7 @@
                                                   const int32_t *__restrict__ u_cols, const int32_t *__restrict__ s_ptr,
                                                   const double *__restrict__ sval, const uint16_t *__restrict__ slidx,
                                                   const int32_t *__restrict__ sinfo, const int64_t *__restrict__ dn_off,
-                                                  const double *__restrict__ P, const double *__restrict__ b, double *x, double *D0, double *D1,
+                                                  const double *__restrict__ P, const double *__restrict__ b, const double *x_in, double *x, double *D0, double *D1,
                                                   double *H, double rtol, int maxiter, unsigned long long *box, unsigned long long *box_other,
                                                   double *pub_vals, unsigned long long *pub_flag, unsigned long long seq, int *err_dev, int drop_wg,
                                                   const int32_t *__restrict__ a_rowptr, const double *__restrict__ a_val,
@@ -299,12 +299,12 @@
 
   double bi = 0.0;
   if (own) {
-    xs[tid] = x[r0 + tid];
+    xs[tid] = x_in[r0 + tid];
     bi = b[r0 + tid];
   }
 #pragma unroll
   for (int k = 0; k < NU; ++k)
-    if (ucol[k] >= 0) xst[tid + CG_THREADS * k] = x[ucol[k]];
+    if (ucol[k] >= 0) xst[tid + CG_THREADS * k] = x_in[ucol[k]];
   prefetch_A();
   __syncthreads();
   block_spmv();
@@ -493,7 +493,7 @@
             h->cg_max_wg, per_cu_res[0], per_cu_res[1], per_cu_lres[0], per_cu_lres[1]);
 }
 
-bool cg_schur_persistent(nsx_handle *h, double *x, const double *b, double rtol, int maxiter, int *steps, double *last, int *status) {
+bool cg_schur_persistent(nsx_handle *h, const double *x_in, double *x, const double *b, double rtol, int maxiter, int *steps, double *last, int *status) {
   const IluSchedule &s = h->schedS;
   const CgPlan &pl = h->cgplan;
   if (h->comm || !s.dense || s.max_rows > CG_MAXB || !pl.ok || !pl.values_current) return false;
@@ -518,7 +518,7 @@
     pe = ls.e;
 #define NSX_CG_GO(PRES_, LRES_)                                                                                                                       \
   hipLaunchKernelGGL((k_cg_schur<PRES_, LRES_>), dim3(s.n_blocks), dim3(CG_THREADS), 0, h->stream, s.block_ptr.p, pl.u_ptr.p, pl.u_cols.p, pl.s_ptr.p,  \
-                     pl.s_val.p, pl.s_lidx.p, pl.s_info.p, s.dn_off.p, s.dn_P.p, b, x, D0, D1, H, rtol, maxiter, box, box_other, pub_vals, pub_flag, seq, \
+                     pl.s_val.p, pl.s_lidx.p, pl.s_info.p, s.dn_off.p, s.dn_P.p, b, x_in, x, D0, D1, H, rtol, maxiter, box, box_other, pub_vals, pub_flag, seq, \
                      err_dev, h->gx_drop_wg, h->gS.rowptr.p, h->vSchur.p, pl.a_lidx.p)
     if (rpg == 6 && lres) NSX_CG_GO(6, true); else if (rpg == 8 && lres) NSX_CG_GO(8, true);
     else if (rpg == 6) NSX_CG_GO(6, false); else if (rpg == 8) NSX_CG_GO(8, false); else NSX_CG_GO(0, false);
diff --git a/navierstokes_project_nm4pde_amd/csrc/nsx_internal.hpp b/navierstokes_project_nm4pde_amd/csrc/nsx_internal.hpp
--- a/navierstokes_project_nm4pde_amd/csrc/nsx_internal.hpp
+++ b/navierstokes_project_nm4pde_amd/csrc/nsx_internal.hpp
@@ -221,6 +221,7 @@
   int inner_precision = NSX_INNER_FP64;
   nsx::DevBuf<float> vF32;
   int inner_F_fp32_used = 0, ilu_F_fp32_used = 0;
+  int handover_used = 0;
   nsx::DevBuf<int32_t> bt_of_g;
   nsx::GatherMap gmA, gmG, gmB, gmPM;
   nsx::DevBuf<double> cellbuf;
@@ -343,8 +344,10 @@
 void run_dirichlet(nsx_handle *h, int n, const int32_t *dofs, const double *vals);
 
 bool blocked_usable(const nsx_handle *h);
-void spmv_F(nsx_handle *h, const double *vals, const double *x, double *y, const float *vals32 = nullptr);
+void spmv_F(nsx_handle *h, const double *vals, const double *x, double *y, const float *vals32 = nullptr, const int32_t *pos = nullptr);
 void spmv_F_inner(nsx_handle *h, const double *x, double *y);
+void spmv_F_ilu(nsx_handle *h, const double *src, double *tmp, double *dst, bool allow_packed);
+bool handover_enabled();
 void convert_F_f32(nsx_handle *h);
 void spmv_saddle(nsx_handle *h, const double *x, double *y);
 void spmv_G(nsx_handle *h, const double *xp, double *yu, bool accumulate);
@@ -354,7 +357,7 @@
 void ilu_factor(nsx_handle *h, const DevCsr &g, IluSchedule &s, const double *vals, double *lu, const char *name, bool f32 = false);
 void ilu_check(nsx_handle *h);
 bool ilu_solve(nsx_handle *h, const DevCsr &g, const IluSchedule &s, const double *lu, const double *b, double *x, int ncomp,
-               const char *name, int dot_slot = -1, bool f32 = false, int *used_f32 = nullptr);
+               const char *name, int dot_slot = -1, bool f32 = false, int *used_f32 = nullptr, bool b_packed = false);
 void extract_diag(nsx_handle *h, const DevCsr &g, const double *vals, double *d);
 void abs_rowsum(nsx_handle *h, const DevCsr &g, const double *vals, double *d);
 
@@ -393,6 +396,7 @@
 bool v_mgs(nsx_handle *h, Span n, double *w, int dim, double *const *vs, int slot0, bool normalize, double *out,
            const std::function<void()> *after_launch = nullptr, bool consider = false, double *gram = nullptr, const double *ilu_rhs = nullptr);
 void v_axpy_multi(nsx_handle *h, Span n, double *x, int k, double *const *vs, const double *coef_host);
+void v_axpy_multi(nsx_handle *h, Span n, const double *x_in, double *x_out, int k, double *const *vs, const double *coef_host, const double *sub);
 void finalize_slots(nsx_handle *h, int slot0, int count);
 double *red_out(nsx_handle *h, int slot, int nb);
 void after_reduction(nsx_handle *h, int slot, int nb);
@@ -404,7 +408,7 @@
 void wait_published(nsx_handle *h, unsigned long long seq);
 void build_cg_plan(nsx_handle *h);
 void cg_pack_values(nsx_handle *h);
-bool cg_schur_persistent(nsx_handle *h, double *x, const double *b, double rtol, int maxiter, int *steps, double *last, int *status);
+bool cg_schur_persistent(nsx_handle *h, const double *x_in, double *x, const double *b, double rtol, int maxiter, int *steps, double *last, int *status);
 bool cg_schur_fused(nsx_handle *h, double *x, const double *b, double rtol, int maxiter, int *steps, double *last, int *status);
 void write_scalar(nsx_handle *h, int slot, double v);
 
diff --git a/navierstokes_project_nm4pde_amd/csrc/nsx_setup.hip b/navierstokes_project_nm4pde_amd/csrc/nsx_setup.hip
--- a/navierstokes_project_nm4pde_amd/csrc/nsx_setup.hip
+++ b/navierstokes_project_nm4pde_amd/csrc/nsx_setup.hip
@@ -224,11 +224,7 @@
               (long long)st.in_block_nnz, st.max_wave_rows, st.ok ? "" : " (too many: not used)");
     s.pk_row_ptr.upload(st.row_ptr, h->stream);
     s.pk_rows.upload(st.rows, h->stream);
-    {
-      std::vector<int32_t> slot(g.n_rows);
-      for (size_t k = 0; k < st.rows.size(); ++k) slot[st.rows[k]] = (int32_t)k;
-      s.pk_dinv_slot.upload(slot, h->stream);
-    }
+    s.pk_dinv_slot.upload(st.pos_of_row, h->stream);
     s.pk_slab_ptr.upload(st.slab_ptr, h->stream);
     s.pk_meta.upload(reinterpret_cast<const int32_t *>(st.meta.data()), st.meta.size(), h->stream);
     s.pk_slot_of.upload(st.slot_of, h->stream);
diff --git a/navierstokes_project_nm4pde_amd/csrc/nsx_solve.hip b/navierstokes_project_nm4pde_amd/csrc/nsx_solve.hip
--- a/navierstokes_project_nm4pde_amd/csrc/nsx_solve.hip
+++ b/navierstokes_project_nm4pde_amd/csrc/nsx_solve.hip
@@ -33,6 +33,7 @@
 };
 
 using Op = std::function<void(double *dst, const double *src)>;
+using OpPair = std::function<void(double *dst, double *tmp, const double *src)>;
 
 struct SolveResult {
   int status;
@@ -70,7 +71,8 @@
 enum { S_H = 8 , S_NRM = 40, S_H2 = 41 , S_DH = 2, S_GH = 3, S_RES = 4, S_GH2 = 5 , S_T = 6 };
 
 static SolveResult gmres(nsx_handle *h, const Op &A, double *x, const double *b, const Op &P, Span n, int len, double tol, int maxiter,
-                         bool zero_new = false, bool x_is_zero = false, bool plain_P = false, bool P_is_ilu_F = false) {
+                         bool zero_new = false, bool x_is_zero = false, bool plain_P = false, bool P_is_ilu_F = false, const OpPair *AP = nullptr,
+                         const double *x0 = nullptr, double *fin_dst = nullptr, const double *fin_sub = nullptr) {
   SolveResult res{1, 0, 0.0};
   std::vector<std::unique_ptr<Tmp>> tmp(N_TMP);
   auto vec = [&](int i) -> double * {
@@ -102,13 +104,14 @@
   bool re_orth = false;
   double *v = vec(0), *p = vec(N_TMP - 1);
   int ahead = 0;
+  const double *xin = x0 ? x0 : x;
+  bool fin_written = false;
   do {
     ahead = 0;
     if (x_is_zero) {
       P(v, b);
-      x_is_zero = false;
     } else {
-      A(p, x);
+      A(p, xin);
       v_sadd(h, n, p, -1., 1., b);
       P(v, p);
     }
@@ -127,6 +130,10 @@
       if (trace && h->gmres_depth == 1) fprintf(stderr, "[nsx trace] rank %d: outer iteration %d, residual %.3e\n", h->rank, accumulated, rho);
       double *vv = vec(inner + 1);
       auto apply_AP = [&](double *dst, const double *src) {
+        if (AP && plain_P) {
+          (*AP)(dst, p, src);
+          return;
+        }
         A(p, src);
         P(dst, p);
       };
@@ -203,8 +210,15 @@
     }
     double *vs[N_TMP];
     for (int i = 0; i < dim; ++i) vs[i] = vec(i);
-    v_axpy_multi(h, n, x, dim, vs, y);
+    const bool fin = fin_dst && state != 0;
+    v_axpy_multi(h, n, x_is_zero ? nullptr : xin, fin ? fin_dst : x, dim, vs, y, fin ? fin_sub : nullptr);
+    fin_written = fin;
+    x_is_zero = false;
+    xin = x;
   } while (state == 0);
+  if (fin_dst && !fin_written) v_axpy_multi(h, n, x_is_zero ? nullptr : xin, fin_dst, 0, nullptr, nullptr, fin_sub);
+  else if (!fin_dst && x_is_zero) v_zero(h, n.n, x);
+  else if (!fin_dst && xin != x) v_copy(h, n.n, x, xin);
   res.status = state == 1 ? 0 : 1;
   res.steps = accumulated;
   return res;
@@ -372,35 +386,45 @@
     if (used) h->ilu_F_fp32_used = 1;
   };
   Op PS = [h](double *d, const double *s) { ilu_solve(h, h->gS, h->schedS, h->luS.p, s, d, 1, "ilu_solve_S"); };
+  OpPair FPF = [h](double *d, double *t, const double *s) { spmv_F_ilu(h, s, t, d, true); };
   OpDot PSdot = [h](double *d, const double *s, int slot) { return ilu_solve(h, h->gS, h->schedS, h->luS.p, s, d, 1, "ilu_solve_S", slot); };
-  auto cg_S = [&](double *x, const double *b) {
+  auto cg_S = [&](double *x, const double *b, const double *x0 = nullptr) {
     int steps = 0, status = 0;
     double last = 0.0;
-    if (cg_schur_persistent(h, x, b, tol, maxit, &steps, &last, &status)) return SolveResult{status, steps, last};
+    if (cg_schur_persistent(h, x0 ? x0 : x, x, b, tol, maxit, &steps, &last, &status)) return SolveResult{status, steps, last};
+    if (x0) v_copy(h, n_p, x, x0);
     if (cg_schur_fused(h, x, b, tol, maxit, &steps, &last, &status)) return SolveResult{status, steps, last};
     h->cg_last_path = 1;
     return cg(h, Sm, x, b, PS, n_p, len_p, tol * norm2(h, n_p, b), maxit, &PSdot);
   };
 
+  const bool lean = !(getenv("NSX_PREC_LEAN") && atoi(getenv("NSX_PREC_LEAN")) == 0);
   if (type == NSX_PREC_YOSIDA) {
     Tmp yu(h, len_u), yp(h, len_p), tmp(h, len_p), tmp2(h, len_u), res(h, len_u);
-    v_copy(h, n_u, yu.p(), src_u);
-    v_copy(h, n_p, yp.p(), src_p);
-    count(st, true, gmres(h, Fm, yu.p(), src_u, PF, n_u, len_u, tol * norm2(h, n_u, src_u), maxit, false, false, true, true));
+    if (!lean) v_copy(h, n_u, yu.p(), src_u);
+    if (!lean) v_copy(h, n_p, yp.p(), src_p);
+    count(st, true, gmres(h, Fm, yu.p(), src_u, PF, n_u, len_u, tol * norm2(h, n_u, src_u), maxit, false, false, true, true, &FPF, lean ? src_u : nullptr));
     spmv_B(h, yu.p(), tmp.p());
     v_add(h, n_p, tmp.p(), -1.0, src_p);
-    count(st, false, cg_S(yp.p(), tmp.p()));
-    v_copy(h, n_p, dst_p, yp.p());
+    if (lean) {
+      count(st, false, cg_S(dst_p, tmp.p(), src_p));
+    } else {
+      count(st, false, cg_S(yp.p(), tmp.p()));
+      v_copy(h, n_p, dst_p, yp.p());
+    }
     spmv_G(h, dst_p, tmp2.p(), false);
-    v_zero(h, n_u, res.p());
-    v_copy(h, n_u, dst_u, yu.p());
-    count(st, true, gmres(h, Fm, res.p(), tmp2.p(), PF, n_u, len_u, tol * norm2(h, n_u, tmp2.p()), maxit, false, true, true, true));
-    v_sadd(h, n_u, dst_u, -1., 1., res.p());
+    if (!lean) {
+      v_zero(h, n_u, res.p());
+      v_copy(h, n_u, dst_u, yu.p());
+    }
+    count(st, true, gmres(h, Fm, res.p(), tmp2.p(), PF, n_u, len_u, tol * norm2(h, n_u, tmp2.p()), maxit, false, true, true, true, &FPF, nullptr,
+                          lean ? dst_u : nullptr, lean ? yu.p() : nullptr));
+    if (!lean) v_sadd(h, n_u, dst_u, -1., 1., res.p());
   } else if (type == NSX_PREC_SIMPLE) {
     Tmp sol1_u(h, len_u), sol1_p(h, len_p), temp_1(h, len_p), tmp(h, len_u);
-    v_copy(h, n_u, sol1_u.p(), src_u);
+    if (!lean) v_copy(h, n_u, sol1_u.p(), src_u);
     v_copy(h, n_p, sol1_p.p(), src_p);
-    count(st, true, gmres(h, Fm, sol1_u.p(), src_u, PF, n_u, len_u, tol * norm2(h, n_u, src_u), maxit, false, false, true, true));
+    count(st, true, gmres(h, Fm, sol1_u.p(), src_u, PF, n_u, len_u, tol * norm2(h, n_u, src_u), maxit, false, false, true, true, &FPF, lean ? src_u : nullptr));
     spmv_B(h, sol1_u.p(), temp_1.p());
     v_add(h, n_p, temp_1.p(), -1.0, src_p);
     count(st, false, cg_S(sol1_p.p(), temp_1.p()));
@@ -412,7 +436,7 @@
     v_add(h, n_u, dst_u, -1.0, tmp.p());
   } else if (type == NSX_PREC_ASIMPLE) {
     Tmp tmp_u(h, len_u), tmp_p(h, len_p);
-    count(st, true, gmres(h, Fm, dst_u, src_u, PF, n_u, len_u, tol * norm2(h, n_u, src_u), maxit, false, false, true, true));
+    count(st, true, gmres(h, Fm, dst_u, src_u, PF, n_u, len_u, tol * norm2(h, n_u, src_u), maxit, false, false, true, true, &FPF));
     spmv_B(h, dst_u, dst_p);
     v_sadd(h, n_p, dst_p, -1.0, 1.0, src_p);
     v_copy(h, n_p, tmp_p.p(), dst_p);
@@ -449,7 +473,7 @@
   nsx_solve_stats local;
   if (!st) st = &local;
   memset(st, 0, sizeof(*st));
-  h->inner_F_fp32_used = h->ilu_F_fp32_used = 0;
+  h->inner_F_fp32_used = h->ilu_F_fp32_used = h->handover_used = 0;
   v_copy(h, h->len_blk, h->prev_sol.p, h->sol.p);
   HIP_CHECK(hipStreamSynchronize(h->stream));
   double t0 = now_s();
@@ -535,7 +559,7 @@
     if (stats) memset(stats, 0, sizeof(*stats));
     h->defer_red = false;
     h->pending_red.clear();
-    h->inner_F_fp32_used = h->ilu_F_fp32_used = 0;
+    h->inner_F_fp32_used = h->ilu_F_fp32_used = h->handover_used = 0;
     nsx::prec_vmult(h, prec_type, inner_rtol, inner_maxiter, d.p(), s.p(), stats);
     if (stats) stats->persistent_fallbacks = h->n_persistent_fallbacks;
     nsx::vec_to_caller(h, d.p(), dst);
@@ -592,4 +616,27 @@
   })
 }
 
-}
+int nsx_inner_F_ilu_apply(nsx_handle *h, double *dst, const double *src, int packed) {
+  NSX_API_BODY(h, {
+    if (!dst || !src || !h->assembled) NSX_THROW(NSX_ERR_ARG, "null vector / nothing assembled");
+    if (!h->prec_ready) NSX_THROW(NSX_ERR_ARG, "no factors: call nsx_prec_initialize first");
+    HIP_CHECK(hipSetDevice(h->prm.device));
+    h->inner_F_fp32_used = h->ilu_F_fp32_used = h->handover_used = 0;
+    nsx::Tmp t(h, h->len_u);
+    if (h->dist) {
+      nsx::Tmp d(h, h->len_blk), s(h, h->len_blk);
+      nsx::vec_from_caller(h, s.p(), src, false);
+      nsx::v_zero(h, h->len_blk, d.p());
+      nsx::spmv_F_ilu(h, s.p(), t.p(), d.p(), packed != 0);
+      nsx::vec_to_caller(h, d.p(), dst);
+    } else {
+      nsx::Tmp d(h, h->len_u), s(h, h->len_u);
+      nsx::part_from_caller(h, 0, s.p(), src);
+      nsx::spmv_F_ilu(h, s.p(), t.p(), d.p(), packed != 0);
+      nsx::part_to_caller(h, 0, d.p(), dst);
+    }
+    nsx::ilu_check(h);
+  })
+}
+
+}
diff --git a/navierstokes_project_nm4pde_amd/csrc/nsx_sparse.hip b/navierstokes_project_nm4pde_amd/csrc/nsx_sparse.hip
--- a/navierstokes_project_nm4pde_amd/csrc/nsx_sparse.hip
+++ b/navierstokes_project_nm4pde_amd/csrc/nsx_sparse.hip
@@ -134,7 +134,7 @@
 template <int DIM, int W, class VT>
 __device__ __forceinline__ void spmv_blocked_rows(int n_rows, const int32_t *__restrict__ desc, const int32_t *__restrict__ rp,
                                                   const uint16_t *__restrict__ lidx, const VT *__restrict__ av, const int32_t *__restrict__ ucols,
-                                                  const double *__restrict__ x, double *__restrict__ y) {
+                                                  const double *__restrict__ x, double *__restrict__ y, const int32_t *__restrict__ pos) {
   extern __shared__ double xs[];
   __shared__ int rps[449];
   const int4 d = reinterpret_cast<const int4 *>(desc)[blockIdx.x];
@@ -156,9 +156,11 @@
   const int grp = threadIdx.x / W, lane = threadIdx.x % W;
   double a[U], na[U];
   int l[U], nl[U];
+  int at = 0, nat = 0;
   int row = r0 + grp;
-  auto fetch = [&](int rw, double (&va)[U], int (&vl)[U]) {
+  auto fetch = [&](int rw, double (&va)[U], int (&vl)[U], int &vat) {
     const bool live = rw < r1;
+    vat = pos && live && lane == 0 ? pos[rw] : rw;
     const int p0 = live ? rps[rw - r0] + lane : 0, e = live ? rps[rw - r0 + 1] : 0;
 #pragma unroll
     for (int k = 0; k < U; ++k) {
@@ -168,7 +170,7 @@
       vl[k] = ok ? (int)ld_stream<2>(lidx + q) : 0;
     }
   };
-  auto consume = [&](int rw, const double (&va)[U], const int (&vl)[U]) {
+  auto consume = [&](int rw, const double (&va)[U], const int (&vl)[U], int vat) {
     if (rw >= r1) return;
     double acc[DIM];
 #pragma unroll
@@ -190,17 +192,17 @@
     for (int c = 0; c < DIM; ++c) acc[c] = group_sum<W>(acc[c]);
     if (lane == 0) {
 #pragma unroll
-      for (int c = 0; c < DIM; ++c) y[(size_t)rw * DIM + c] = acc[c];
+      for (int c = 0; c < DIM; ++c) y[(size_t)vat * DIM + c] = acc[c];
     }
   };
   if (SPMV_DBG == 3) row = r1;
-  fetch(row, a, l);
-  fetch(row + G, na, nl);
+  fetch(row, a, l, at);
+  fetch(row + G, na, nl, nat);
   for (; row < r1; row += 2 * G) {
-    consume(row, a, l);
-    fetch(row + 2 * G, a, l);
-    consume(row + G, na, nl);
-    fetch(row + 3 * G, na, nl);
+    consume(row, a, l, at);
+    fetch(row + 2 * G, a, l, at);
+    consume(row + G, na, nl, nat);
+    fetch(row + 3 * G, na, nl, nat);
   }
 #ifdef NSX_SPMV_TRACE
   __syncthreads();
@@ -217,8 +219,8 @@
 template <int DIM, int W>
 __global__ __launch_bounds__(256) void k_spmv_blocked(int n_rows, const int32_t *__restrict__ desc, const int32_t *__restrict__ rp, const uint16_t *__restrict__ lidx,
                                                       const double *__restrict__ av, const int32_t *__restrict__ ucols, const double *__restrict__ x,
-                                                      double *__restrict__ y) {
-  spmv_blocked_rows<DIM, W, double>(n_rows, desc, rp, lidx, av, ucols, x, y);
+                                                      double *__restrict__ y, const int32_t *__restrict__ pos) {
+  spmv_blocked_rows<DIM, W, double>(n_rows, desc, rp, lidx, av, ucols, x, y, pos);
 }
 #ifndef NSX_SPMV_F32_W
 #define NSX_SPMV_F32_W 16
@@ -226,8 +228,8 @@
 template <int DIM, int W>
 __global__ __launch_bounds__(256) void k_spmv_blocked_f32(int n_rows, const int32_t *__restrict__ desc, const int32_t *__restrict__ rp, const uint16_t *__restrict__ lidx,
                                                           const float *__restrict__ av, const int32_t *__restrict__ ucols, const double *__restrict__ x,
-                                                          double *__restrict__ y) {
-  spmv_blocked_rows<DIM, W, float>(n_rows, desc, rp, lidx, av, ucols, x, y);
+                                                          double *__restrict__ y, const int32_t *__restrict__ pos) {
+  spmv_blocked_rows<DIM, W, float>(n_rows, desc, rp, lidx, av, ucols, x, y, pos);
 }
 
 __global__ __launch_bounds__(256) void k_to_f32(int64_t n, const double *__restrict__ v, float *__restrict__ out, int *__restrict__ err) {
@@ -286,7 +288,7 @@
   const SpmvBlocked &b = h->blkA;
   return blocked && b.n_chunks > 0 && b.max_rows <= 448 && (size_t)b.max_ucols * h->dim * sizeof(double) <= 64 * 1024;
 }
-static bool launch_blocked(nsx_handle *h, const double *vals, const double *x, double *y, int part = 0, const float *vals32 = nullptr) {
+static bool launch_blocked(nsx_handle *h, const double *vals, const double *x, double *y, int part = 0, const float *vals32 = nullptr, const int32_t *pos = nullptr) {
   const SpmvBlocked &b = h->blkA;
   if (!blocked_usable(h)) return false;
   const size_t shm = (size_t)b.max_ucols * h->dim * sizeof(double);
@@ -294,12 +296,12 @@
   const int32_t *desc = part ? b.desc_if.p : b.desc.p;
   if (grid == 0) return true;
 #define NSX_BLK(D) \
-  hipLaunchKernelGGL((k_spmv_blocked<D, 16>), dim3(grid), dim3(256), shm, h->stream, h->N2, desc, h->gA.rowptr.p, b.lidx.p, vals, b.ucols.p, x, y)
+  hipLaunchKernelGGL((k_spmv_blocked<D, 16>), dim3(grid), dim3(256), shm, h->stream, h->N2, desc, h->gA.rowptr.p, b.lidx.p, vals, b.ucols.p, x, y, pos)
   if (vals32) {
     if (h->dim == 2)
-      hipLaunchKernelGGL((k_spmv_blocked_f32<2, NSX_SPMV_F32_W>), dim3(grid), dim3(256), shm, h->stream, h->N2, desc, h->gA.rowptr.p, b.lidx.p, vals32, b.ucols.p, x, y);
+      hipLaunchKernelGGL((k_spmv_blocked_f32<2, NSX_SPMV_F32_W>), dim3(grid), dim3(256), shm, h->stream, h->N2, desc, h->gA.rowptr.p, b.lidx.p, vals32, b.ucols.p, x, y, pos);
     else
-      hipLaunchKernelGGL((k_spmv_blocked_f32<3, NSX_SPMV_F32_W>), dim3(grid), dim3(256), shm, h->stream, h->N2, desc, h->gA.rowptr.p, b.lidx.p, vals32, b.ucols.p, x, y);
+      hipLaunchKernelGGL((k_spmv_blocked_f32<3, NSX_SPMV_F32_W>), dim3(grid), dim3(256), shm, h->stream, h->N2, desc, h->gA.rowptr.p, b.lidx.p, vals32, b.ucols.p, x, y, pos);
     return true;
   }
 #ifdef NSX_SPMV_TRACE
@@ -343,7 +345,8 @@
   return nn ? 16.0 * (p.send_ptr[nn] + p.recv_ptr[nn]) * ncomp : 0.0;
 }
 
-void spmv_F(nsx_handle *h, const double *vals, const double *x, double *y, const float *vals32) {
+void spmv_F(nsx_handle *h, const double *vals, const double *x, double *y, const float *vals32, const int32_t *pos) {
+  if (pos && !blocked_usable(h)) NSX_THROW(NSX_ERR_ARG, "internal: only the LDS-staged product stores by a position table");
   if (vals32 && !blocked_usable(h)) vals32 = nullptr;
   const bool f32 = vals32 != nullptr;
   if (f32) h->inner_F_fp32_used = 1;
@@ -354,7 +357,7 @@
     comm_halo_begin(h, h->haloU, xx, h->dim);
     {
       LaunchScope ls(h, "spmv_F", bytes_vel(h, false, f32) * (1.0 - frac_if));
-      if (blk) launch_blocked(h, vals, x, y, 0, vals32);
+      if (blk) launch_blocked(h, vals, x, y, 0, vals32, pos);
       else launch_vel(h, false, vals, x, nullptr, y, h->splitA.interior.p, h->splitA.n_interior);
     }
     {
@@ -363,17 +366,29 @@
     }
     {
       LaunchScope ls(h, "spmv_F_if", bytes_vel(h, false, f32) * frac_if);
-      if (blk) launch_blocked(h, vals, x, y, 1, vals32);
+      if (blk) launch_blocked(h, vals, x, y, 1, vals32, pos);
       else launch_vel(h, false, vals, x, nullptr, y, h->splitA.interface.p, h->splitA.n_interface);
     }
     return;
   }
   LaunchScope ls(h, "spmv_F", bytes_vel(h, false, f32));
-  if (!launch_blocked(h, vals, x, y, 0, vals32)) launch_vel(h, false, vals, x, nullptr, y, nullptr, h->N2);
+  if (!launch_blocked(h, vals, x, y, 0, vals32, pos)) launch_vel(h, false, vals, x, nullptr, y, nullptr, h->N2);
 }
 
 void spmv_F_inner(nsx_handle *h, const double *x, double *y) {
   spmv_F(h, h->vF.p, x, y, h->inner_precision == NSX_INNER_FP32 ? h->vF32.p : nullptr);
+}
+
+bool handover_enabled() { return getenv("NSX_HANDOVER") && atoi(getenv("NSX_HANDOVER")) == 1; }
+void spmv_F_ilu(nsx_handle *h, const double *src, double *tmp, double *dst, bool allow_packed) {
+  const bool f32 = h->inner_precision == NSX_INNER_FP32;
+  const IluSchedule &s = h->schedF;
+  const bool packed = allow_packed && handover_enabled() && blocked_usable(h) && ilu_lanes_stream(s, h->dim) && s.pk_dinv_slot.n == (size_t)h->N2 && tmp != dst;
+  spmv_F(h, h->vF.p, src, tmp, f32 ? h->vF32.p : nullptr, packed ? s.pk_dinv_slot.p : nullptr);
+  int used = 0;
+  ilu_solve(h, h->gA, s, h->luF.p, tmp, dst, h->dim, "ilu_solve_F", -1, f32, &used, packed);
+  if (used) h->ilu_F_fp32_used = 1;
+  if (packed) h->handover_used = 1;
 }
 
 static double bytes_B(nsx_handle *h) { return (4.0 + 8.0 * h->dim) * h->gB.nnz() + 12.0 * h->NP + 8.0 * h->dim * h->N2; }
@@ -1169,7 +1184,7 @@
 __device__ __forceinline__ void ilu_solve_lanes_wave(const int32_t *__restrict__ row_ptr, const int32_t *__restrict__ rows,
                                                      const int32_t *__restrict__ slab_ptr, const uint32_t *__restrict__ meta,
                                                      const VT *__restrict__ val, const double *__restrict__ dinv, const double *b, double *x,
-                                                     double *__restrict__ dot_partial, int *err_host, int force_guard) {
+                                                     double *__restrict__ dot_partial, int *err_host, int force_guard, int b_packed) {
   extern __shared__ double xs[];
   if ((uint32_t)(uintptr_t)(lds_f64 *)xs != 0u || force_guard) {
     if (threadIdx.x == 0) __hip_atomic_store(err_host, 3, __ATOMIC_RELAXED, __HIP_MEMORY_SCOPE_SYSTEM);
@@ -1192,13 +1207,22 @@
   }
   {
     double v[K][NCOMP];
+    if (b_packed) {
+#pragma unroll
+      for (int k = 0; k < K; ++k) {
+        const int t = 64 * k + (int)lane;
+#pragma unroll
+        for (int c = 0; c < NCOMP; ++c) v[k][c] = t < nr ? b[(size_t)(rb + t) * NCOMP + c] : 0.0;
+      }
+    } else {
+#pragma unroll
+      for (int k = 0; k < K; ++k)
+#pragma unroll
+        for (int c = 0; c < NCOMP; ++c) v[k][c] = idx0[k] >= 0 ? b[(size_t)idx0[k] * NCOMP + c] : 0.0;
+    }
 #pragma unroll
     for (int k = 0; k < K; ++k)
-#pragma unroll
-      for (int c = 0; c < NCOMP; ++c) v[k][c] = idx0[k] >= 0 ? b[(size_t)idx0[k] * NCOMP + c] : 0.0;
-#pragma unroll
-    for (int k = 0; k < K; ++k)
-      if (idx0[k] >= 0) {
+      if (64 * k + (int)lane < nr) {
 #pragma unroll
         for (int c = 0; c < NCOMP; ++c) xs[(64 * k + (int)lane) * NCOMP + c] = v[k][c];
       }
@@ -1214,7 +1238,7 @@
 #pragma unroll
     for (int k = 0; k < K; ++k)
 #pragma unroll
-      for (int c = 0; c < NCOMP; ++c) v[k][c] = idx[k] >= 0 ? b[(size_t)idx[k] * NCOMP + c] : 0.0;
+      for (int c = 0; c < NCOMP; ++c) v[k][c] = idx[k] >= 0 ? b[(size_t)(b_packed ? rb + base + 64 * k + (int)lane : idx[k]) * NCOMP + c] : 0.0;
 #pragma unroll
     for (int k = 0; k < K; ++k)
       if (idx[k] >= 0) {
@@ -1267,7 +1291,7 @@
 #pragma unroll
       for (int k = 0; k < K; ++k)
 #pragma unroll
-        for (int c = 0; c < NCOMP; ++c) bv[k][c] = idx[k] >= 0 ? b[(size_t)idx[k] * NCOMP + c] : 0.0;
+        for (int c = 0; c < NCOMP; ++c) bv[k][c] = idx[k] >= 0 ? b[(size_t)(b_packed ? rb + base + 64 * k + (int)lane : idx[k]) * NCOMP + c] : 0.0;
     }
 #pragma unroll
     for (int k = 0; k < K; ++k)
@@ -1290,29 +1314,31 @@
 __global__ __launch_bounds__(64) void k_ilu_solve_lanes(const int32_t *__restrict__ row_ptr, const int32_t *__restrict__ rows,
                                                         const int32_t *__restrict__ slab_ptr, const uint32_t *__restrict__ meta,
                                                         const double *__restrict__ val, const double *__restrict__ dinv, const double *b, double *x,
-                                                        double *__restrict__ dot_partial, int *err_host, int force_guard) {
-  ilu_solve_lanes_wave<NCOMP, E, PF, double>(row_ptr, rows, slab_ptr, meta, val, dinv, b, x, dot_partial, err_host, force_guard);
+                                                        double *__restrict__ dot_partial, int *err_host, int force_guard, int b_packed) {
+  ilu_solve_lanes_wave<NCOMP, E, PF, double>(row_ptr, rows, slab_ptr, meta, val, dinv, b, x, dot_partial, err_host, force_guard, b_packed);
 }
 template <int NCOMP, int E, int PF>
 __global__ __launch_bounds__(64) void k_ilu_solve_lanes_f32(const int32_t *__restrict__ row_ptr, const int32_t *__restrict__ rows,
                                                             const int32_t *__restrict__ slab_ptr, const uint32_t *__restrict__ meta,
                                                             const float *__restrict__ val, const double *__restrict__ dinv, const double *b, double *x,
-                                                            double *__restrict__ dot_partial, int *err_host, int force_guard) {
-  ilu_solve_lanes_wave<NCOMP, E, PF, float>(row_ptr, rows, slab_ptr, meta, val, dinv, b, x, dot_partial, err_host, force_guard);
+                                                            double *__restrict__ dot_partial, int *err_host, int force_guard, int b_packed) {
+  ilu_solve_lanes_wave<NCOMP, E, PF, float>(row_ptr, rows, slab_ptr, meta, val, dinv, b, x, dot_partial, err_host, force_guard, b_packed);
 }
 
 template <int NCOMP>
-static void launch_lanes(nsx_handle *h, const IluSchedule &s, const double *b, double *x, double *dot_partial, bool f32) {
+static void launch_lanes(nsx_handle *h, const IluSchedule &s, const double *b, double *x, double *dot_partial, bool f32, bool b_packed) {
+  if (b_packed && b == x) NSX_THROW(NSX_ERR_ARG, "internal: a right-hand side in the waves' order cannot be solved in place");
+  const int bp = b_packed ? 1 : 0;
   const size_t shm = (size_t)(s.max_wave_rows + 64) * NCOMP * sizeof(double);
   static const int pf = getenv("NSX_PF") ? atoi(getenv("NSX_PF")) : 8;
   int *err = (int *)(h->pub_dev + N_SLOTS + 3);
   const int force_guard = getenv("NSX_ILU_LDS_GUARD_TEST") ? atoi(getenv("NSX_ILU_LDS_GUARD_TEST")) : 0;
 #define NSX_GO(E_, PF_)                                                                                                                        \
   hipLaunchKernelGGL((k_ilu_solve_lanes<NCOMP, E_, PF_>), dim3(s.n_waves), dim3(64), shm, h->stream, s.pk_row_ptr.p, s.pk_rows.p, s.pk_slab_ptr.p, \
-                     reinterpret_cast<const uint32_t *>(s.pk_meta.p), s.pk_val.p, s.pk_dinv.p, b, x, dot_partial, err, force_guard)
+                     reinterpret_cast<const uint32_t *>(s.pk_meta.p), s.pk_val.p, s.pk_dinv.p, b, x, dot_partial, err, force_guard, bp)
 #define NSX_GO32(E_, PF_)                                                                                                                          \
   hipLaunchKernelGGL((k_ilu_solve_lanes_f32<NCOMP, E_, PF_>), dim3(s.n_waves), dim3(64), shm, h->stream, s.pk_row_ptr.p, s.pk_rows.p, s.pk_slab_ptr.p, \
-                     reinterpret_cast<const uint32_t *>(s.pk_meta.p), s.pk_val32.p, s.pk_dinv.p, b, x, dot_partial, err, force_guard)
+                     reinterpret_cast<const uint32_t *>(s.pk_meta.p), s.pk_val32.p, s.pk_dinv.p, b, x, dot_partial, err, force_guard, bp)
 #define NSX_GO_E(E_)                                            \
   if (f32) {                                                    \
     if (pf == 4) NSX_GO32(E_, 4); else NSX_GO32(E_, 8);         \
@@ -1343,8 +1369,9 @@
 }
 
 bool ilu_solve(nsx_handle *h, const DevCsr &g, const IluSchedule &s, const double *lu, const double *b, double *x, int ncomp,
-               const char *name, int dot_slot, bool f32, int *used_f32) {
+               const char *name, int dot_slot, bool f32, int *used_f32, bool b_packed) {
   if (used_f32) *used_f32 = 0;
+  if (b_packed && !ilu_lanes_stream(s, ncomp)) NSX_THROW(NSX_ERR_ARG, "internal: only the lane-owner stream takes a right-hand side in its waves' order");
   if (s.levelled) {
     LaunchScope ls(h, name, 12.0 * (double)s.in_block_nnz + (double)g.n_rows() * (4 + 16.0 * ncomp));
     if (ncomp == 1) ilu_solve_levelled<1>(h, g, s, lu, b, x);
@@ -1368,9 +1395,9 @@
     if (used_f32) *used_f32 = lanes32 ? 1 : 0;
     const bool with_dot = dot_slot >= 0 && !h->comm && s.n_waves >= 2 && s.n_waves <= 512;
     double *dp = with_dot ? red_out(h, dot_slot, s.n_waves) : nullptr;
-    if (ncomp == 1) launch_lanes<1>(h, s, b, x, dp, lanes32);
-    else if (ncomp == 2) launch_lanes<2>(h, s, b, x, dp, lanes32);
-    else launch_lanes<3>(h, s, b, x, dp, lanes32);
+    if (ncomp == 1) launch_lanes<1>(h, s, b, x, dp, lanes32, b_packed);
+    else if (ncomp == 2) launch_lanes<2>(h, s, b, x, dp, lanes32, b_packed);
+    else launch_lanes<3>(h, s, b, x, dp, lanes32, b_packed);
     if (with_dot) after_reduction(h, dot_slot, s.n_waves);
     return with_dot;
   }
diff --git a/navierstokes_project_nm4pde_amd/frontend.py b/navierstokes_project_nm4pde_amd/frontend.py
--- a/navierstokes_project_nm4pde_amd/frontend.py
+++ b/navierstokes_project_nm4pde_amd/frontend.py
@@ -69,6 +69,8 @@
         "nsxh_ilu_stream_stats": (C.c_int, [C.c_int, _i32p, _i32p, C.c_int, _i32p, C.c_int, C.c_int, C.c_int, C.c_int, C.POINTER(C.c_int64)]),
         "nsxh_ilu_stream_apply": (C.c_int, [C.c_int, _i32p, _i32p, C.c_int, _i32p, C.c_int, C.c_int, C.c_int, C.c_int, _f64p, _f64p, _f64p]),
         "nsxh_ilu_stream_apply_f32": (C.c_int, [C.c_int, _i32p, _i32p, C.c_int, _i32p, C.c_int, C.c_int, C.c_int, C.c_int, _f64p, _f64p, _f64p]),
+        "nsxh_ilu_stream_apply_packed": (C.c_int, [C.c_int, _i32p, _i32p, C.c_int, _i32p, C.c_int, C.c_int, C.c_int, C.c_int, _f64p, _f64p, _f64p]),
+        "nsxh_ilu_stream_tables": (C.c_int, [C.c_int, _i32p, _i32p, C.c_int, _i32p, C.c_int, C.c_int, C.c_int, C.c_int, _i32p, _i32p, _i32p, _i32p]),
         "nsxh_internal_layout": (C.c_int, [C.c_int, C.c_int, C.c_int, _i32p, _f64p, C.c_int, C.c_int, C.c_int, _i32p, _i32p, C.c_int, C.c_int, C.c_int,
                                            _i32p, _i32p, _i32p, _i32p, _i32p, _i32p, _i32p, _i32p]),
     }
@@ -298,6 +300,30 @@
     return x
 
 
+def ilu_stream_tables(rowptr, colind, block_ptr, ncomp=1, blocks_per_wave=8, gap=2, entries_per_tick=1):
+    rp, ci, bp = (np.ascontiguousarray(a, dtype=np.int32) for a in (rowptr, colind, block_ptr))
+    n = len(rp) - 1
+    rows, pos, wptr, nw = np.empty(n, np.int32), np.empty(n, np.int32), np.zeros(len(bp), np.int32), np.zeros(1, np.int32)
+    rc = _lib().nsxh_ilu_stream_tables(n, rp.ctypes.data_as(_i32p), ci.ctypes.data_as(_i32p), len(bp) - 1, bp.ctypes.data_as(_i32p),
+                                       int(blocks_per_wave), int(ncomp), int(gap), int(entries_per_tick), rows.ctypes.data_as(_i32p),
+                                       pos.ctypes.data_as(_i32p), nw.ctypes.data_as(_i32p), wptr.ctypes.data_as(_i32p))
+    if rc:
+        raise ValueError("nsxh_ilu_stream_tables failed (%d)" % rc)
+    return rows, pos, wptr[:int(nw[0]) + 1].copy()
+
+
+def ilu_stream_apply_packed(rowptr, colind, block_ptr, lu, b_packed, ncomp=1, blocks_per_wave=8, gap=2, entries_per_tick=1):
+    rp, ci, bp = (np.ascontiguousarray(a, dtype=np.int32) for a in (rowptr, colind, block_ptr))
+    lu, b = np.ascontiguousarray(lu, dtype=np.float64), np.ascontiguousarray(b_packed, dtype=np.float64)
+    x = np.empty_like(b)
+    rc = _lib().nsxh_ilu_stream_apply_packed(len(rp) - 1, rp.ctypes.data_as(_i32p), ci.ctypes.data_as(_i32p), len(bp) - 1, bp.ctypes.data_as(_i32p),
+                                             int(blocks_per_wave), int(ncomp), int(gap), int(entries_per_tick), lu.ctypes.data_as(_f64p),
+                                             b.ctypes.data_as(_f64p), x.ctypes.data_as(_f64p))
+    if rc:
+        raise ValueError("nsxh_ilu_stream_apply_packed failed (%d)" % rc)
+    return x
+
+
 def merge_ranks(ptr, max_rows):
     ptr = np.asarray(ptr)
     out = [int(ptr[0])]
diff --git a/navierstokes_project_nm4pde_amd/host/frontend.cpp b/navierstokes_project_nm4pde_amd/host/frontend.cpp
--- a/navierstokes_project_nm4pde_amd/host/frontend.cpp
+++ b/navierstokes_project_nm4pde_amd/host/frontend.cpp
@@ -1330,6 +1330,40 @@
   }
 }
 
+extern "C" int nsxh_ilu_stream_tables(int n_rows, const int32_t *rowptr, const int32_t *colind, int n_blocks, const int32_t *block_ptr,
+                                      int blocks_per_wave, int ncomp, int gap, int entries_per_tick, int32_t *rows, int32_t *pos_of_row,
+                                      int32_t *n_waves, int32_t *row_ptr) {
+  if (!rowptr || !colind || !block_ptr || !rows || !pos_of_row || !n_waves || !row_ptr || n_rows < 0 || n_blocks < 1 || ncomp < 1 || gap < 1 || entries_per_tick < 1 || entries_per_tick > 4) return -1;
+  try {
+    nsx::IluStream s;
+    nsx::build_ilu_stream(csr_of(n_rows, rowptr, colind), std::vector<int32_t>(block_ptr, block_ptr + n_blocks + 1), blocks_per_wave, ncomp, gap, s, entries_per_tick);
+    if ((int)s.rows.size() != n_rows || (int)s.pos_of_row.size() != n_rows) return -1;
+    std::copy(s.rows.begin(), s.rows.end(), rows);
+    std::copy(s.pos_of_row.begin(), s.pos_of_row.end(), pos_of_row);
+    *n_waves = s.n_waves;
+    std::copy(s.row_ptr.begin(), s.row_ptr.end(), row_ptr);
+    return s.ok ? 0 : -3;
+  } catch (const std::exception &) {
+    return -1;
+  }
+}
+
+extern "C" int nsxh_ilu_stream_apply_packed(int n_rows, const int32_t *rowptr, const int32_t *colind, int n_blocks, const int32_t *block_ptr,
+                                            int blocks_per_wave, int ncomp, int gap, int entries_per_tick, const double *lu, const double *b_packed, double *x) {
+  if (!rowptr || !colind || !block_ptr || !lu || !b_packed || !x || ncomp < 1 || gap < 1 || entries_per_tick < 1 || entries_per_tick > 4) return -1;
+  try {
+    const nsx::Csr g = csr_of(n_rows, rowptr, colind);
+    const std::vector<int32_t> bptr(block_ptr, block_ptr + n_blocks + 1);
+    nsx::IluStream s;
+    nsx::build_ilu_stream(g, bptr, blocks_per_wave, ncomp, gap, s, entries_per_tick);
+    if (!s.ok) return -3;
+    nsx::replay_ilu_stream(g, bptr, s, lu, b_packed, x, true);
+    return 0;
+  } catch (const std::exception &) {
+    return -1;
+  }
+}
+
 extern "C" int nsxh_internal_layout(int dim, int n_cells, int dofs_per_cell, const int32_t *cell_dofs, const double *cell_coords, int n_u, int n_p,
                                     int n_in_ranks, const int32_t *in_u_ptr, const int32_t *in_p_ptr, int n_virtual, int order, int schur_max_rows,
                                     int32_t *node_perm, int32_t *pnode_perm, int32_t *n_ranks, int32_t *u_ptr, int32_t *p_ptr, int32_t *n_schur,
diff --git a/navierstokes_project_nm4pde_amd/host/ilu_stream.hpp b/navierstokes_project_nm4pde_amd/host/ilu_stream.hpp
--- a/navierstokes_project_nm4pde_amd/host/ilu_stream.hpp
+++ b/navierstokes_project_nm4pde_amd/host/ilu_stream.hpp
@@ -23,6 +23,7 @@
   std::vector<int32_t> xoff;
   std::vector<int32_t> row_ptr;
   std::vector<int32_t> rows;
+  std::vector<int32_t> pos_of_row;
   bool ok = false;
 };
 
@@ -235,11 +236,14 @@
     }
     s.max_wave_slabs = std::max<int64_t>(s.max_wave_slabs, s.slab_ptr[2 * (size_t)w + 2] - s.slab_ptr[2 * (size_t)w]);
   }
+  s.pos_of_row.assign(g.n_rows, -1);
+  for (size_t k = 0; k < s.rows.size(); ++k) s.pos_of_row[s.rows[k]] = (int32_t)k;
   s.n_slabs = (int64_t)(s.meta.size() / ((size_t)64 * MW));
   s.meta.resize(s.meta.size() + (size_t)ILU_STREAM_PAD * 64 * MW, 0u);
 }
 
-inline void replay_ilu_stream(const Csr &g, const std::vector<int32_t> &bptr, const IluStream &s, const double *lu, const double *b, double *x) {
+inline void replay_ilu_stream(const Csr &g, const std::vector<int32_t> &bptr, const IluStream &s, const double *lu, const double *b, double *x,
+                              bool b_packed = false) {
   const int nc = s.ncomp, E = s.epl, MW = ilu_meta_words(E);
   std::vector<double> val((size_t)(s.n_slabs + ILU_STREAM_PAD) * 64 * E, 0.0);
   for (int64_t q = 0; q < g.nnz(); ++q)
@@ -252,7 +256,7 @@
   for (int w = 0; w < s.n_waves; ++w) {
     xs.assign((size_t)(s.max_wave_rows + 64) * nc, 0.0);
     for (int t = s.row_ptr[w]; t < s.row_ptr[w + 1]; ++t)
-      for (int c = 0; c < nc; ++c) xs[(size_t)(t - s.row_ptr[w]) * nc + c] = b[(size_t)s.rows[t] * nc + c];
+      for (int c = 0; c < nc; ++c) xs[(size_t)(t - s.row_ptr[w]) * nc + c] = b[(size_t)(b_packed ? t : s.rows[t]) * nc + c];
     for (int dir = 0; dir < 2; ++dir) {
       std::fill(acc.begin(), acc.end(), 0.0);
       std::fill(pend_a.begin(), pend_a.end(), -1);
diff --git a/navierstokes_project_nm4pde_amd/nsx.py b/navierstokes_project_nm4pde_amd/nsx.py
--- a/navierstokes_project_nm4pde_amd/nsx.py
+++ b/navierstokes_project_nm4pde_amd/nsx.py
@@ -20,7 +20,7 @@
     "nsx_comm_init", "nsx_comm_init_callbacks", "nsx_comm_counters", "nsx_set_mesh_distributed", "nsx_set_force_faces", "nsx_compute_forces",
     "nsx_set_internal_layout", "nsx_layout_info", "nsx_layout_get", "nsx_gram_schmidt_cycle", "nsx_set_inner_precision",
 ]
-API_EXTRA = ["nsx_inner_F_vmult"]
+API_EXTRA = ["nsx_inner_F_vmult", "nsx_inner_F_ilu_apply"]
 FIRST_TOUCH, COLOUR, COLOUR_ALL = 0, 1, 2
 INNER_FP64, INNER_FP32 = 0, 1
 
@@ -98,6 +98,7 @@
     L.nsx_compute_forces.argtypes = [vp, _f64p, _f64p]
     L.nsx_set_inner_precision.argtypes = [vp, C.c_int]
     L.nsx_inner_F_vmult.argtypes = [vp, _f64p, _f64p]
+    L.nsx_inner_F_ilu_apply.argtypes = [vp, _f64p, _f64p, C.c_int]
     L._nsx_ready = True
     return L
 
@@ -203,11 +204,12 @@
                  "schur_dense_inverses", "sweep_off", "fallbacks", "rccl_sweep_velocity_plain", "rccl_sweep_velocity_masked", "rccl_sweep_block_plain",
                  "rccl_sweep_block_masked", "schur_blocks_per_partial", "sweep_velocity_one_gpu", "owned_p2_nodes", "owned_p1_nodes", "sweep_with_ilu_inside", "fused_launches",
                  "inner_F_fp32", "ilu_F_fp32")
+    PATH_KEYS_MORE = ("inner_handover",)
 
     def path_info(self):
         v = (C.c_int * 32)()
         self._ck(self.L.nsx_path_info(self._h, v))
-        return {k: int(v[i]) for i, k in enumerate(self.PATH_KEYS)}
+        return {k: int(v[i]) for i, k in enumerate(self.PATH_KEYS + self.PATH_KEYS_MORE)}
 
     def comm_counters(self):
         c = (C.c_longlong * 2)()
@@ -354,6 +356,12 @@
         self._ck(self.L.nsx_inner_F_vmult(self._h, _d(dst), _d(src)))
         return dst
 
+    def inner_F_ilu_apply(self, src, packed=True):
+        src = _cd(src)
+        dst = np.zeros_like(src)
+        self._ck(self.L.nsx_inner_F_ilu_apply(self._h, _d(dst), _d(src), 1 if packed else 0))
+        return dst
+
     def ilu_apply(self, which, src):
         src = _cd(src)
         dst = np.empty_like(src)
```

Result: no change. 14.21 (median of 6 runs) (+0.8%).
